# tsilva/gymnasium-solver

Hardware: AMD Instinct MI355X
Metric: env steps/sec (rollout+PPO update), CartPole n_envs=4096, 1/2/4/8 MI355X (higher is better)
Workload: dtype f32; 1 GPU; CartPole-v1:ppo C2 (rollout 4096 envs x 32 steps + 20-epoch PPO update, B=256); n_envs_per_gpu=4096, n_steps=32, batch_size=256, n_epochs=20, policy=MLP 4-256-256-{2,1}, parallelism=single, graph=True, same_device=False, dp_mode=local, track_stats=False

## Files before the change

### gymnasium-solver_amd/csrc/gs_common.h

```cpp
#pragma once
#include <hip/hip_runtime.h>
#include <stdint.h>
#include <stdio.h>
#include <string>
#include <type_traits>

#include "../../include/gsamd.h"

typedef float f32x4 __attribute__((ext_vector_type(4)));
typedef __bf16 bf16x8 __attribute__((ext_vector_type(8)));

namespace gs {

#ifdef GS_STAMPS
extern __device__ unsigned long long g_stamp_acc[8][16];
extern __device__ unsigned long long g_stamp_cnt[8];
#define GS_STAMP_BEGIN_IF(k, cond)                                                 \
    unsigned long long _st_t[17];                                                  \
    int _st_n = 0;                                                                 \
    unsigned long long _st_entry = 0;                                              \
    const bool _st_on = (cond) && threadIdx.x == 0;                                \
    const int _st_k = (k);                                                         \
    if (_st_on) _st_t[0] = __builtin_amdgcn_s_memtime();
#define GS_STAMP_BEGIN(k) GS_STAMP_BEGIN_IF(k, blockIdx.x == 0 && blockIdx.y == 0)
#define GS_STAMP(i)                                                                \
    if (_st_on) _st_t[(i) + 1] = __builtin_amdgcn_s_memtime();                     \
    _st_n = (i) + 1;
#define GS_STAMP_T0 const unsigned long long _st_t0 = __builtin_amdgcn_s_memtime();
#define GS_STAMP_ENTRY                                                             \
    if (_st_on) _st_entry = __builtin_amdgcn_s_memtime() - _st_t0;
#define GS_STAMP_END(i)                                                            \
    GS_STAMP(i)                                                                    \
    if (_st_on) {                                                                  \
        atomicAdd(&g_stamp_acc[_st_k][15], _st_entry);                             \
        for (int _j = 0; _j < _st_n; ++_j)                                         \
            atomicAdd(&g_stamp_acc[_st_k][_j], _st_t[_j + 1] - _st_t[_j]);         \
        atomicAdd(&g_stamp_cnt[_st_k], 1ull);                                      \
    }
#else
#define GS_STAMP_BEGIN(k)
#define GS_STAMP_T0
#define GS_STAMP_ENTRY
#define GS_STAMP_BEGIN_IF(k, cond)
#define GS_STAMP(i)
#define GS_STAMP_END(i)
#endif

void set_error(const char *fmt, ...);
int hip_fail(hipError_t e, const char *what, const char *file, int line);

#define GS_HIP(call)                                                         \
    do {                                                                     \
        hipError_t _e = (call);                                              \
        if (_e != hipSuccess) return gs::hip_fail(_e, #call, __FILE__, __LINE__); \
    } while (0)

#define GS_REQUIRE(cond, ...)                    \
    do {                                         \
        if (!(cond)) {                           \
            gs::set_error(__VA_ARGS__);          \
            return GS_E_INVALID;                 \
        }                                        \
    } while (0)

#define GS_LAUNCH_CHECK(name)                                                        \
    do {                                                                             \
        hipError_t _e = hipGetLastError();                                           \
        if (_e != hipSuccess) return gs::hip_fail(_e, "launch " name, __FILE__, __LINE__); \
    } while (0)

struct Layout {
    int D, H1, H2, A;
    int64_t oW1, ob1, oW2, ob2, oWp, obp, oWv, obv, P;
    __host__ __device__ static constexpr Layout make(int D, int H1, int H2, int A) {
        Layout L{};
        L.D = D; L.H1 = H1; L.H2 = H2; L.A = A;
        L.oW1 = 0;
        L.ob1 = L.oW1 + (int64_t)H1 * D;
        L.oW2 = L.ob1 + H1;
        L.ob2 = L.oW2 + (int64_t)H2 * H1;
        L.oWp = L.ob2 + H2;
        L.obp = L.oWp + (int64_t)A * H2;
        L.oWv = L.obp + A;
        L.obv = L.oWv + H2;
        L.P = L.obv + 1;
        return L;
    }
    __host__ __device__ constexpr int64_t head_row(int a) const { return a < A ? oWp + (int64_t)a * H2 : oWv; }
    __host__ __device__ constexpr int64_t head_bias(int a) const { return a < A ? obp + a : obv; }
};

__host__ __device__ __forceinline__ int64_t part1_index(const Layout &L, int64_t p)
{
    const int D1 = L.D + 1;
    if (p < L.ob1) {
        const int64_t k = p / L.D, d = p - k * L.D;
        return k * D1 + d;
    }
    return (p - L.ob1) * D1 + L.D;
}

template <int D_, int H1_, int H2_, int A_, int B_, int RB_ = 32>
struct ShapeC {
    static constexpr int AMAX = A_, AEX = A_, H1c = H1_, Bc = B_;
    static constexpr int RB = RB_;
    static constexpr bool BF = false;
    __host__ __device__ static constexpr Layout lay(const Layout &) { return Layout::make(D_, H1_, H2_, A_); }
    __host__ __device__ static constexpr int batch(int b) { return B_ > 0 ? B_ : b; }
};
template <int AMAX_>
struct ShapeR {
    static constexpr int AMAX = AMAX_, AEX = 0, H1c = 0, Bc = 0;
    static constexpr int RB = 32;
    static constexpr bool BF = false;
    __host__ __device__ static Layout lay(const Layout &L) { return L; }
    __host__ __device__ static int batch(int b) { return b; }
};

template <class S>
struct Bf16Shape : S {
    static constexpr bool BF = true;
};

constexpr int kTile = 16;

constexpr int kMaxObsDim = 64;
constexpr int kMaxHidden = 1024;
constexpr int kMaxActions = 32;

struct Workspace {
    float *x;
    float *h1;
    float *h2;
    uint16_t *h2mask;
    float *zpart;
    float *dz;
    float *part1;
    float *sumsq;
    float *kl4;
    double *act_parts;
    int32_t *f_act;
    float *f_olp, *f_ov, *f_adv, *f_ret;
    int n_slots;
    size_t bytes;
};
constexpr int kRowsB = 32;
int rows_b(const Layout &L, int64_t B);

struct RowGather {
    const int64_t *actions;
    const float *logprobs, *values, *advantages, *returns;
    int32_t *f_act;
    float *f_olp, *f_ov, *f_adv, *f_ret;
    const int64_t *step_base;
};
Workspace carve_workspace(void *base, const Layout &L, int64_t B);

struct FusedFwd {
    const float *xg;
    const int32_t *fa;
    const float *folp, *fov, *fadv, *fret;
    double *mpart;
    float *headsq;
    double *normsq;
    float *dz;
    const int64_t *step_base;
    int k_local;
    uint32_t *act;
};
constexpr int kActRec = 12;

struct LossArgs {
    float clip_lo, clip_hi;
    float clip_vf;
    float vf_coef, ent_coef;
    float target_kl;
    const int64_t *step_base;
    int normalize;
    float inv_batch;
    int batch_rows;
    const float *adv_stats;
    double *sums_out;
    float *kl_part;
    int bf16;
};

struct AdamArgs {
    float max_norm;
    float one_minus_b1;
    float b2;
    float one_minus_b2;
    float neg_step_size;
    float bc2_sqrt;
    float inv_bc2_sqrt;
    float eps;
    float grad_scale;
    int n_slots;
    int nrb;
    const float *sched;
    int sched_idx;
    const int64_t *step_base;
    int stage_lds;
    double *normsq;
};

struct AdamFwd {
    const float *Min, *Vin;
    const float *G, *part1, *sumsq;
    float *Pout, *Mout, *Vout;
    float *metrics;
    AdamArgs aa;
    int force;
};

constexpr int kBwdXMaxRanks = 8;
constexpr int kBwdXMaxWG = 1024;
constexpr int kBwdXSlot = 1024;
struct BwdXchg {
    char *peer[kBwdXMaxRanks];
    uint32_t off_flags1, off_flags2;
    uint32_t off_data, off_res;
    int world, rank, rsag, region_bytes;
    float scale;
    uint64_t timeout;
    uint32_t *seq;
    uint32_t *err;
};

struct SynthEnvArgs {
    int32_t *state;
    float *ep_ret, *obs;
    int32_t *ep_cnt;
    float *ep_ret_sum, *ep_len_sum;
    int L, trunc_every;
    float reward;
    uint64_t seed, step0;
    int64_t env_offset;
};
struct RolloutRows {
    float *obs;
    int64_t *actions;
    float *logp, *value, *reward;
    uint8_t *done, *timeout;
};

bool rollout_synth_fits(const Layout &L);
int launch_rollout_synth(const float *P, const Layout &L, int64_t N, int T, int mode, uint64_t rng_seed,
                         uint64_t counter0, const SynthEnvArgs &ev, const RolloutRows &rw, hipStream_t s);
bool rollout_env_fits(const Layout &L, int kind);
template <class E>
int launch_rollout(const float *P, const Layout &L, int64_t N, int T, int mode, uint64_t rng_seed, uint64_t counter0,
                   const typename E::Args &ev, const RolloutRows &rw, hipStream_t s);

inline int n_col_blocks(int H) { return (H + kTile - 1) / kTile; }
inline int n_sumsq_slots(const Layout &L) { return n_col_blocks(L.H2) * n_col_blocks(L.H1) + 2 * n_col_blocks(L.H2) + 1; }

int launch_fwd_fused(const float *params, const Layout &L, int64_t B, const FusedFwd &ff, const LossArgs &la,
                     const Workspace &ws, const int32_t *stop, hipStream_t s, const AdamFwd *af = nullptr);
bool has_lagged(const Layout &L, int64_t B);
int launch_gather_all(const Layout &L, int64_t B, int64_t n, const int32_t *idx, const float *obs,
                      const int64_t *actions, const float *logprobs, const float *values, const float *advantages,
                      const float *returns, int64_t T, int64_t N, int normalize, const FusedFwd &ff, float *metrics,
                      hipStream_t s, const float *adv_stats = nullptr);
int launch_kl_decide(const float *kl, float target_kl, int32_t *stop, float *metrics, const int64_t *step_base,
                     hipStream_t s);
int launch_metrics_all(const Layout &L, int64_t B, int64_t n, const FusedFwd &ff, const LossArgs &la, float *metrics,
                       hipStream_t s);
bool has_fused(const Layout &L, int64_t B);
bool has_bf16_chain(const Layout &L, int64_t B);
int launch_fwd_hidden(const float *params, const Layout &L, const float *obs, const int32_t *idx,
                      int64_t T, int64_t N, int64_t rows, float *x_out, float *h1_out, float *h2_out,
                      float *zpart, float *obs_copy, const int32_t *stop_flag, const RowGather *rg, hipStream_t s, uint16_t *h2mask = nullptr);
size_t fwd_lds_bytes(const Layout &L);
int launch_heads_act(const float *P, const Layout &L, const float *zpart, int64_t rows, int mode, uint64_t seed,
                     uint64_t counter, int64_t *actions, float *logp, float *value, hipStream_t s,
                     const uint64_t *clock = nullptr);
int launch_loss(const float *P, const Layout &L, int64_t B, const Workspace &ws, const LossArgs &la, float *metrics,
                int32_t *stop, hipStream_t s);
size_t bwd_lds_bytes(const Layout &L, int64_t B);
int prepare_kernels(const Layout &L, int64_t B);
int launch_bwd(const float *P, const Layout &L, int64_t B, const Workspace &ws, float *G, const int32_t *stop,
               hipStream_t s, const FusedFwd *ff = nullptr, const LossArgs *la = nullptr,
               const BwdXchg *bx = nullptr);
bool bwd_xchg_fits(const Layout &L, int64_t B, int colocated = 1);
int launch_clip_adam(float *P, const Layout &L, float *G, float *M, float *V, const float *part1,
                     const float *sumsq, const AdamArgs &aa, float *metrics, const int32_t *stop, hipStream_t s,
                     bool comp_norms = true);
int launch_act_stats(const float *P, const Layout &L, const float *obs, const int32_t *idx, int64_t T, int64_t N,
                     int64_t R, double *part, hipStream_t s, const int64_t *step_base = nullptr);
int launch_act_parts_record(const Layout &L, int64_t R, const double *part, const int32_t *stop, float *metrics,
                            const int64_t *step_base, hipStream_t s);
int launch_act_stats_fused(const Layout &L, int64_t B, int64_t n, const uint32_t *act, float *metrics, hipStream_t s);
int launch_head_sq(const Layout &L, const float *G, float scale, const FusedFwd &ff, hipStream_t s);
int launch_reduce_part1(const float *part1, const Layout &L, int nrb, float *G, const int32_t *stop, hipStream_t s);
int launch_global_adv_sums(const int32_t *idx, int64_t n, int64_t B, const float *adv, int64_t T, int64_t N,
                           double *sums, hipStream_t s);
int launch_global_adv_stats(const double *sums, int64_t n, int64_t Bg, float *stats, hipStream_t s);
int launch_global_records(const double *sums, int64_t n, const LossArgs &la, float *metrics, hipStream_t s);
int launch_sumsq_flat(const float *G, int64_t n, float *out, int nblocks, hipStream_t s);
int set_lds_limit(const void *fn, size_t bytes);

struct Layout1 {
    int D, H, A;
    int oW1, ob1, oWp, obp, oWv, obv, P;
    __host__ __device__ static constexpr Layout1 make(int D, int H, int A)
    {
        Layout1 L{};
        L.D = D; L.H = H; L.A = A;
        L.oW1 = 0;
        L.ob1 = L.oW1 + H * D;
        L.oWp = L.ob1 + H;
        L.obp = L.oWp + A * H;
        L.oWv = L.obp + A;
        L.obv = L.oWv + H;
        L.P = L.obv + 1;
        return L;
    }
    __host__ __device__ constexpr int head_row(int a) const { return a < A ? oWp + a * H : oWv; }
    __host__ __device__ constexpr int head_bias(int a) const { return a < A ? obp + a : obv; }
};
int mlp1_check_dims(const gs_mlp_dims &d);
size_t mlp1_update_lds_bytes(const gs_mlp_dims &d);
int mlp1_policy_act(const float *params, const gs_mlp_dims &d, const float *obs, int64_t N, int mode, uint64_t rng_seed,
                    uint64_t rng_counter, int64_t *actions, float *logp, float *value, float *obs_store,
                    const uint64_t *clock, hipStream_t s);
int mlp1_update(float *params, float *grads, float *adam_m, float *adam_v, const gs_mlp_dims &d,
                const gs_ppo_hparams &hp, const gs_rollout_view &ro, const int32_t *idx, int64_t batch, int64_t n,
                int64_t adam_step0, float *metrics, int32_t *stop_flag, bool loss_only, hipStream_t s);
int mlp1_activation_stats(const float *params, const gs_mlp_dims &d, const gs_rollout_view &ro, const int32_t *idx,
                          int64_t rows, double *part, hipStream_t s);

__device__ __forceinline__ bf16x8 bf16_frag(float4 lo, float4 hi)
{
    bf16x8 r;
    r[0] = (__bf16)lo.x, r[1] = (__bf16)lo.y, r[2] = (__bf16)lo.z, r[3] = (__bf16)lo.w;
    r[4] = (__bf16)hi.x, r[5] = (__bf16)hi.y, r[6] = (__bf16)hi.z, r[7] = (__bf16)hi.w;
    return r;
}
__device__ __forceinline__ bf16x8 bf16_frag(const float (&v)[8])
{
    bf16x8 r;
#pragma unroll
    for (int j = 0; j < 8; ++j) r[j] = (__bf16)v[j];
    return r;
}
__device__ __forceinline__ f32x4 mfma16_bf16(bf16x8 a, bf16x8 b, f32x4 c)
{
    return __builtin_amdgcn_mfma_f32_16x16x32_bf16(a, b, c, 0, 0, 0);
}

__device__ __forceinline__ uint16_t act_bf16(float v)
{
    const uint16_t u = __builtin_bit_cast(uint16_t, (__bf16)v);
    return (v > 0.f && u == 0) ? (uint16_t)1 : u;
}
__device__ __forceinline__ float bf16_f32(uint16_t u) { return __uint_as_float((uint32_t)u << 16); }
__device__ __forceinline__ float4 bf16x4_f32(uint2 u)
{
    return make_float4(__uint_as_float(u.x << 16), __uint_as_float(u.x & 0xffff0000u), __uint_as_float(u.y << 16),
                       __uint_as_float(u.y & 0xffff0000u));
}
template <bool XH>
using act_t = typename std::conditional<XH, uint16_t, float>::type;
template <bool XH>
__device__ __forceinline__ float act_ld(const act_t<XH> *p, int64_t i)
{
    if constexpr (XH) return bf16_f32(p[i]);
    else return p[i];
}
template <bool XH>
__device__ __forceinline__ float4 act_ld4(const act_t<XH> *p, int64_t i)
{
    if constexpr (XH) return bf16x4_f32(*reinterpret_cast<const uint2 *>(p + i));
    else return *reinterpret_cast<const float4 *>(p + i);
}
template <bool XH>
__device__ __forceinline__ void act_st(act_t<XH> *p, int64_t i, float v)
{
    if constexpr (XH) p[i] = act_bf16(v);
    else p[i] = v;
}

struct ActOut {
    uint32_t *cnt;
    float *part;
};
__device__ __forceinline__ void act_acc(const ActOut &ao, float z, int64_t neuron, float &s, float &q)
{
    s += z;
    q += z * z;
    if (fabsf(z) < 1e-6f) atomicAdd(ao.cnt + neuron, 1u);
}
__device__ __forceinline__ void act_flush(const ActOut &ao, int64_t slot, float s, float q)
{
#pragma unroll
    for (int o = 32; o > 0; o >>= 1) {
        s += __shfl_xor(s, o, 64);
        q += __shfl_xor(q, o, 64);
    }
    if ((threadIdx.x & 63) == 0) {
        ao.part[2 * slot] = s;
        ao.part[2 * slot + 1] = q;
    }
}

}
```

### gymnasium-solver_amd/csrc/gs_mlp.hip

```cpp
#include <float.h>

#include <mutex>
#include <type_traits>
#include <unordered_map>

#include "gs_common.h"
#include "gs_head.h"
#include "gs_xgmi_dev.h"
#include "gs_synth_env.h"
#include "gs_cartpole_env.h"
#include "gs_acrobot_env.h"
#include "gs_mountaincar_env.h"
#include "gs_bandit_env.h"

namespace gs {

#ifdef GS_STAMPS
__device__ unsigned long long g_stamp_acc[8][16];
__device__ unsigned long long g_stamp_cnt[8];
#endif
#if defined(GS_STAMPS) || defined(GS_SPANS)
constexpr int kSpanK = 2048, kSpanWG = 288;
__device__ unsigned g_span[2][kSpanK][kSpanWG][9];
__device__ __forceinline__ int span_wg() { return (int)(blockIdx.x + blockIdx.y * gridDim.x); }
__device__ __forceinline__ void span_start(int kern, int64_t k, unsigned long long t0)
{
    if (threadIdx.x == 0 && k >= 0 && k < kSpanK && span_wg() < kSpanWG) g_span[kern][k][span_wg()][0] = (unsigned)t0;
}
__device__ __forceinline__ void span_end(int kern, int64_t k)
{
    if ((threadIdx.x & 63) == 0 && k >= 0 && k < kSpanK && span_wg() < kSpanWG) {
        asm volatile("s_waitcnt vmcnt(0) lgkmcnt(0)" ::: "memory");
        g_span[kern][k][span_wg()][1 + (threadIdx.x >> 6)] = (unsigned)__builtin_amdgcn_s_memrealtime();
    }
}
#define GS_SPAN_T0 const unsigned long long _sp_t0 = __builtin_amdgcn_s_memrealtime();
#define GS_SPAN_START(slot, k) span_start(slot, k, _sp_t0);
#define GS_SPAN_END(slot, k) span_end(slot, k);
#else
#define GS_SPAN_T0
#define GS_SPAN_START(slot, k) ;
#define GS_SPAN_END(slot, k) ;
#endif

__device__ __forceinline__ f32x4 mfma4(float a, float b, f32x4 c)
{
    return __builtin_amdgcn_mfma_f32_16x16x4f32(a, b, c, 0, 0, 0);
}

__device__ __forceinline__ f32x4 mfma_bf16_pair(float4 a0, float4 a1, float4 b0, float4 b1, f32x4 c)
{
    return mfma16_bf16(bf16_frag(a0, a1), bf16_frag(b0, b1), c);
}
__device__ __forceinline__ float4 f4(const float (&v)[4]) { return make_float4(v[0], v[1], v[2], v[3]); }

template <typename T>
__device__ __forceinline__ T wave_sum(T v)
{
#pragma unroll
    for (int o = 32; o > 0; o >>= 1) v += __shfl_xor(v, o, 64);
    return v;
}

__host__ __device__ constexpr int round4(int n) { return (n + 3) & ~3; }


__device__ __forceinline__ void store_component_norms(double (&hq)[2], double total_sq, float gscale, float *rec,
                                                      double *scratch)
{
    block_reduce<2>(hq, scratch);
    if (threadIdx.x == 0 && rec) {
        rec[GS_M_GN_POLICY_HEAD] = (float)sqrt(hq[0]) * gscale;
        rec[GS_M_GN_VALUE_HEAD] = (float)sqrt(hq[1]) * gscale;
        rec[GS_M_GN_BACKBONE] = (float)sqrt(fmax(0.0, total_sq - hq[0] - hq[1])) * gscale;
        rec[GS_M_GN_MLP] = 0.0f;
    }
}

template <int NV, typename T>
__device__ __forceinline__ void block_reduce_t0(T (&v)[NV], T *scratch)
{
    const int tid = threadIdx.x;
    if (tid < 256)
#pragma unroll
        for (int k = 0; k < NV; ++k) scratch[k * 256 + tid] = v[k];
    __syncthreads();
    T *part = scratch + NV * 256;
    if (tid < NV * 16) {
        const int k = tid >> 4, j = tid & 15;
        T acc = 0;
#pragma unroll
        for (int m = 0; m < 16; ++m) acc += scratch[k * 256 + j * 16 + m];
        part[tid] = acc;
    }
    __syncthreads();
    if (tid == 0)
#pragma unroll
        for (int k = 0; k < NV; ++k) {
            T acc = 0;
#pragma unroll
            for (int j = 0; j < 16; ++j) acc += part[k * 16 + j];
            v[k] = acc;
        }
}

__device__ __forceinline__ void copy_to_lds(float *dst, const float *src, int n)
{
    const int tid = threadIdx.x;
    if ((((uintptr_t)src | (uintptr_t)dst) & 15) == 0) {
        const int n4 = n >> 2;
#pragma unroll 8
        for (int u = tid; u < n4; u += 256)
            reinterpret_cast<float4 *>(dst)[u] = reinterpret_cast<const float4 *>(src)[u];
        for (int u = (n4 << 2) + tid; u < n; u += 256) dst[u] = src[u];
    } else {
#pragma unroll 4
        for (int u = tid; u < n; u += 256) dst[u] = src[u];
    }
}

__device__ __forceinline__ void store_component_norms(double (&hq)[2], double total_sq, float gscale, float *rec,
                                                      double *scratch);
__host__ __device__ inline int64_t head_grad_offset(const Layout &L, int u, bool *value)
{
    const int nw = (L.A + 1) * L.H2;
    if (u < nw) {
        const int a = u / L.H2;
        *value = a == L.A;
        return L.head_row(a) + (u - a * L.H2);
    }
    *value = u - nw == L.A;
    return L.head_bias(u - nw);
}


size_t fwd_lds_bytes(const Layout &L)
{
    const int A1 = L.A + 1;
    size_t n = 16 + round4(L.H1 * L.D) + round4(L.H1) + kTile * (L.H1 + 4) + 16 + round4(A1 * 16) +
               round4(kTile * L.D) + kTile * (L.H1 + 4) + 1024 + kTile * 17;
    return n * sizeof(float);
}

template <int AMAX, int AEX>
__device__ __forceinline__ void gather_head_row(const float *__restrict__ zpart, const float *__restrict__ P,
                                                const Layout &L, int64_t r, float (&z)[AMAX + 1]);
template <int AMAX>
__device__ __forceinline__ void loss_row(const float (&z)[AMAX + 1], int A, int act, float olp, float ov, float adv,
                                         float ret, const LossArgs &la, float invB, float *__restrict__ dzr,
                                         double (&acc)[14]);

#ifndef GS_FWD_ADAM_NT
#define GS_FWD_ADAM_NT 512
#endif
constexpr int kFwdAdamThreads = GS_FWD_ADAM_NT;
static_assert(kFwdAdamThreads == 256 || kFwdAdamThreads == 512, "lagged forward: 256 or 512 threads");

constexpr int kMinDeadWaveLoads = 64;
template <int NT, int NQ1, int NRB>
struct FwdWaveClasses {
    static constexpr int NW = NT / 64, NQ = (NQ1 + 255) / 256, NQP = (NQ1 + NT - 1) / NT;
    static constexpr int live_npq(int w)
    {
        int n = 0;
        for (int j = 0; j < NQ; ++j) n += w < 4 && 256 * j + 64 * w < NQ1;
        return n;
    }
    static constexpr int live_nw1(int w)
    {
        int n = 0;
        for (int j = 0; j < NQP; ++j) n += NT * j + 64 * w < NQ1;
        return n;
    }
    static constexpr int dead_wave_loads()
    {
        int n = 0;
        for (int w = 0; w < NW; ++w) n += (NQ - live_npq(w)) * NRB + (NQP - live_nw1(w)) * 3;
        return n;
    }
    static constexpr bool kSplit = dead_wave_loads() >= kMinDeadWaveLoads;
    static constexpr bool nrm(int w) { return !kSplit || w < 4; }
    static constexpr int npq(int w) { return kSplit ? live_npq(w) : NQ; }
    static constexpr int nw1(int w) { return kSplit ? live_nw1(w) : NQP; }
    static constexpr bool same(int a, int b) { return nrm(a) == nrm(b) && npq(a) == npq(b) && nw1(a) == nw1(b); }
    static constexpr int end(int w)
    {
        int e = w + 1;
        while (e < NW && same(w, e)) ++e;
        return e;
    }
};
template <class WC, int W, class F>
__device__ __forceinline__ void for_wave_class(int wv, F &&f)
{
    constexpr int E = WC::end(W);
    if constexpr (E >= WC::NW) {
        f(std::integral_constant<int, W>{});
    } else {
        if (wv < E)
            f(std::integral_constant<int, W>{});
        else
            for_wave_class<WC, E>(wv, f);
    }
}

template <class S, bool FUSED, bool ADAM, bool STATS, bool BASE>
__device__ __forceinline__ void fwd_hidden_body(
    const float *__restrict__ P, const Layout &Lrt, const float *__restrict__ obs, const int32_t *__restrict__ idx,
    int T, int N, int rows, float *__restrict__ x_out, float *__restrict__ h1_out, float *__restrict__ h2_out,
    float *__restrict__ zpart, float *__restrict__ obs_copy, const int32_t *__restrict__ stop, const RowGather &rg,
    const FusedFwd &ff, uint16_t *__restrict__ h2mask, const AdamFwd &af)
{
    GS_STAMP_BEGIN(0)
    GS_SPAN_T0
    GS_STAMP_T0
    if constexpr (!FUSED)
        if (stop && *stop) return;
    extern __shared__ float lds[];
    const Layout L = S::lay(Lrt);
    const int D = L.D, H1 = L.H1, H2 = L.H2, A1 = L.A + 1;
    const int cb = blockIdx.x, rb = blockIdx.y;
    const int r0 = rb * kTile;
    const int c0 = cb * kTile;
    const int tid = threadIdx.x, lane = tid & 63, wave = tid >> 6;
    constexpr int NT = ADAM ? kFwdAdamThreads : 256;
    const int ldh = H1 + 4;
    int *srcs = reinterpret_cast<int *>(lds);
    float *W1s = lds + 16;
    float *b1s = W1s + round4(H1 * D);
    float *W2s = b1s + round4(H1);
    float *b2s = W2s + kTile * ldh;
    float *whs = b2s + 16;
    float *xs = whs + round4(A1 * 16);
    float *h1s = xs + round4(kTile * D);
    float *red = h1s + kTile * ldh;
    float *h2s = red + 1024;

    if constexpr (!FUSED)
        if (rg.step_base && idx) idx += *rg.step_base * rows;
    int64_t kstep = FUSED ? ff.k_local : 0;
    if constexpr (FUSED && BASE) kstep += ff.step_base ? *ff.step_base : 0;
    if constexpr (ADAM) GS_SPAN_START(0, kstep)
    constexpr bool kStage0 = FUSED && S::H1c > 0 && (S::H1c * 4) % 4 == 0;
    constexpr int kW2v = S::H1c > 0 ? kTile * S::H1c / 4 / NT : 0;
    float4 w2r[kW2v > 0 ? kW2v : 1];
    static_assert(!ADAM || (kStage0 && kW2v > 0), "lagged Adam: compile-time fused shapes only");
    if constexpr (ADAM) {
        constexpr Layout Lc = S::lay(Layout{});
        constexpr int cD = Lc.D, cH1 = Lc.H1, cA1 = Lc.A + 1, n1 = cH1 * (cD + 1), k4n = cH1 / 4;
        constexpr int NQ = (n1 / 4 + 255) / 256, NRB = (S::Bc + S::RB - 1) / S::RB, NS = 2;
        static_assert(Lc.oW1 == 0 && Lc.oW2 == n1 && (cH1 * cD) % 4 == 0 && cH1 % 4 == 0, "W1|b1: one float4 region");
        static_assert(NRB >= 1 && NRB <= 8 && NQ <= 2 && n1 <= kTile * (cH1 + 4), "lagged-Adam register / LDS budget");
        const AdamArgs &aa = af.aa;
        const bool fold = af.part1 != nullptr;
        const float4 z4 = make_float4(0.f, 0.f, 0.f, 0.f);
        auto ld4 = [](const float *base, int64_t q) {
            const f32x4 v = *(const __attribute__((address_space(1))) f32x4 *)(base + 4 * q);
            return make_float4(v[0], v[1], v[2], v[3]);
        };
        auto ld1 = [](const float *base, int64_t o) { return *(const __attribute__((address_space(1))) float *)(base + o); };
        constexpr int nq1 = n1 / 4;
        using WC = FwdWaveClasses<NT, nq1, NRB>;
        static_assert(WC::NQ == NQ, "norm partial quads");
        const float *tsrc = fold ? af.part1 : af.G;
        const int64_t tstride = fold ? (int64_t)n1 : 0;
        const int nrb_used = fold ? NRB : 1;
        auto prologue = [&](auto first_wave) __attribute__((always_inline)) {
            constexpr int W0 = decltype(first_wave)::value;
            constexpr bool nrmc = WC::nrm(W0);
            const bool nrm = nrmc && (WC::kSplit || NT == 256 || tid < 256);
            constexpr int NPQ = WC::npq(W0), NQP = WC::nw1(W0);
            float sl[nrmc ? NS : 1];
            if constexpr (nrmc)
#pragma unroll
                for (int j = 0; j < NS; ++j) sl[j] = ld1(af.sumsq, nrm ? min(tid + 256 * j, aa.n_slots - 1) : 0);
            GS_STAMP_ENTRY
            float4 w1p[NQP > 0 ? NQP : 1], w1m[NQP > 0 ? NQP : 1], w1v[NQP > 0 ? NQP : 1], t[NPQ > 0 ? NPQ : 1][NRB];
#pragma unroll
            for (int j = 0; j < NPQ; ++j)
#pragma unroll
                for (int b = 0; b < NRB; ++b)
                    t[j][b] = ld4(tsrc + (int64_t)b * tstride, nrm ? min(tid + 256 * j, nq1 - 1) : 0);
#pragma unroll
            for (int j = 0; j < NQP; ++j) {
                const int q = min(tid + NT * j, nq1 - 1);
                w1p[j] = ld4(P, q);
                w1m[j] = ld4(af.Min, q);
                w1v[j] = ld4(af.Vin, q);
            }
            float4 w2m[kW2v], w2v[kW2v], w2g[kW2v];
#pragma unroll
            for (int j = 0; j < kW2v; ++j) {
                const int u = tid + NT * j, i = u / k4n, k4 = u - i * k4n;
                const int64_t q = (Lc.oW2 + (int64_t)min(c0 + i, H2 - 1) * cH1) / 4 + k4;
                w2r[j] = ld4(P, q);
                w2m[j] = ld4(af.Min, q);
                w2v[j] = ld4(af.Vin, q);
                w2g[j] = ld4(af.G, q);
            }
            int force = af.force;
            if constexpr (WC::kSplit) {
                __builtin_amdgcn_sched_barrier(0);
                asm volatile("; lagged forward: wave class %1" : "+s"(force) : "n"(W0));
// ... 699 lines not shown
            for (int i = tid / H1; i < kTile; i += 256 / H1) {
                float acc = 0.0f;
#pragma unroll
                for (int d = 0; d < kW1Reg; ++d)
                    if (d < D) acc = fmaf(xs[i * D + d], w1r[d], acc);
                acc += b1r;
                h1s[i * ldh + k] = acc > 0.0f ? acc : 0.0f;
            }
        } else {
            for (int u = tid; u < kTile * H1; u += 256) {
                const int i = u / H1, k = u - i * H1;
                float acc = 0.0f;
                for (int d = 0; d < D; ++d) acc = fmaf(xs[i * D + d], W1s[k * D + d], acc);
                acc += b1s[k];
                h1s[i * ldh + k] = acc > 0.0f ? acc : 0.0f;
            }
        }
        __syncthreads();
        for (int cb = wave; cb < ncb; cb += 4) {
            const int c0 = cb * kTile;
            f32x4 acc0[4], acc1[4], part[4];
#pragma unroll
            for (int q = 0; q < 4; ++q) acc0[q] = acc1[q] = f32x4{0.f, 0.f, 0.f, 0.f};
            const int nmax = (nch + 3) / 4;
            for (int c = 0; c < nmax; ++c) {
#pragma unroll
                for (int q = 0; q < 4; ++q) {
                    const int ch = (q * nch) / 4 + c;
                    if (ch >= ((q + 1) * nch) / 4) continue;
                    const int k = ch * kTile + 4 * lq;
                    const float4 a = *reinterpret_cast<const float4 *>(h1s + li * ldh + k);
                    const float4 b = c0 + li < H2 ? *reinterpret_cast<const float4 *>(W2s + (c0 + li) * ldh + k)
                                                  : make_float4(0.f, 0.f, 0.f, 0.f);
                    acc0[q] = mfma4(a.x, b.x, acc0[q]);
                    acc1[q] = mfma4(a.y, b.y, acc1[q]);
                    acc0[q] = mfma4(a.z, b.z, acc0[q]);
                    acc1[q] = mfma4(a.w, b.w, acc1[q]);
                }
            }
#pragma unroll
            for (int q = 0; q < 4; ++q) part[q] = acc0[q] + acc1[q];
#pragma unroll
            for (int r = 0; r < 4; ++r) {
                const int row = lq * 4 + r;
                const float s = ((part[0][r] + part[1][r]) + part[2][r]) + part[3][r];
                float h = 0.0f;
                if (c0 + li < H2) {
                    h = s + b2s[c0 + li];
                    h = h > 0.0f ? h : 0.0f;
                }
                h2s[(cb * kTile + row) * 17 + li] = h;
            }
        }
        __syncthreads();
        for (int u = tid; u < ncb * kTile * A1; u += 256) {
            const int cb = u / (kTile * A1), rem = u - cb * kTile * A1, row = rem / A1, a = rem - row * A1;
            float z = 0.0f;
#pragma unroll
            for (int c = 0; c < kTile; ++c) {
                const float w = cb * kTile + c < H2 ? whs[a * H2 + cb * kTile + c] : 0.0f;
                z = fmaf(h2s[(cb * kTile + row) * 17 + c], w, z);
            }
            zps[(row * ncb + cb) * A1 + a] = z;
        }
        __syncthreads();
        if (env_thread) {
            float z[AMAX + 1];
#pragma unroll
            for (int a = 0; a < AMAX + 1; ++a) z[a] = 0.0f;
            if constexpr (S::AEX > 0) {
                for (int cbb = 0; cbb < ncb; cbb += 16)
#pragma unroll
                    for (int j = 0; j < 16; ++j)
#pragma unroll
                        for (int a = 0; a < AMAX + 1; ++a)
                            if (a < A1) z[a] += cbb + j < ncb ? zps[(tid * ncb + cbb + j) * A1 + a] : 0.0f;
            } else {
                for (int cb = 0; cb < ncb; ++cb)
#pragma unroll
                    for (int a = 0; a < AMAX + 1; ++a)
                        if (a < A1) z[a] += zps[(tid * ncb + cb) * A1 + a];
            }
#pragma unroll
            for (int a = 0; a < AMAX + 1; ++a)
                if (a < A1) z[a] += bhs[a];
            const int64_t o = row0 + me;
            head_act_row<AMAX>(z, A, mode, rng_seed, counter0 + (uint64_t)t, me, rw.actions + o, rw.logp + o,
                               rw.value + o);
            const auto so = env.step(ev, me, rw.actions[o]);
            rw.reward[o] = so.reward;
            rw.done[o] = so.done ? 1 : 0;
            rw.timeout[o] = so.timeout ? 1 : 0;
        }
        env.next_obs(ev, xs, e0, N, D, t, tid, env_thread);
        __syncthreads();
    }
    if (env_thread) env.store(ev, me);
    for (int u = tid; u < kTile * D; u += 256) {
        const int i = u / D;
        if (e0 + i < N) ev.obs[(e0 + i) * D + (u - i * D)] = xs[u];
    }
}

bool rollout_synth_fits(const Layout &L)
{
    return L.H1 % kTile == 0 && L.H1 >= kTile && rollout_synth_lds_bytes(L) <= 160 * 1024;
}

template <class Sh, class E>
int launch_rollout_sh(const float *P, const Layout &L, int64_t N, int T, int mode, uint64_t rng_seed,
                      uint64_t counter0, const typename E::Args &ev, const RolloutRows &rw, hipStream_t s)
{
    const size_t lds = rollout_synth_lds_bytes(L);
    const dim3 grid((unsigned)((N + kTile - 1) / kTile));
    int rc = set_lds_limit((const void *)k_rollout_env<Sh, E>, lds);
    if (rc) return rc;
    hipLaunchKernelGGL((k_rollout_env<Sh, E>), grid, dim3(256), lds, s, P, L, N, T, mode, rng_seed, counter0, ev, rw);
    GS_LAUNCH_CHECK("k_rollout_env");
    return GS_OK;
}

int launch_rollout_synth(const float *P, const Layout &L, int64_t N, int T, int mode, uint64_t rng_seed,
                         uint64_t counter0, const SynthEnvArgs &ev, const RolloutRows &rw, hipStream_t s)
{
    GS_REQUIRE(rollout_synth_fits(L), "gs_rollout_synth: the policy does not fit in LDS");
    return with_shape(L, 0, [&](auto sh) {
        return launch_rollout_sh<decltype(sh), RolloutSynthEnv>(P, L, N, T, mode, rng_seed, counter0, ev, rw, s);
    });
}

template <class E>
static bool rollout_fits(const Layout &L)
{
    return E::takes_policy(L.D, L.A) && rollout_synth_fits(L);
}

bool rollout_env_fits(const Layout &L, int kind)
{
    if (kind == GS_ENV_CARTPOLE) return rollout_fits<CartPoleEnv>(L);
    if (kind == GS_ENV_ACROBOT) return rollout_fits<AcrobotEnv>(L);
    if (kind == GS_ENV_MOUNTAINCAR) return rollout_fits<MountainCarEnv>(L);
    if (kind == GS_ENV_BANDIT) return rollout_fits<BanditEnv>(L);
    return false;
}

template <class E>
int launch_rollout(const float *P, const Layout &L, int64_t N, int T, int mode, uint64_t rng_seed, uint64_t counter0,
                   const typename E::Args &ev, const RolloutRows &rw, hipStream_t s)
{
    GS_REQUIRE(rollout_fits<E>(L),
               "one-launch rollout: the policy (obs dim %d, %d actions) is not the env's or does not fit in LDS", L.D,
               L.A);
    return launch_rollout_sh<ShapeR<E::kRolloutAmax>, E>(P, L, N, T, mode, rng_seed, counter0, ev, rw, s);
}
#define GS_ROLLOUT_INSTANCE(E)                                                                                  \
    template int launch_rollout<E>(const float *, const Layout &, int64_t, int, int, uint64_t, uint64_t,       \
                                   const E::Args &, const RolloutRows &, hipStream_t)
GS_ROLLOUT_INSTANCE(CartPoleEnv);
GS_ROLLOUT_INSTANCE(CartPoleShapedEnv);
GS_ROLLOUT_INSTANCE(AcrobotEnv);
GS_ROLLOUT_INSTANCE(MountainCarEnv);
GS_ROLLOUT_INSTANCE(BanditEnv);
#undef GS_ROLLOUT_INSTANCE



template <class S>
__global__ __launch_bounds__(256) void k_loss(const float *__restrict__ P, Layout Lrt, const float *__restrict__ zpart,
                                              int Brt, const int32_t *__restrict__ f_act,
                                              const float *__restrict__ f_olp, const float *__restrict__ f_ov,
                                              const float *__restrict__ f_adv, const float *__restrict__ f_ret,
                                              LossArgs la, float *__restrict__ dz, float *__restrict__ metrics,
                                              int32_t *__restrict__ stop)
{
    __shared__ double sred[kNumSums * (256 + 16)];
    constexpr int AMAX = S::AMAX, AEX = S::AEX;
    const Layout L = S::lay(Lrt);
    const int B = S::batch(Brt);
    const int tid = threadIdx.x;
    if (la.step_base) metrics += *la.step_base * GS_NUM_METRICS;
    GS_STAMP_BEGIN(1)
    if (stop && *stop) {
        if (tid == 0) {
            for (int k = 0; k < GS_NUM_METRICS; ++k) metrics[k] = 0.0f;
            metrics[GS_M_SKIPPED] = 1.0f;
            metrics[GS_M_KL_STOP] = 1.0f;
            metrics[GS_M_UNEVALUATED] = 1.0f;
        }
        return;
    }
    const int A = L.A, A1 = A + 1;
    const float invB = la.inv_batch;
    const int64_t kb = la.step_base ? *la.step_base : 0;

    float meanf = 0.0f, stdf = 1.0f;
    if (la.normalize && la.adv_stats) {
        meanf = la.adv_stats[2 * kb];
        stdf = la.adv_stats[2 * kb + 1];
    } else if (la.normalize) {
        double m1[1] = {0.0};
        for (int r = tid; r < B; r += 256) m1[0] += (double)f_adv[r];
        block_reduce<1>(m1, sred);
        const double mean = m1[0] / (double)B;
        double q[1] = {0.0};
        for (int r = tid; r < B; r += 256) {
            const double dv = (double)f_adv[r] - mean;
            q[0] += dv * dv;
        }
        block_reduce<1>(q, sred);
        meanf = (float)mean;
        stdf = (float)sqrt(q[0] / (double)(B - 1));
    }
    GS_STAMP(0)

    double acc[kNumSums];
#pragma unroll
    for (int k = 0; k < kNumSums; ++k) acc[k] = 0.0;
    for (int r = tid; r < B; r += 256) {
        float z[AMAX + 1];
        gather_head_row<AMAX, AEX>(zpart, P, L, r, z);
        const int act = f_act[r];
        float adv = f_adv[r];
        if (la.normalize) adv = (adv - meanf) / (stdf + 1e-8f);
        if (act < 0) {
            for (int a = 0; a < A1; ++a) dz[(int64_t)r * A1 + a] = 0.0f;
            continue;
        }
        loss_row<AMAX>(z, A, act, f_olp[r], f_ov[r], adv, f_ret[r], la, invB, dz + (int64_t)r * A1, acc);
    }
    GS_STAMP(1)
    block_reduce<kNumSums>(acc, sred);
    GS_STAMP(2)
    if (tid == 0) {
        const double rows = (double)la.batch_rows;
        write_metrics(acc, rows, la, metrics, true);
        metrics[GS_M_GRAD_NORM] = 0.0f;
        if (la.sums_out)
            for (int q = 0; q < kNumSums; ++q) la.sums_out[kb * kNumSums + q] = acc[q];
        if (la.kl_part) {
            la.kl_part[0] = (float)(acc[6] * (double)invB);
            metrics[GS_M_KL_STOP] = metrics[GS_M_SKIPPED] = 0.0f;
        } else {
            const float approx_kl = (float)(acc[6] / rows);
            if (la.target_kl > 0.0f && approx_kl > la.target_kl && stop) *stop = 1;
        }
    }
    GS_STAMP_END(3)
}

__device__ __forceinline__ void block_sumsq_store(float v, float *slot, float *sbuf)
{
    float t[1] = {v};
    block_reduce_t0<1>(t, sbuf);
    if (threadIdx.x == 0) *slot = t[0];
}

__device__ __forceinline__ void store_head_split(const float *v, int A, float *headsq, int64_t o)
{
    if (threadIdx.x == 0 && headsq) {
        float p = 0.0f;
        for (int a = 0; a < A; ++a) p += v[a];
        headsq[o] = p;
        headsq[o + 1] = v[A];
    }
}

__device__ __forceinline__ void store_head_sums(float sq, float sqp, float sqv, float *slot, float *headsq,
                                                int64_t o, float *sbuf)
{
    if (!headsq) {
        block_sumsq_store(sq, slot, sbuf);
        return;
    }
    float t[3] = {sq, sqp, sqv};
    block_reduce_t0<3>(t, sbuf);
    if (threadIdx.x == 0) {
        *slot = t[0];
        headsq[o] = t[1];
        headsq[o + 1] = t[2];
    }
}

__host__ __device__ inline int metric_owner(int g, int G, int nW) { return G <= nW ? g : (int)(((int64_t)g * nW) / G); }
__host__ __device__ inline int metric_groups_per_wg(int G, int nW) { return G <= nW ? 1 : (G + nW - 1) / nW; }

struct BwdShape {
    int ncb, nkb, nrbB, ka, nT, nA, nB, nC;
    __host__ __device__ static BwdShape make(const Layout &L, int B, int rb)
    {
        const int kRowsB = rb;
        BwdShape s;
        s.ncb = (L.H2 + kTile - 1) / kTile;
        s.nkb = (L.H1 + kTile - 1) / kTile;
        s.nrbB = (B + kRowsB - 1) / kRowsB;
        s.ka = s.nkb % 2 == 0 ? 2 : 1;
        s.nT = s.ncb * s.nkb;
        s.nA = s.ncb * (s.nkb / s.ka);
        s.nB = s.nrbB * s.nkb;
        s.nC = s.ncb + 1;
        return s;
    }
};

size_t bwd_lds_bytes(const Layout &L, int64_t B)
{
    const int kRowsB = rows_b(L, B);
    const int A1 = L.A + 1;
    const int64_t Bp64 = (B + 63) / 64 * 64, Bp16 = (B + 15) / 16 * 16;
    const int64_t H2p = (L.H2 + 63) / 64 * 64;
    const BwdShape shp = BwdShape::make(L, (int)B, kRowsB);
    const bool fastA = A1 <= 5, regsB = A1 <= 5 && L.H2 % 64 == 0;
    const int64_t roleA = round4((int)B * A1) + round4(A1 * 16) + ((fastA ? 0 : 1) + 2) * kTile * (Bp64 + 4) + 3072 +
                          Bp64 + (fastA ? 0 : 816);
    const int64_t roleB = (regsB ? (int64_t)round4(kRowsB / 16 * 16 * (L.D + 1)) : (int64_t)kRowsB * (H2p + 4)) +
                          kTile * (H2p + 4) + round4(A1 * L.H2) + round4(kRowsB * A1) +
                          kRowsB * 16 + round4(kRowsB * L.D) + kRowsB * 17 + 1024 +
                          (int64_t)kRowsB * n_col_blocks(L.H2);
    const int64_t roleC = Bp16 * 17 + round4((int)Bp16 * A1) + (A1 * 256 > 1024 ? A1 * 256 : 1024) + 2 +
                          (int64_t)metric_groups_per_wg((int)B / kTile, shp.nC) * kTile * kNumSums * 2;
    int64_t m = roleA;
    if (roleB > m) m = roleB;
    if (roleC > m) m = roleC;
    return (size_t)m * sizeof(float);
}

template <class S>
__device__ __forceinline__ void loss_rows_lds(const float *__restrict__ P, const Layout &L,
                                              const float *__restrict__ zpart, const FusedFwd &ff,
                                              const LossArgs &la, int B, int64_t k, int r0, int n, float *dzs,
                                              double *dscr, int t0 = 0, int nthr = 256, int d0 = 0,
                                              int d1 = 1 << 30)
{
    constexpr int AMAX = S::AMAX, AEX = S::AEX;
    const int A1 = L.A + 1;
    const int me = (int)threadIdx.x - t0;
    if (me < 0 || me >= nthr) return;
    for (int i = me; i < n; i += nthr) {
        const int r = r0 + i;
        double acc[kNumSums];
#pragma unroll
        for (int q = 0; q < kNumSums; ++q) acc[q] = 0.0;
        const int rc = r < B ? r : B - 1;
        const int64_t o = k * B + rc;
        const int fa = ff.fa[o];
        const float folp = ff.folp[o], fov = ff.fov[o], fadv = ff.fadv[o], fret = ff.fret[o];
        float z[AMAX + 1];
        gather_head_row<AMAX, AEX>(zpart, P, L, rc, z);
        const bool live = r < B && fa >= 0;
        loss_row<AMAX>(z, L.A, fa, folp, fov, fadv, fret, la, la.inv_batch, dzs + i * A1, acc);
        if (!live) {
            for (int a = 0; a < A1; ++a) dzs[i * A1 + a] = 0.0f;
#pragma unroll
            for (int q = 0; q < kNumSums; ++q) acc[q] = 0.0;
        }
        if (dscr && r >= d0 && r < d1)
#pragma unroll
            for (int q = 0; q < kNumSums; ++q) dscr[(r - d0) * kNumSums + q] = acc[q];
    }
}

__device__ __forceinline__ void store_metric_groups(const double *dscr, int n, int r0, int B, int64_t k,
                                                    double *__restrict__ mp)
{
    const int ng = n / kTile;
    if ((int)threadIdx.x < ng * kNumSums) {
        const int g = threadIdx.x / kNumSums, q = threadIdx.x - g * kNumSums;
        double t = 0.0;
        for (int i = 0; i < kTile; ++i) t += dscr[(g * kTile + i) * kNumSums + q];
        mp[(k * (B / kTile) + r0 / kTile + g) * kNumSums + q] = t;
    }
}

template <class S, bool FUSED, bool XCHG, bool BASE>
__device__ __forceinline__ void bwd_body(const float *__restrict__ P, const Layout &Lrt, int Brt,
                                         const float *__restrict__ x, const float *__restrict__ h1,
                                         const float *__restrict__ h2, const float *__restrict__ dz,
                                         float *__restrict__ G, float *__restrict__ part1,
                                         float *__restrict__ sumsq, const int32_t *__restrict__ stop,
                                         const float *__restrict__ zpart, const FusedFwd &ff, const LossArgs &la,
                                         const uint16_t *__restrict__ h2mask, const BwdXchg &bx)
{
    GS_SPAN_T0
    GS_STAMP_T0
    if constexpr (!FUSED)
        if (stop && *stop) return;
    const bool xchg = XCHG && bx.world > 1;
    const uint32_t xseq = xchg ? bx.seq[blockIdx.x] + 1u : 0u;
    int64_t kstep = FUSED ? ff.k_local : 0;
    if constexpr (FUSED && BASE) kstep += ff.step_base ? *ff.step_base : 0;
    if constexpr (FUSED) GS_SPAN_START(1, kstep)
    extern __shared__ float lds[];
    __shared__ float sbuf[FUSED ? 3 * 272 : 272];
    const Layout L = S::lay(Lrt);
    const int B = S::batch(Brt);
    const int D = L.D, H1 = L.H1, H2 = L.H2, A = L.A, A1 = A + 1;
    constexpr int kRowsB = S::RB;
    const BwdShape sh = BwdShape::make(L, B, kRowsB);
    const int tid = threadIdx.x, lane = tid & 63, wave = tid >> 6;
    const int li = lane & 15, lq = lane >> 4;
    int bid = (int)blockIdx.x;
    if (bid < sh.nB) bid += sh.nA;
    else if (bid < sh.nB + sh.nA) bid -= sh.nB;

    if (bid < sh.nA) {
        const int nkg = sh.nkb / sh.ka;
        const int nb = bid / nkg, kb = (bid - nb * nkg) * sh.ka;
        const int n0 = nb * kTile, k0 = kb * kTile, kw = kTile * sh.ka;
        GS_STAMP_BEGIN_IF(2, bid == 0)
        const int Bp = (B + 63) / 64 * 64;
        const int ld = Bp + 4;
        const bool fast = A1 <= 5;
        float *dzs = lds;
        float *whs = dzs + round4(B * A1);
        float *dh2T = whs + round4(A1 * 16);
        float *h1T = dh2T + (fast ? 0 : kTile * ld);
        float *red = h1T + kw * ld;
        int *mkA = reinterpret_cast<int *>(red + 3072);
        if constexpr (S::H1c > 0 && S::Bc > 0) {
            constexpr Layout Lc = S::lay(Layout{});
            constexpr int cB = S::Bc, cBp = (cB + 63) / 64 * 64, cncb = (Lc.H2 + kTile - 1) / kTile;
            constexpr int cka = (Lc.H1 / kTile) % 2 == 0 ? 2 : 1, ckw = kTile * cka, cq = ckw / 4;
            constexpr int NMk = (cBp + 255) / 256, NH1 = (cBp * cq + 255) / 256;
            int mr[NMk];
            float4 hr[NH1];
            float wh = 0.0f;
#pragma unroll
            for (int j = 0; j < NMk; ++j) {
                const int b = tid + 256 * j;
                mr[j] = (int)h2mask[(int64_t)min(b, cB - 1) * cncb + nb];
            }
            GS_STAMP_ENTRY
#pragma unroll
            for (int j = 0; j < NH1; ++j) {
                const int u = tid + 256 * j, b = u / cq, c4 = u % cq;
                hr[j] = *reinterpret_cast<const float4 *>(h1 + (int64_t)min(b, cB - 1) * Lc.H1 +
                                                          min(k0 + 4 * c4, Lc.H1 - 4));
            }
            {
                const int a = min(tid >> 4, A1 - 1), j = tid & 15;
                wh = P[L.head_row(a) + min(n0 + j, H2 - 1)];
            }
            if constexpr (FUSED)
                loss_rows_lds<S>(P, L, zpart, ff, la, B, kstep, 0, B, dzs, nullptr);
            else
                copy_to_lds(dzs, dz, B * A1);
            if (tid < A1 * kTile) whs[tid] = n0 + (tid & 15) < H2 ? wh : 0.0f;
#pragma unroll
            for (int j = 0; j < NMk; ++j)
                if (tid + 256 * j < cBp) mkA[tid + 256 * j] = tid + 256 * j < cB ? mr[j] : 0;
#pragma unroll
            for (int j = 0; j < NH1; ++j) {
                const int u = tid + 256 * j, b = u / cq, c4 = u % cq;
                if (u < cBp * cq) {
                    const bool ok = b < cB && k0 + 4 * c4 < Lc.H1;
                    h1T[(4 * c4 + 0) * ld + b] = ok ? hr[j].x : 0.0f;
                    h1T[(4 * c4 + 1) * ld + b] = ok ? hr[j].y : 0.0f;
                    h1T[(4 * c4 + 2) * ld + b] = ok ? hr[j].z : 0.0f;
                    h1T[(4 * c4 + 3) * ld + b] = ok ? hr[j].w : 0.0f;
                }
            }
        } else {
            if constexpr (FUSED)
                loss_rows_lds<S>(P, L, zpart, ff, la, B, kstep, 0, B, dzs, nullptr);
            else
                copy_to_lds(dzs, dz, B * A1);
            if (tid < A1 * kTile) {
                const int a = tid >> 4, j = tid & 15;
                whs[tid] = n0 + j < H2 ? P[L.head_row(a) + n0 + j] : 0.0f;
            }
            for (int b = tid; b < Bp; b += 256) mkA[b] = b < B ? (int)h2mask[(int64_t)b * sh.ncb + nb] : 0;
            const int q4 = kw / 4;
#pragma unroll 4
            for (int u = tid; u < Bp * q4; u += 256) {
                const int b = u / q4, c4 = u - b * q4;
                float4 gv = make_float4(0.f, 0.f, 0.f, 0.f);
                if (b < B && k0 + 4 * c4 < H1)
                    gv = *reinterpret_cast<const float4 *>(h1 + (int64_t)b * H1 + k0 + 4 * c4);
                h1T[(4 * c4 + 0) * ld + b] = gv.x;
                h1T[(4 * c4 + 1) * ld + b] = gv.y;
                h1T[(4 * c4 + 2) * ld + b] = gv.z;
                h1T[(4 * c4 + 3) * ld + b] = gv.w;
            }
        }
        __syncthreads();
        GS_STAMP(0)
        const int nch = Bp / kTile;
        const int ch0 = (wave * nch) / 4, ch1 = ((wave + 1) * nch) / 4;
        const int nt = sh.ka + (!fast && kb == 0 ? 1 : 0);
        if (fast) {
            float w[5];
#pragma unroll
            for (int a = 0; a < 5; ++a) w[a] = a < A1 ? whs[a * 16 + li] : 0.0f;
            f32x4 acc[3][2];
#pragma unroll
            for (int t = 0; t < 3; ++t) acc[t][0] = acc[t][1] = f32x4{0.f, 0.f, 0.f, 0.f};
            float dsum = 0.0f;
            auto dh2_rows = [&](int b, float (&av)[4]) {
#pragma unroll
                for (int c = 0; c < 4; ++c) {
                    float sacc = 0.0f;
#pragma unroll
                    for (int a = 0; a < 5; ++a) sacc = a < A1 ? fmaf(dzs[(b + c) * A1 + a], w[a], sacc) : sacc;
                    av[c] = (mkA[b + c] >> li) & 1 ? sacc : 0.0f;
                }
            };
            if constexpr (S::BF) {
                const float4 z4 = make_float4(0.f, 0.f, 0.f, 0.f);
#pragma unroll 2
                for (int ch = ch0; ch < ch1; ch += 2) {
                    const int b = ch * kTile + 4 * lq;
                    const bool two = ch + 1 < ch1;
                    float av0[4], av1[4] = {0.f, 0.f, 0.f, 0.f};
                    dh2_rows(b, av0);
                    if (two) dh2_rows(b + kTile, av1);
                    if (kb == 0) {
                        dsum = (((dsum + av0[0]) + av0[1]) + av0[2]) + av0[3];
                        dsum = (((dsum + av1[0]) + av1[1]) + av1[2]) + av1[3];
                    }
#pragma unroll
                    for (int t = 0; t < 2; ++t) {
                        if (t >= nt) break;
                        const float *hb = h1T + (t * kTile + li) * ld + b;
                        const float4 bb0 = *reinterpret_cast<const float4 *>(hb);
                        const float4 bb1 = two ? *reinterpret_cast<const float4 *>(hb + kTile) : z4;
                        acc[t][0] = mfma_bf16_pair(f4(av0), f4(av1), bb0, bb1, acc[t][0]);
                    }
                }
            } else {
#pragma unroll 2
            for (int ch = ch0; ch < ch1; ++ch) {
                const int b = ch * kTile + 4 * lq;
                float av[4];
                dh2_rows(b, av);
                if (kb == 0) dsum = (((dsum + av[0]) + av[1]) + av[2]) + av[3];
#pragma unroll
                for (int t = 0; t < 3; ++t) {
                    if (t >= nt) break;
                    const float4 bb = t == sh.ka ? make_float4(1.f, 1.f, 1.f, 1.f)
                                                 : *reinterpret_cast<const float4 *>(h1T + (t * kTile + li) * ld + b);
                    acc[t][0] = mfma4(av[0], bb.x, acc[t][0]);
                    acc[t][1] = mfma4(av[1], bb.y, acc[t][1]);
                    acc[t][0] = mfma4(av[2], bb.z, acc[t][0]);
                    acc[t][1] = mfma4(av[3], bb.w, acc[t][1]);
                }
            }
            }
            GS_STAMP(1)
#pragma unroll
            for (int t = 0; t < 3; ++t) {
                if (t >= nt) break;
                const f32x4 at = acc[t][0] + acc[t][1];
#pragma unroll
                for (int r = 0; r < 4; ++r) red[(wave * 3 + t) * 256 + (lq * 4 + r) * kTile + li] = at[r];
            }
            if (kb == 0) red[(wave * 3 + 2) * 256 + lq * kTile + li] = dsum;
        } else {
            {
                const int i = tid & 15;
                float w[kMaxActions + 1];
#pragma unroll
                for (int a = 0; a < kMaxActions + 1; ++a) w[a] = a < A1 ? whs[a * 16 + i] : 0.0f;
                for (int b = tid >> 4; b < Bp; b += 16) {
                    const bool on = (mkA[b] >> i) & 1;
                    float s = 0.0f;
#pragma unroll
                    for (int a = 0; a < kMaxActions + 1; ++a) s = a < A1 ? fmaf(dzs[b * A1 + a], w[a], s) : s;
                    dh2T[i * ld + b] = on ? s : 0.0f;
                }
            }
            __syncthreads();
            GS_STAMP(1)
            for (int t = 0; t < nt; ++t) {
                f32x4 acc0 = {0.f, 0.f, 0.f, 0.f}, acc1 = {0.f, 0.f, 0.f, 0.f};
                const float *hb = h1T + t * kTile * ld;
                const bool ones = t == sh.ka;
#pragma unroll 4
                for (int ch = ch0; ch < ch1; ++ch) {
                    const int b = ch * kTile + 4 * lq;
                    const float4 a = *reinterpret_cast<const float4 *>(dh2T + li * ld + b);
                    const float4 bb = ones ? make_float4(1.f, 1.f, 1.f, 1.f)
                                           : *reinterpret_cast<const float4 *>(hb + li * ld + b);
                    acc0 = mfma4(a.x, bb.x, acc0);
                    acc1 = mfma4(a.y, bb.y, acc1);
                    acc0 = mfma4(a.z, bb.z, acc0);
                    acc1 = mfma4(a.w, bb.w, acc1);
                }
                const f32x4 acc = acc0 + acc1;
#pragma unroll
                for (int r = 0; r < 4; ++r) red[(wave * 3 + t) * 256 + (lq * 4 + r) * kTile + li] = acc[r];
            }
        }
        __syncthreads();
        GS_STAMP(2)
        {
            const int row = tid >> 4, col = tid & 15;
            float gv[3] = {0.0f, 0.0f, 0.0f};
            bool ok[3] = {false, false, false};
            for (int t = 0; t < nt; ++t) {
                const float g = ((red[(0 + t) * 256 + tid] + red[(3 + t) * 256 + tid]) + red[(6 + t) * 256 + tid]) +
                                red[(9 + t) * 256 + tid];
                const int j = t < sh.ka ? t : 2;
                gv[j] = g;
                ok[j] = t < sh.ka ? (n0 + row < H2 && k0 + t * kTile + col < H1) : (col == 0 && n0 + row < H2);
            }
            int db2n = n0 + row;
            if (fast && kb == 0) {
                db2n = n0 + tid;
                float d = 0.0f;
                if (tid < kTile)
#pragma unroll
                    for (int q = 0; q < 16; ++q) d += red[((q >> 2) * 3 + 2) * 256 + (q & 3) * kTile + tid];
                gv[2] = d;
                ok[2] = tid < kTile && n0 + tid < H2;
            }
            if (xchg) bwd_exchange<3>(bx, xseq, gv, ok);
            float sqt[3] = {0.0f, 0.0f, 0.0f};
            for (int t = 0; t < sh.ka; ++t) {
                if (!ok[t]) continue;
                G[L.oW2 + (int64_t)(n0 + row) * H1 + k0 + t * kTile + col] = gv[t];
                sqt[t] = gv[t] * gv[t];
            }
            if (ok[2]) {
                G[L.ob2 + db2n] = gv[2];
                sqt[2] = gv[2] * gv[2];
            }
            block_reduce_t0<3>(sqt, fast ? h1T : reinterpret_cast<float *>(mkA + Bp));
            if (tid == 0) {
                for (int t = 0; t < sh.ka; ++t) sumsq[nb * sh.nkb + kb + t] = sqt[t];
                if (kb == 0) sumsq[sh.nT + nb] = sqt[2];
            }
        }
        GS_STAMP_END(3)
        if constexpr (FUSED) GS_SPAN_END(1, kstep)
        return;
    }
    bid -= sh.nA;
    if (bid < sh.nB) {
        int rb, kb;
        if (sh.nkb == 16 && sh.ka == 2 && sh.nB % 8 == 0) {
            const int x = bid & 7, i = bid >> 3;
            kb = 2 * x + (i & 1);
            rb = i >> 1;
        } else {
            rb = bid / sh.nkb;
            kb = bid - rb * sh.nkb;
        }
        const int b0 = rb * kRowsB, k0 = kb * kTile;
        GS_STAMP_BEGIN_IF(4, bid == 0)
        const int H2p = (H2 + 63) / 64 * 64;
        const int ld = H2p + 4;
        const bool dh2_regs = A1 <= 5 && H2 % 64 == 0;
        float *dh2s = lds;
        float *W2T = dh2s + (dh2_regs ? round4(kRowsB / 16 * 16 * (D + 1)) : kRowsB * ld);
        float *whs = W2T + kTile * ld;
        float *dzs = whs + round4(A1 * H2);
        float *h1m = dzs + round4(kRowsB * A1);
        float *xs = h1m + kRowsB * 16;
        float *tile = xs + round4(kRowsB * D);
        float *kred = tile + kRowsB * 17;
        constexpr int kLd = FUSED ? 192 : 256;
        int *mkB = reinterpret_cast<int *>(kred + 1024);
        if constexpr (S::H1c > 0 && S::Bc > 0) {
            constexpr Layout Lc = S::lay(Layout{});
            constexpr int cH1 = Lc.H1, cH2 = Lc.H2, cD = Lc.D, cA1 = Lc.A + 1, cB = S::Bc;
            constexpr int cncb = (cH2 + kTile - 1) / kTile, cH2p = (cH2 + 63) / 64 * 64;
            constexpr int NM = (kRowsB * cncb + kLd - 1) / kLd, NW = (cH2p * 4 + kLd - 1) / kLd;
            constexpr int NH = (cA1 * cH2 + kLd - 1) / kLd, N1 = (kRowsB * 16 + kLd - 1) / kLd;
            constexpr int NX = (kRowsB * cD + kLd - 1) / kLd;
            if (tid < kLd) {
                int mr[NM];
                float4 wr[NW];
                float hr[NH], h1r[N1], xr[NX];
#pragma unroll
                for (int j = 0; j < NM; ++j) {
                    const int u = min(tid + j * kLd, kRowsB * cncb - 1), i = u / cncb, c = u - i * cncb;
                    mr[j] = (int)h2mask[(int64_t)min(b0 + i, cB - 1) * cncb + c];
                }
                GS_STAMP_ENTRY
#pragma unroll
                for (int j = 0; j < NW; ++j) {
                    const int u = tid + j * kLd, n = min(u >> 2, cH2 - 1), c4 = u & 3;
                    wr[j] = *reinterpret_cast<const float4 *>(P + Lc.oW2 + (int64_t)n * cH1 + min(k0 + 4 * c4, cH1 - 4));
                }
#pragma unroll
                for (int j = 0; j < NH; ++j) {
                    const int u = min(tid + j * kLd, cA1 * cH2 - 1), a = u / cH2, n = u - a * cH2;
                    hr[j] = P[Lc.head_row(a) + n];
                }
#pragma unroll
                for (int j = 0; j < N1; ++j) {
                    const int u = tid + j * kLd, i = min(u >> 4, kRowsB - 1), jj = u & 15;
                    h1r[j] = h1[(int64_t)min(b0 + i, cB - 1) * cH1 + min(k0 + jj, cH1 - 1)];
                }
#pragma unroll
                for (int j = 0; j < NX; ++j) {
                    const int u = tid + j * kLd;
                    xr[j] = x[min((int64_t)b0 * cD + u, (int64_t)cB * cD - 1)];
                }
#pragma unroll
                for (int j = 0; j < NM; ++j) {
                    const int u = tid + j * kLd, i = u / cncb;
                    if (u < kRowsB * cncb) mkB[u] = b0 + i < cB ? mr[j] : 0;
                }
#pragma unroll
                for (int j = 0; j < NW; ++j) {
                    const int u = tid + j * kLd, n = u >> 2, c4 = u & 3;
                    if (u < cH2p * 4) {
                        const bool ok = n < cH2 && k0 + 4 * c4 < cH1;
                        W2T[(4 * c4 + 0) * ld + n] = ok ? wr[j].x : 0.0f;
                        W2T[(4 * c4 + 1) * ld + n] = ok ? wr[j].y : 0.0f;
                        W2T[(4 * c4 + 2) * ld + n] = ok ? wr[j].z : 0.0f;
                        W2T[(4 * c4 + 3) * ld + n] = ok ? wr[j].w : 0.0f;
                    }
                }
#pragma unroll
                for (int j = 0; j < NH; ++j)
                    if (tid + j * kLd < cA1 * cH2) whs[tid + j * kLd] = hr[j];
#pragma unroll
                for (int j = 0; j < N1; ++j) {
                    const int u = tid + j * kLd, i = u >> 4, jj = u & 15;
                    if (u < kRowsB * 16) h1m[u] = (b0 + i < cB && k0 + jj < cH1) ? h1r[j] : 0.0f;
                }
#pragma unroll
                for (int j = 0; j < NX; ++j) {
                    const int u = tid + j * kLd;
                    if (u < kRowsB * cD) xs[u] = b0 * cD + u < cB * cD ? xr[j] : 0.0f;
                }
            }
        } else if (!FUSED || tid < kLd) {
            for (int u = tid; u < kRowsB * sh.ncb; u += kLd) {
                const int i = u / sh.ncb, c = u - i * sh.ncb;
                mkB[u] = b0 + i < B ? (int)h2mask[(int64_t)(b0 + i) * sh.ncb + c] : 0;
            }
#pragma unroll 4
            for (int u = tid; u < H2p * 4; u += kLd) {
                const int n = u >> 2, c4 = u & 3;
                float4 w = make_float4(0.f, 0.f, 0.f, 0.f);
                if (n < H2 && k0 + 4 * c4 < H1)
                    w = *reinterpret_cast<const float4 *>(P + L.oW2 + (int64_t)n * H1 + k0 + 4 * c4);
                W2T[(4 * c4 + 0) * ld + n] = w.x;
                W2T[(4 * c4 + 1) * ld + n] = w.y;
                W2T[(4 * c4 + 2) * ld + n] = w.z;
                W2T[(4 * c4 + 3) * ld + n] = w.w;
            }
            for (int u = tid; u < A1 * H2; u += kLd) {
                const int a = u / H2, n = u - a * H2;
                whs[u] = P[L.head_row(a) + n];
            }
            for (int u = tid; u < kRowsB * 16; u += kLd) {
                const int i = u >> 4, j = u & 15;
                h1m[u] = (b0 + i < B && k0 + j < H1) ? h1[(int64_t)(b0 + i) * H1 + k0 + j] : 0.0f;
            }
            for (int u = tid; u < kRowsB * D; u += kLd) xs[u] = b0 * D + u < B * D ? x[(int64_t)b0 * D + u] : 0.0f;
        }
#ifdef GS_STAMPS
        const unsigned long long t_rb0 = __builtin_amdgcn_s_memtime();
        if (bid == 0 && tid == 0) {
            asm volatile("s_waitcnt vmcnt(0) lgkmcnt(0)" ::: "memory");
            atomicAdd(&g_stamp_acc[6][0], __builtin_amdgcn_s_memtime() - t_rb0);
            atomicAdd(&g_stamp_cnt[6], 1ull);
        }
#endif
        if constexpr (FUSED) {
            loss_rows_lds<S>(P, L, zpart, ff, la, B, kstep, b0, kRowsB, dzs, nullptr, kLd, 256 - kLd);
        } else {
            for (int u = tid; u < kRowsB * A1; u += 256)
                dzs[u] = b0 * A1 + u < B * A1 ? dz[(int64_t)b0 * A1 + u] : 0.0f;
        }
#ifdef GS_STAMPS
        if (bid == 0 && tid == 192) {
            asm volatile("s_waitcnt vmcnt(0) lgkmcnt(0)" ::: "memory");
            atomicAdd(&g_stamp_acc[7][0], __builtin_amdgcn_s_memtime() - t_rb0);
            atomicAdd(&g_stamp_cnt[7], 1ull);
        }
#endif
        __syncthreads();
        GS_STAMP(0)
        static_assert(kRowsB == 32 || kRowsB == 64, "role-B slabs of 32 or 64 rows");
        const int nchB = H2p / kTile;
        const int rt = kRowsB == 64 ? wave : wave >> 1, half = kRowsB == 64 ? 0 : wave & 1;
        const int chb = half ? nchB / 2 : 0, che = (half || kRowsB == 64) ? nchB : nchB / 2;
        f32x4 acc0 = {0.f, 0.f, 0.f, 0.f}, acc1 = {0.f, 0.f, 0.f, 0.f};
        if (dh2_regs) {
            const int row = rt * 16 + li;
            float dzr[5];
#pragma unroll
            for (int a = 0; a < 5; ++a) dzr[a] = a < A1 ? dzs[row * A1 + a] : 0.0f;
            const float *brow = W2T + li * ld;
            auto dh2_cols = [&](int ch, float (&av)[4]) {
                const int n = ch * kTile + 4 * lq;
                const unsigned m = (unsigned)(mkB[row * sh.ncb + ch] >> (4 * lq));
                float4 wh[5];
#pragma unroll
                for (int a = 0; a < 5; ++a)
                    wh[a] = a < A1 ? *reinterpret_cast<const float4 *>(whs + a * H2 + n) : make_float4(0.f, 0.f, 0.f, 0.f);
#pragma unroll
                for (int j = 0; j < 4; ++j) {
                    float sacc = 0.0f;
#pragma unroll
                    for (int a = 0; a < 5; ++a) {
                        const float wv = j == 0 ? wh[a].x : j == 1 ? wh[a].y : j == 2 ? wh[a].z : wh[a].w;
                        sacc = a < A1 ? fmaf(dzr[a], wv, sacc) : sacc;
                    }
                    av[j] = ((m >> j) & 1u) ? sacc : 0.0f;
                }
            };
            if constexpr (S::BF) {
                const float4 z4 = make_float4(0.f, 0.f, 0.f, 0.f);
#pragma unroll 2
                for (int ch = chb; ch < che; ch += 2) {
                    const int n = ch * kTile + 4 * lq;
                    const bool two = ch + 1 < che;
                    float av0[4], av1[4] = {0.f, 0.f, 0.f, 0.f};
                    dh2_cols(ch, av0);
                    if (two) dh2_cols(ch + 1, av1);
                    const float4 w0 = *reinterpret_cast<const float4 *>(brow + n);
                    const float4 w1 = two ? *reinterpret_cast<const float4 *>(brow + n + kTile) : z4;
                    acc0 = mfma_bf16_pair(f4(av0), f4(av1), w0, w1, acc0);
                }
            } else {
#pragma unroll 2
            for (int ch = chb; ch < che; ++ch) {
                const int n = ch * kTile + 4 * lq;
                float av[4];
                dh2_cols(ch, av);
                const float4 w = *reinterpret_cast<const float4 *>(brow + n);
                acc0 = mfma4(av[0], w.x, acc0);
                acc1 = mfma4(av[1], w.y, acc1);
                acc0 = mfma4(av[2], w.z, acc0);
                acc1 = mfma4(av[3], w.w, acc1);
            }
            }
            GS_STAMP(1)
        } else {
        if (A1 <= 5 && H2 <= 1024 && 1024 % H2 == 0) {
            const int nt = H2 >> 2, rstep = 256 / nt;
            const int n0 = 4 * (tid % nt), nb = n0 >> 4, sh4 = n0 & 15;
            float w[5][4];
#pragma unroll
            for (int a = 0; a < 5; ++a)
#pragma unroll
                for (int j = 0; j < 4; ++j) w[a][j] = a < A1 ? whs[a * H2 + n0 + j] : 0.0f;
            for (int i0 = tid / nt; i0 < kRowsB; i0 += 8 * rstep) {
                unsigned mm[8];
                float dzr[8][5];
#pragma unroll
                for (int c = 0; c < 8; ++c) {
                    const int i = min(i0 + c * rstep, kRowsB - 1);
                    mm[c] = (unsigned)(mkB[i * sh.ncb + nb] >> sh4);
#pragma unroll
                    for (int a = 0; a < 5; ++a) dzr[c][a] = a < A1 ? dzs[i * A1 + a] : 0.0f;
                }
#pragma unroll
                for (int c = 0; c < 8; ++c) {
                    const int i = i0 + c * rstep;
                    float o[4];
#pragma unroll
                    for (int j = 0; j < 4; ++j) {
                        float sacc = 0.0f;
#pragma unroll
                        for (int a = 0; a < 5; ++a) sacc = a < A1 ? fmaf(dzr[c][a], w[a][j], sacc) : sacc;
                        o[j] = ((mm[c] >> j) & 1u) ? sacc : 0.0f;
                    }
                    if (i < kRowsB)
                        *reinterpret_cast<float4 *>(dh2s + i * ld + n0) = make_float4(o[0], o[1], o[2], o[3]);
                }
            }
        } else
        for (int n = tid; n < H2; n += 256) {
            float w[kMaxActions + 1];
#pragma unroll
            for (int a = 0; a < kMaxActions + 1; ++a) w[a] = a < A1 ? whs[a * H2 + n] : 0.0f;
            const int nb = n >> 4, nbit = n & 15;
            if (A1 <= 5) {
#pragma unroll 8
                for (int i = 0; i < kRowsB; ++i) {
                    const bool on = (mkB[i * sh.ncb + nb] >> nbit) & 1;
                    float s = 0.0f;
#pragma unroll
                    for (int a = 0; a < 5; ++a) s = a < A1 ? fmaf(dzs[i * A1 + a], w[a], s) : s;
                    dh2s[i * ld + n] = on ? s : 0.0f;
                }
            } else {
                for (int i = 0; i < kRowsB; ++i) {
                    const bool on = (mkB[i * sh.ncb + nb] >> nbit) & 1;
                    float s = 0.0f;
#pragma unroll
                    for (int a = 0; a < kMaxActions + 1; ++a) s = a < A1 ? fmaf(dzs[i * A1 + a], w[a], s) : s;
                    dh2s[i * ld + n] = on ? s : 0.0f;
                }
            }
        }
        for (int u = tid; u < kRowsB * (H2p - H2); u += 256) {
            const int i = u / (H2p - H2), n = H2 + (u - i * (H2p - H2));
            dh2s[i * ld + n] = 0.0f;
        }
        __syncthreads();
        GS_STAMP(1)
        {
            const float *arow = dh2s + (rt * 16 + li) * ld;
            const float *brow = W2T + li * ld;
#pragma unroll 4
            for (int ch = chb; ch < che; ++ch) {
                const int n = ch * kTile + 4 * lq;
                const float4 a = *reinterpret_cast<const float4 *>(arow + n);
                const float4 w = *reinterpret_cast<const float4 *>(brow + n);
                acc0 = mfma4(a.x, w.x, acc0);
                acc1 = mfma4(a.y, w.y, acc1);
                acc0 = mfma4(a.z, w.z, acc0);
                acc1 = mfma4(a.w, w.w, acc1);
            }
        }
        }
        {
            const f32x4 acc = acc0 + acc1;
#pragma unroll
            for (int r = 0; r < 4; ++r) kred[wave * 256 + (lq * 4 + r) * kTile + li] = acc[r];
        }
        __syncthreads();
        for (int u = tid; u < kRowsB * kTile; u += 256) {
            const int row = u >> 4, col = u & 15;
            const int t = row >> 4, rr = row & 15;
            const float g = kRowsB == 64 ? kred[t * 256 + rr * kTile + col]
                                         : kred[(2 * t) * 256 + rr * kTile + col] + kred[(2 * t + 1) * 256 + rr * kTile + col];
            tile[row * 17 + col] = h1m[row * 16 + col] > 0.0f ? g : 0.0f;
        }
        __syncthreads();
        GS_STAMP(2)
        {
            constexpr int ng = kRowsB / 16;
            float *pr = dh2s;
            const int nout = kTile * (D + 1);
            for (int u = tid; u < ng * nout; u += 256) {
                const int g = u / nout, o = u - g * nout;
                const int col = o / (D + 1), d = o - col * (D + 1);
                float s = 0.0f;
#pragma unroll 4
                for (int row = g * 16; row < g * 16 + 16; ++row) {
                    const float xv = d < D ? xs[row * D + d] : 1.0f;
                    s = fmaf(tile[row * 17 + col], xv, s);
                }
                pr[u] = s;
            }
            __syncthreads();
            if (xchg) {
                float pv[4];
                bool ok[4];
#pragma unroll
                for (int j = 0; j < 4; ++j) {
                    const int o = tid + 256 * j, col = o / (D + 1);
                    ok[j] = o < nout && k0 + col < H1;
                    float t = 0.0f;
                    if (o < nout)
#pragma unroll
                        for (int g = 0; g < ng; ++g) t += pr[g * nout + o];
                    pv[j] = t;
                }
                bwd_exchange<4>(bx, xseq, pv, ok);
#pragma unroll
                for (int j = 0; j < 4; ++j) {
                    const int o = tid + 256 * j, col = o / (D + 1), d = o - col * (D + 1);
                    if (ok[j]) part1[((int64_t)rb * H1 + k0 + col) * (D + 1) + d] = pv[j];
                }
            } else
            for (int o = tid; o < nout; o += 256) {
                const int col = o / (D + 1), d = o - col * (D + 1);
                float t = 0.0f;
#pragma unroll
                for (int g = 0; g < ng; ++g) t += pr[g * nout + o];
                if (k0 + col < H1) part1[((int64_t)rb * H1 + k0 + col) * (D + 1) + d] = t;
            }
        }
        GS_STAMP_END(3)
        if constexpr (FUSED) GS_SPAN_END(1, kstep)
        return;
    }
    bid -= sh.nB;
    {
        const int nb = (sh.ncb == 16 && bid < 16) ? 2 * (bid & 7) + (bid >> 3) : bid;
        const int n0 = nb * kTile;
        const int Bp = (B + 15) / 16 * 16;
        GS_STAMP_BEGIN_IF(5, bid == 0)
        float *hs = lds;
        float *dzs = hs + Bp * 17;
        int gs = 0, ge = 0;
        if constexpr (FUSED) {
            const int G = B / kTile;
            gs = G;
            for (int g = 0; g < G; ++g)
                if (metric_owner(g, G, sh.nC) == nb) {
                    gs = min(gs, g);
                    ge = g + 1;
                }
            if (ge == 0) gs = 0;
        }
        double *dscrC = reinterpret_cast<double *>(
            (reinterpret_cast<uintptr_t>(dzs + Bp * A1 + (A1 * 256 > 1024 ? A1 * 256 : 1024)) + 7) & ~(uintptr_t)7);
        auto loss_in = [&]() {
            if constexpr (FUSED)
                loss_rows_lds<S>(P, L, zpart, ff, la, B, kstep, 0, Bp, dzs, ge > gs ? dscrC : nullptr, 0, 256,
                                 kTile * gs, kTile * ge);
            else
                for (int u = tid; u < Bp * A1; u += 256) dzs[u] = u < B * A1 ? dz[u] : 0.0f;
        };
        if constexpr (S::H1c > 0 && S::Bc > 0) {
            constexpr Layout Lc = S::lay(Layout{});
            constexpr int cB = S::Bc, cBp = (cB + 15) / 16 * 16, NH = (cBp * 4 + 255) / 256;
            float4 hr[NH];
#pragma unroll
            for (int j = 0; j < NH; ++j) {
                const int u = tid + 256 * j, b = u >> 2, c4 = u & 3;
                hr[j] = *reinterpret_cast<const float4 *>(h2 + (int64_t)min(b, cB - 1) * Lc.H2 +
                                                          min(n0 + 4 * c4, Lc.H2 - 4));
            }
            GS_STAMP_ENTRY
            loss_in();
#pragma unroll
            for (int j = 0; j < NH; ++j) {
                const int u = tid + 256 * j, b = u >> 2, c4 = u & 3;
                if (u < cBp * 4) {
                    const bool ok = b < cB && n0 + 4 * c4 < Lc.H2;
                    hs[b * 17 + 4 * c4 + 0] = ok ? hr[j].x : 0.0f;
                    hs[b * 17 + 4 * c4 + 1] = ok ? hr[j].y : 0.0f;
                    hs[b * 17 + 4 * c4 + 2] = ok ? hr[j].z : 0.0f;
                    hs[b * 17 + 4 * c4 + 3] = ok ? hr[j].w : 0.0f;
                }
            }
        } else {
#pragma unroll 4
            for (int u = tid; u < Bp * 4; u += 256) {
                const int b = u >> 2, c4 = u & 3;
                float4 hv = make_float4(0.f, 0.f, 0.f, 0.f);
                if (b < B && n0 + 4 * c4 < H2)
                    hv = *reinterpret_cast<const float4 *>(h2 + (int64_t)b * H2 + n0 + 4 * c4);
                hs[b * 17 + 4 * c4 + 0] = hv.x;
                hs[b * 17 + 4 * c4 + 1] = hv.y;
                hs[b * 17 + 4 * c4 + 2] = hv.z;
                hs[b * 17 + 4 * c4 + 3] = hv.w;
            }
            loss_in();
        }
        __syncthreads();
        GS_STAMP(0)
        if constexpr (FUSED)
            for (int g = gs; g < ge; ++g)
                store_metric_groups(dscrC + (int64_t)(g - gs) * kTile * kNumSums, kTile, g * kTile, B, kstep,
                                    ff.mpart);
        float *partC = dzs + Bp * A1;
        if (nb < sh.ncb) {
            const int nout = kTile * A1;
            float sq = 0.0f, sqp = 0.0f, sqv = 0.0f;
            if (A1 <= kTile) {
                const int li = lane & 15, lq = lane >> 4;
                const int nch = Bp / kTile;
                const int ch0 = (wave * nch) / 4, ch1 = ((wave + 1) * nch) / 4;
                f32x4 acc0 = {0.f, 0.f, 0.f, 0.f}, acc1 = {0.f, 0.f, 0.f, 0.f};
                auto chunk = [&](int b, float (&av)[4], float (&bv)[4]) {
#pragma unroll
                    for (int c = 0; c < 4; ++c) {
                        av[c] = li < A1 ? dzs[(b + c) * A1 + li] : 0.0f;
                        bv[c] = hs[(b + c) * 17 + li];
                    }
                };
                if constexpr (S::BF) {
#pragma unroll 2
                    for (int ch = ch0; ch < ch1; ch += 2) {
                        const int b = ch * kTile + 4 * lq;
                        float av0[4], bv0[4], av1[4] = {0.f, 0.f, 0.f, 0.f}, bv1[4] = {0.f, 0.f, 0.f, 0.f};
                        chunk(b, av0, bv0);
                        if (ch + 1 < ch1) chunk(b + kTile, av1, bv1);
                        acc0 = mfma_bf16_pair(f4(av0), f4(av1), f4(bv0), f4(bv1), acc0);
                    }
                } else {
    #pragma unroll 2
                for (int ch = ch0; ch < ch1; ++ch) {
                    const int b = ch * kTile + 4 * lq;
                    float av[4], bv[4];
                    chunk(b, av, bv);
                    acc0 = mfma4(av[0], bv[0], acc0);
                    acc1 = mfma4(av[1], bv[1], acc1);
                    acc0 = mfma4(av[2], bv[2], acc0);
                    acc1 = mfma4(av[3], bv[3], acc1);
                }
                }
                const f32x4 acc = acc0 + acc1;
#pragma unroll
                for (int r = 0; r < 4; ++r) partC[wave * 256 + (lq * 4 + r) * kTile + li] = acc[r];
                __syncthreads();
                const int a = tid >> 4, i = tid & 15;
                float hv[1] = {tid < nout ? ((partC[tid] + partC[256 + tid]) + partC[512 + tid]) + partC[768 + tid]
                                          : 0.0f};
                bool ok[1] = {tid < nout && n0 + i < H2};
                if (xchg) bwd_exchange<1>(bx, xseq, hv, ok);
                if (ok[0]) {
                    G[L.head_row(a) + n0 + i] = hv[0];
                    sq = hv[0] * hv[0];
                }
            } else {
                for (int u = tid; u < nout * 16; u += 256) {
                    const int o = u >> 4, j = u & 15;
                    const int a = o >> 4, i = o & 15;
                    float s = 0.0f;
                    for (int b = j; b < Bp; b += 16) s = fmaf(dzs[b * A1 + a], hs[b * 17 + i], s);
                    partC[u] = s;
                }
                __syncthreads();
                float hv[4];
                bool ok[4];
#pragma unroll
                for (int j = 0; j < 4; ++j) {
                    const int o = tid + 256 * j;
                    float s = 0.0f;
                    if (o < nout)
#pragma unroll
                        for (int m = 0; m < 16; ++m) s += partC[o * 16 + m];
                    hv[j] = s;
                    ok[j] = o < nout && n0 + (o & 15) < H2;
                }
                if (xchg) bwd_exchange<4>(bx, xseq, hv, ok);
#pragma unroll
                for (int j = 0; j < 4; ++j) {
                    const int o = tid + 256 * j, a = o >> 4, i = o & 15;
                    if (ok[j]) {
                        G[L.head_row(a) + n0 + i] = hv[j];
                        sq += hv[j] * hv[j];
                        if (a == A) sqv += hv[j] * hv[j];
                        else sqp += hv[j] * hv[j];
                    }
                }
            }
            if (A1 <= kTile) {
                block_sumsq_store(sq, sumsq + sh.nT + sh.ncb + nb, sbuf);
                if constexpr (FUSED) store_head_split(sbuf + 256, A, ff.headsq, (kstep * (sh.ncb + 1) + nb) * 2);
            } else {
                store_head_sums(sq, sqp, sqv, sumsq + sh.nT + sh.ncb + nb, FUSED ? ff.headsq : nullptr,
                                (kstep * (sh.ncb + 1) + nb) * 2, sbuf);
            }
        } else {
            for (int u = tid; u < A1 * 16; u += 256) {
                const int a = u >> 4, j = u & 15;
                float s = 0.0f;
                for (int b = j; b < Bp; b += 16) s += dzs[b * A1 + a];
                partC[u] = s;
            }
            __syncthreads();
            float sqb = 0.0f;
            float bv[1] = {0.0f};
            bool ok[1] = {tid < A1};
            if (tid < A1)
#pragma unroll
                for (int m = 0; m < 16; ++m) bv[0] += partC[tid * 16 + m];
            if (xchg) bwd_exchange<1>(bx, xseq, bv, ok);
            if (ok[0]) {
                G[L.head_bias(tid)] = bv[0];
                sqb = bv[0] * bv[0];
            }
            block_sumsq_store(sqb, sumsq + sh.nT + 2 * sh.ncb, sbuf);
            if constexpr (FUSED) store_head_split(sbuf, A, ff.headsq, (kstep * (sh.ncb + 1) + sh.ncb) * 2);
        }
        GS_STAMP_END(1)
        if constexpr (FUSED) GS_SPAN_END(1, kstep)
    }
}

template <class S, bool FUSED>
__global__ __launch_bounds__(256) void k_bwd(const float *__restrict__ P, Layout Lrt, int Brt,
                                             const float *__restrict__ x, const float *__restrict__ h1,
                                             const float *__restrict__ h2, const float *__restrict__ dz,
                                             float *__restrict__ G, float *__restrict__ part1,
                                             float *__restrict__ sumsq, const int32_t *__restrict__ stop,
                                             const float *__restrict__ zpart, FusedFwd ff, LossArgs la,
                                             const uint16_t *__restrict__ h2mask, BwdXchg bx)
{
    bwd_body<S, FUSED, true, true>(P, Lrt, Brt, x, h1, h2, dz, G, part1, sumsq, stop, zpart, ff, la, h2mask, bx);
}

struct BwdTail {
    const float *h2;
    float *G, *part1, *sumsq;
    double *mpart;
    float *headsq;
    const int64_t *step_base;
    LossArgs la;
};
template <class S, bool BASE>
__global__ __launch_bounds__(256) void k_bwd_chain(const float *__restrict__ P, const float *__restrict__ h1,
                                                   const uint16_t *__restrict__ h2mask,
                                                   const float *__restrict__ zpart, const float *__restrict__ fields,
                                                   const float *__restrict__ x, int fstride, int k_local, BwdTail t)
{
    static_assert(S::Bc > 0 && S::H1c > 0, "chain entry: compile-time shapes only");
    FusedFwd ff{};
    ff.fa = reinterpret_cast<const int32_t *>(fields);
    ff.folp = fields + fstride, ff.fov = fields + 2 * (int64_t)fstride;
    ff.fadv = fields + 3 * (int64_t)fstride, ff.fret = fields + 4 * (int64_t)fstride;
    ff.mpart = t.mpart, ff.headsq = t.headsq, ff.step_base = t.step_base, ff.k_local = k_local;
    bwd_body<S, true, false, BASE>(P, Layout{}, S::Bc, x, h1, t.h2, nullptr, t.G, t.part1, t.sumsq, nullptr, zpart, ff,
                                   t.la, h2mask, BwdXchg{});
}


template <class S, int NRB, int NQ>
__global__ __launch_bounds__(256) void k_clip_adam(float *__restrict__ Pm, Layout Lrt, float *__restrict__ G,
                                                   float *__restrict__ M, float *__restrict__ V,
                                                   const float *__restrict__ part1, const float *__restrict__ sumsq,
                                                   AdamArgs aa, float *__restrict__ metrics,
                                                   const int32_t *__restrict__ stop)
{
    if (stop && *stop) {
        if (metrics && blockIdx.x == 0 && threadIdx.x == 0) {
            float *m = metrics + (aa.step_base ? *aa.step_base : 0) * GS_NUM_METRICS;
            m[GS_M_SKIPPED] = 1.0f;
            m[GS_M_KL_STOP] = 1.0f;
        }
        return;
    }
    GS_STAMP_BEGIN(3)
    const int64_t kb = aa.step_base ? *aa.step_base : 0;
    if (metrics) metrics += kb * GS_NUM_METRICS;
    __shared__ double sred[2 * 272];
    __shared__ float s_coef;
    const Layout L = S::lay(Lrt);
    const int tid = threadIdx.x;
    const int64_t n1 = (int64_t)L.H1 * (L.D + 1);
    const int64_t base = (int64_t)blockIdx.x * 1024;
    extern __shared__ float stage[];
    double ss = 0.0;
    float gv[4], mv[4], vv[4], pv[4];
    const int64_t p0 = base + 4 * tid;
    auto pidx = [&](int i) -> int64_t { return NRB > 0 ? p0 + i : base + i * 256 + tid; };
    if constexpr (NRB > 0) {
        const bool full = p0 + 3 < L.P;
        if (full) {
            const float4 g4 = p0 >= L.oW2 ? *reinterpret_cast<const float4 *>(G + p0) : make_float4(0.f, 0.f, 0.f, 0.f);
            const float4 m4 = *reinterpret_cast<const float4 *>(M + p0);
            const float4 v4 = *reinterpret_cast<const float4 *>(V + p0);
            const float4 q4 = *reinterpret_cast<const float4 *>(Pm + p0);
            gv[0] = g4.x, gv[1] = g4.y, gv[2] = g4.z, gv[3] = g4.w;
            mv[0] = m4.x, mv[1] = m4.y, mv[2] = m4.z, mv[3] = m4.w;
            vv[0] = v4.x, vv[1] = v4.y, vv[2] = v4.z, vv[3] = v4.w;
            pv[0] = q4.x, pv[1] = q4.y, pv[2] = q4.z, pv[3] = q4.w;
        } else {
#pragma unroll
            for (int i = 0; i < 4; ++i) {
                const int64_t p = p0 + i;
                const bool ok = p < L.P;
                gv[i] = ok && p >= L.oW2 ? G[p] : 0.0f;
                mv[i] = ok ? M[p] : 0.0f;
                vv[i] = ok ? V[p] : 0.0f;
                pv[i] = ok ? Pm[p] : 0.0f;
            }
        }
        constexpr int NS = 2;
        float sl[NS];
#pragma unroll
        for (int j = 0; j < NS; ++j) sl[j] = tid + 256 * j < aa.n_slots ? sumsq[tid + 256 * j] : 0.0f;
        float4 t[NQ][NRB];
#pragma unroll
        for (int j = 0; j < NQ; ++j) {
            const int64_t q = tid + 256 * j;
#pragma unroll
            for (int rb = 0; rb < NRB; ++rb)
                t[j][rb] = 4 * q < n1 ? *reinterpret_cast<const float4 *>(part1 + (int64_t)rb * n1 + 4 * q)
                                      : make_float4(0.f, 0.f, 0.f, 0.f);
        }
#pragma unroll
        for (int j = 0; j < NS; ++j)
            if (tid + 256 * j < aa.n_slots) stage[tid + 256 * j] = sl[j];
        float *w1s = stage + round4(aa.n_slots);
        float4 gsum[NQ];
#pragma unroll
        for (int j = 0; j < NQ; ++j) {
            const int64_t q = tid + 256 * j;
            float4 g = make_float4(0.f, 0.f, 0.f, 0.f);
#pragma unroll
            for (int rb = 0; rb < NRB; ++rb) {
                g.x += t[j][rb].x;
                g.y += t[j][rb].y;
                g.z += t[j][rb].z;
                g.w += t[j][rb].w;
            }
            gsum[j] = g;
            if (4 * q < n1) *reinterpret_cast<float4 *>(w1s + 4 * q) = g;
        }
        __syncthreads();
        GS_STAMP(0)
        if (p0 < L.oW2) {
#pragma unroll
            for (int i = 0; i < 4; ++i) gv[i] = w1s[part1_index(L, p0 + i)];
        }
        for (int s0 = tid; s0 < aa.n_slots; s0 += 256) ss += (double)stage[s0];
#pragma unroll
        for (int j = 0; j < NQ; ++j)
            if (4 * (tid + 256 * j) < n1) {
                const float4 g = gsum[j];
                ss += (double)g.x * (double)g.x;
                ss += (double)g.y * (double)g.y;
                ss += (double)g.z * (double)g.z;
                ss += (double)g.w * (double)g.w;
            }
    } else {
#pragma unroll
        for (int j = 0; j < 4; ++j) {
            const int64_t p = pidx(j);
            const bool ok = p < L.P;
            float g = 0.0f;
            if (ok) {
                if (aa.nrb > 0 && p < L.oW2) {
                    if (!aa.stage_lds) {
                        const int64_t u = part1_index(L, p);
#pragma unroll 4
                        for (int rb = 0; rb < aa.nrb; ++rb) g += part1[(int64_t)rb * n1 + u];
                    }
                } else {
                    g = G[p];
                }
            }
            gv[j] = g;
            mv[j] = ok ? M[p] : 0.0f;
            vv[j] = ok ? V[p] : 0.0f;
            pv[j] = ok ? Pm[p] : 0.0f;
        }
        const int64_t npart = (int64_t)aa.nrb * n1;
        if (aa.stage_lds) {
            copy_to_lds(stage, sumsq, aa.n_slots);
            const int off = round4(aa.n_slots);
            if (npart > 0) copy_to_lds(stage + off, part1, (int)npart);
            __syncthreads();
            GS_STAMP(0)
            if (aa.nrb > 0 && base < L.oW2) {
#pragma unroll
                for (int j = 0; j < 4; ++j) {
                    const int64_t p = pidx(j);
                    if (p < L.oW2) {
                        const int64_t u = part1_index(L, p);
                        float g = 0.0f;
                        for (int rb = 0; rb < aa.nrb; ++rb) g += stage[off + rb * n1 + u];
                        gv[j] = g;
                    }
                }
            }
            for (int s0 = tid; s0 < aa.n_slots; s0 += 256) ss += (double)stage[s0];
            for (int64_t u = tid; u < n1 && aa.nrb > 0; u += 256) {
                float g = 0.0f;
                for (int rb = 0; rb < aa.nrb; ++rb) g += stage[off + rb * n1 + u];
                ss += (double)g * (double)g;
            }
        } else {
            GS_STAMP(0)
            for (int s0 = tid; s0 < aa.n_slots; s0 += 256) ss += (double)sumsq[s0];
            for (int64_t u = tid; u < n1 && aa.nrb > 0; u += 256) {
                float g = 0.0f;
                for (int rb = 0; rb < aa.nrb; ++rb) g += part1[(int64_t)rb * n1 + u];
                ss += (double)g * (double)g;
            }
        }
    }
    GS_STAMP(1)
    double tt[1] = {ss};
    block_reduce<1>(tt, sred);
    GS_STAMP(2)
    if (tid == 0) {
        const double tot = tt[0];
        const float total = (float)sqrt(tot) * aa.grad_scale;
        s_coef = clip_coef(total, aa);
        if (blockIdx.x == 0 && metrics) metrics[GS_M_GRAD_NORM] = total;
        if (blockIdx.x == 0 && aa.normsq) aa.normsq[kb] = tot * (double)aa.grad_scale * (double)aa.grad_scale;
    }
    __syncthreads();
    const float coef = s_coef * aa.grad_scale;
    const float neg_step = aa.sched ? aa.sched[2 * (aa.sched_idx + kb)] : aa.neg_step_size;
    const float bc2s = aa.sched ? aa.sched[2 * (aa.sched_idx + kb) + 1] : aa.inv_bc2_sqrt;
    float go[4], mo[4], vo[4], po[4];
#pragma unroll
    for (int j = 0; j < 4; ++j) {
        float m = mv[j], v = vv[j], p = pv[j];
        go[j] = adam_param(gv[j], coef, m, v, p, aa, neg_step, bc2s);
        mo[j] = m;
        vo[j] = v;
        po[j] = p;
    }
    if (NRB > 0 && p0 + 3 < L.P) {
        *reinterpret_cast<float4 *>(G + p0) = make_float4(go[0], go[1], go[2], go[3]);
        *reinterpret_cast<float4 *>(Pm + p0) = make_float4(po[0], po[1], po[2], po[3]);
        *reinterpret_cast<float4 *>(M + p0) = make_float4(mo[0], mo[1], mo[2], mo[3]);
        *reinterpret_cast<float4 *>(V + p0) = make_float4(vo[0], vo[1], vo[2], vo[3]);
    } else {
#pragma unroll
        for (int j = 0; j < 4; ++j) {
            const int64_t p = pidx(j);
            if (p >= L.P) break;
            G[p] = go[j];
            Pm[p] = po[j];
            M[p] = mo[j];
            V[p] = vo[j];
        }
    }
    GS_STAMP_END(3)
}

__global__ __launch_bounds__(256) void k_sumsq_flat(const float *__restrict__ G, int64_t n, float *__restrict__ out)
{
    __shared__ float sbuf[272];
    float s = 0.0f;
    for (int64_t i = (int64_t)blockIdx.x * 256 + threadIdx.x; i < n; i += (int64_t)gridDim.x * 256) s += G[i] * G[i];
    block_sumsq_store(s, out + blockIdx.x, sbuf);
}

__global__ __launch_bounds__(256) void k_reduce_part1(const float *__restrict__ part1, Layout L, int nrb,
                                                      float *__restrict__ G, const int32_t *__restrict__ stop)
{
    if (stop && *stop) return;
    const int64_t p = (int64_t)blockIdx.x * 256 + threadIdx.x;
    if (p >= L.oW2) return;
    const int64_t n1 = (int64_t)L.H1 * (L.D + 1);
    const int64_t u = part1_index(L, p);
    float g = 0.0f;
    for (int rb = 0; rb < nrb; ++rb) g += part1[(int64_t)rb * n1 + u];
    G[p] = g;
}

template <class F>
static int with_shape(const Layout &L, int64_t B, F &&f)
{
    if (L.D == 4 && L.H1 == 256 && L.H2 == 256 && L.A == 2) {
        if (B == 256) return f(ShapeC<4, 256, 256, 2, 256>{});
        return f(ShapeC<4, 256, 256, 2, 0>{});
    }
    if (L.D == 8 && L.H1 == 128 && L.H2 == 128 && L.A == 4) {
        if (B == 64) return f(ShapeC<8, 128, 128, 4, 64>{});
        return f(ShapeC<8, 128, 128, 4, 0>{});
    }
    if (L.A <= 4) return f(ShapeR<4>{});
    return f(ShapeR<kMaxActions>{});
}

int rows_b(const Layout &L, int64_t B)
{
    int rb = kRowsB;
    with_shape(L, B, [&](auto sh) {
        rb = decltype(sh)::RB;
        return GS_OK;
    });
    return rb;
}

int set_lds_limit(const void *fn, size_t bytes)
{
    static std::mutex mu;
    static std::unordered_map<const void *, size_t> done;
    if (bytes <= 65536) return GS_OK;
    std::lock_guard<std::mutex> lk(mu);
    auto it = done.find(fn);
    if (it != done.end() && it->second >= bytes) return GS_OK;
    GS_HIP(hipFuncSetAttribute(fn, hipFuncAttributeMaxDynamicSharedMemorySize, (int)bytes));
    done[fn] = bytes;
    return GS_OK;
}

template <class Sh>
constexpr bool chain_shape() { return Sh::AEX > 0 && Sh::H1c > 0 && Sh::Bc > 0; }

template <class Sh>
constexpr bool bf16_shape()
{
    if constexpr (Sh::AEX == 0 || Sh::H1c == 0 || Sh::Bc == 0) {
        return false;
    } else {
        constexpr Layout Lc = Sh::lay(Layout{});
        return Lc.A + 1 <= 5 && Lc.H2 % 64 == 0;
    }
}

bool has_bf16_chain(const Layout &L, int64_t B)
{
    bool ok = false;
    with_shape(L, B, [&](auto sh) {
        ok = bf16_shape<decltype(sh)>();
        return GS_OK;
    });
    return ok && has_fused(L, B);
}

int prepare_kernels(const Layout &L, int64_t B)
{
    if (has_bf16_chain(L, B)) {
        const int rc = with_shape(L, B, [&](auto sh) {
            using Sh = decltype(sh);
            if constexpr (bf16_shape<Sh>())
                return set_lds_limit((const void *)k_bwd<Bf16Shape<Sh>, true>, bwd_lds_bytes(L, B));
            return GS_OK;
        });
        if (rc) return rc;
    }
    int rc = with_shape(L, B, [&](auto sh) {
        return set_lds_limit((const void *)k_bwd<decltype(sh), false>, bwd_lds_bytes(L, B));
    });
    if (rc) return rc;
    if (has_fused(L, B)) {
        rc = with_shape(L, B, [&](auto sh) {
            using Sh = decltype(sh);
            const size_t lds = bwd_lds_bytes(L, B);
            int r = set_lds_limit((const void *)k_bwd<Sh, true>, lds);
            if constexpr (chain_shape<Sh>()) {
                if (!r) r = set_lds_limit((const void *)k_bwd_chain<Sh, false>, lds);
                if (!r) r = set_lds_limit((const void *)k_bwd_chain<Sh, true>, lds);
                if constexpr (bf16_shape<Sh>()) {
                    if (!r) r = set_lds_limit((const void *)k_bwd_chain<Bf16Shape<Sh>, false>, lds);
                    if (!r) r = set_lds_limit((const void *)k_bwd_chain<Bf16Shape<Sh>, true>, lds);
                }
            }
            return r;
        });
        if (rc) return rc;
    }
    rc = with_shape(L, 0, [&](auto sh) {
        return set_lds_limit((const void *)k_fwd_hidden<decltype(sh), false>, fwd_lds_bytes(L));
    });
    if (rc) return rc;
    if (!has_fused(L, B)) return GS_OK;
    GS_REQUIRE(fwd_lds_bytes(L) <= 65536, "fused forward: %zu bytes of LDS exceed the default limit", fwd_lds_bytes(L));
    return GS_OK;
}

int launch_heads_act(const float *P, const Layout &L, const float *zpart, int64_t rows, int mode, uint64_t seed,
                     uint64_t counter, int64_t *actions, float *logp, float *value, hipStream_t s,
                     const uint64_t *clock)
{
    const dim3 grid((unsigned)((rows + 255) / 256));
    return with_shape(L, 0, [&](auto sh) {
        hipLaunchKernelGGL(k_heads_act<decltype(sh)>, grid, dim3(256), 0, s, P, L, zpart, rows, mode, seed, counter,
                           actions, logp, value, clock);
        GS_LAUNCH_CHECK("k_heads_act");
        return GS_OK;
    });
}

int launch_loss(const float *P, const Layout &L, int64_t B, const Workspace &ws, const LossArgs &la, float *metrics,
                int32_t *stop, hipStream_t s)
{
    return with_shape(L, B, [&](auto sh) {
        hipLaunchKernelGGL(k_loss<decltype(sh)>, dim3(1), dim3(256), 0, s, P, L, ws.zpart, (int)B, ws.f_act,
                           ws.f_olp, ws.f_ov, ws.f_adv, ws.f_ret, la, ws.dz, metrics, stop);
        GS_LAUNCH_CHECK("k_loss");
        return GS_OK;
    });
}

bool bwd_xchg_coresident(int64_t nblk, size_t lds_bytes, int colocated);

bool bwd_xchg_fits(const Layout &L, int64_t B, int colocated)
{
    const BwdShape sh = BwdShape::make(L, (int)B, rows_b(L, B));
    const int64_t nblk = sh.nA + sh.nB + sh.nC;
    return nblk <= kBwdXMaxWG && kTile * (L.D + 1) <= kBwdXSlot && (L.A + 1) * kTile <= kBwdXSlot &&
           bwd_xchg_coresident(nblk, bwd_lds_bytes(L, B), colocated);
}

bool bwd_xchg_coresident(int64_t nblk, size_t lds_bytes, int colocated)
{
    if (colocated <= 1) return true;
    int dev = 0, ncu = 0;
    if (hipGetDevice(&dev) != hipSuccess ||
        hipDeviceGetAttribute(&ncu, hipDeviceAttributeMultiprocessorCount, dev) != hipSuccess)
        return false;
    int64_t per_cu = (int64_t)(160 * 1024) / (int64_t)(lds_bytes > 0 ? lds_bytes : 1);
    if (per_cu > 4) per_cu = 4;
    return (int64_t)(colocated - 1) * nblk < (int64_t)ncu * per_cu;
}

int launch_bwd(const float *P, const Layout &L, int64_t B, const Workspace &ws, float *G, const int32_t *stop,
               hipStream_t s, const FusedFwd *ff, const LossArgs *la, const BwdXchg *bxp)
{
    const BwdShape sh0 = BwdShape::make(L, (int)B, rows_b(L, B));
    const unsigned nblk = (unsigned)(sh0.nA + sh0.nB + sh0.nC);
    const size_t lds = bwd_lds_bytes(L, B);
    BwdXchg bx{};
    if (bxp && bxp->world > 1) {
        GS_REQUIRE(bwd_xchg_fits(L, B), "k_bwd exchange: %u workgroups or their output slots exceed the limits",
                   nblk);
        bx = *bxp;
    }
    GS_REQUIRE(!ff || !stop, "the fused chain takes no stop flag (it runs only without a KL early stop)");
    GS_REQUIRE(!ff || la, "fused backward: no loss arguments");
    const bool lean = ff && bx.world <= 1;
    BwdTail t{};
    int64_t fstride = 0;
    if (lean) {
        fstride = ff->folp - reinterpret_cast<const float *>(ff->fa);
        GS_REQUIRE(fstride > 0 && fstride < ((int64_t)1 << 29) && ff->fov == ff->folp + fstride &&
                       ff->fadv == ff->fov + fstride && ff->fret == ff->fadv + fstride,
                   "fused backward: the per-update field arrays are not at one stride");
        t.h2 = ws.h2, t.G = G, t.part1 = ws.part1, t.sumsq = ws.sumsq;
        t.mpart = ff->mpart, t.headsq = ff->headsq, t.step_base = ff->step_base, t.la = *la;
    }
    return with_shape(L, B, [&](auto sh) {
        using Sh = decltype(sh);
        auto chain = [&](auto shape) -> int {
            using S = decltype(shape);
            const float *fields = reinterpret_cast<const float *>(ff->fa);
            const void *fn = ff->step_base ? (const void *)k_bwd_chain<S, true> : (const void *)k_bwd_chain<S, false>;
            int rc = set_lds_limit(fn, lds);
            if (rc) return rc;
            if (ff->step_base)
                hipLaunchKernelGGL((k_bwd_chain<S, true>), dim3(nblk), dim3(256), lds, s, P, ws.h1, ws.h2mask, ws.zpart,
                                   fields, ws.x, (int)fstride, ff->k_local, t);
            else
                hipLaunchKernelGGL((k_bwd_chain<S, false>), dim3(nblk), dim3(256), lds, s, P, ws.h1, ws.h2mask,
                                   ws.zpart, fields, ws.x, (int)fstride, ff->k_local, t);
            GS_LAUNCH_CHECK("k_bwd_chain");
            return GS_OK;
        };
        if (ff && la->bf16) {
            if constexpr (bf16_shape<Sh>()) {
                if (lean) return chain(Bf16Shape<Sh>{});
                int rc = set_lds_limit((const void *)k_bwd<Bf16Shape<Sh>, true>, lds);
                if (rc) return rc;
                hipLaunchKernelGGL((k_bwd<Bf16Shape<Sh>, true>), dim3(nblk), dim3(256), lds, s, P, L, (int)B, ws.x,
                                   ws.h1, ws.h2, ws.dz, G, ws.part1, ws.sumsq, stop, ws.zpart, *ff, *la, ws.h2mask, bx);
                GS_LAUNCH_CHECK("k_bwd<bf16>");
                return GS_OK;
            } else {
                GS_REQUIRE(false, "precision bf16: no bf16 instantiation of the MLP chain for this shape");
            }
        }
        if (lean) {
            if constexpr (chain_shape<Sh>()) {
                return chain(sh);
            } else {
                GS_REQUIRE(false, "fused backward: no compile-time instantiation for this shape");
            }
        }
        if (ff) {
            int rc = set_lds_limit((const void *)k_bwd<Sh, true>, lds);
            if (rc) return rc;
            hipLaunchKernelGGL((k_bwd<Sh, true>), dim3(nblk), dim3(256), lds, s, P, L, (int)B, ws.x, ws.h1, ws.h2,
                               ws.dz, G, ws.part1, ws.sumsq, stop, ws.zpart, *ff, *la, ws.h2mask, bx);
        } else {
            int rc = set_lds_limit((const void *)k_bwd<Sh, false>, lds);
            if (rc) return rc;
            hipLaunchKernelGGL((k_bwd<Sh, false>), dim3(nblk), dim3(256), lds, s, P, L, (int)B, ws.x, ws.h1, ws.h2,
                               ws.dz, G, ws.part1, ws.sumsq, stop, (const float *)nullptr, FusedFwd{}, LossArgs{},
                               ws.h2mask, bx);
        }
        GS_LAUNCH_CHECK("k_bwd");
        return GS_OK;
    });
}

__global__ __launch_bounds__(256) void k_component_norms(Layout L, const float *__restrict__ G,
                                                         const float *__restrict__ part1,
                                                         const float *__restrict__ sumsq, int n_slots, int nrb,
                                                         float gscale, const int64_t *__restrict__ step_base,
                                                         float *__restrict__ metrics,
                                                         const int32_t *__restrict__ stop)
{
    if (stop && *stop) return;
    __shared__ double sred[2 * 272];
    const int tid = threadIdx.x;
    const int64_t n1 = (int64_t)L.H1 * (L.D + 1);
    double tt[1] = {0.0};
    for (int s0 = tid; s0 < n_slots; s0 += 256) tt[0] += (double)sumsq[s0];
    for (int64_t u = tid; u < n1 && nrb > 0; u += 256) {
        float g = 0.0f;
        for (int rb = 0; rb < nrb; ++rb) g += part1[(int64_t)rb * n1 + u];
        tt[0] += (double)g * (double)g;
    }
    block_reduce<1>(tt, sred);
    double hq[2] = {0.0, 0.0};
    const int nhg = (L.A + 1) * (L.H2 + 1);
    for (int u = tid; u < nhg; u += 256) {
        bool val;
        const double g = (double)G[head_grad_offset(L, u, &val)];
        hq[val ? 1 : 0] += g * g;
    }
    store_component_norms(hq, tt[0], gscale, metrics + (step_base ? *step_base : 0) * GS_NUM_METRICS, sred);
}

int launch_clip_adam(float *P, const Layout &L, float *G, float *M, float *V, const float *part1,
                     const float *sumsq, const AdamArgs &aa_in, float *metrics, const int32_t *stop, hipStream_t s,
                     bool comp_norms)
{
    AdamArgs aa = aa_in;
    if (metrics && comp_norms) {
        hipLaunchKernelGGL(k_component_norms, dim3(1), dim3(256), 0, s, L, G, part1, sumsq, aa.n_slots, aa.nrb,
                           aa.grad_scale, aa.step_base, metrics, stop);
        GS_LAUNCH_CHECK("k_component_norms");
    }
    const size_t stage = sizeof(float) * (round4(aa.n_slots) + (size_t)aa.nrb * L.H1 * (L.D + 1));
    aa.stage_lds = stage <= 65536 ? 1 : 0;
    const unsigned nblk = (unsigned)((L.P + 1023) / 1024);
    return with_shape(L, 0, [&](auto sh) {
        const int64_t n1 = (int64_t)L.H1 * (L.D + 1);
        const bool al = (((uintptr_t)P | (uintptr_t)G | (uintptr_t)M | (uintptr_t)V | (uintptr_t)part1) & 15) == 0;
        const int nq = (int)((n1 / 4 + 255) / 256);
        const bool vec = aa.stage_lds && n1 % 4 == 0 && L.oW2 % 4 == 0 && al && aa.n_slots <= 512 && nq <= 2;
        using Sh = decltype(sh);
        const void *fn = nullptr;
        if (vec && aa.nrb == 8) fn = nq == 2 ? (const void *)k_clip_adam<Sh, 8, 2> : (const void *)k_clip_adam<Sh, 8, 1>;
        if (vec && aa.nrb == 4) fn = nq == 2 ? (const void *)k_clip_adam<Sh, 4, 2> : (const void *)k_clip_adam<Sh, 4, 1>;
        if (vec && aa.nrb == 2) fn = nq == 2 ? (const void *)k_clip_adam<Sh, 2, 2> : (const void *)k_clip_adam<Sh, 2, 1>;
        if (fn) {
            void *args[] = {&P, (void *)&L, &G, &M, &V, &part1, &sumsq, &aa, &metrics, &stop};
            GS_HIP(hipLaunchKernel(fn, dim3(nblk), dim3(256), args, stage, s));
        } else {
            hipLaunchKernelGGL((k_clip_adam<Sh, 0, 0>), dim3(nblk), dim3(256), aa.stage_lds ? stage : 0, s, P, L, G,
                               M, V, part1, sumsq, aa, metrics, stop);
        }
        GS_LAUNCH_CHECK("k_clip_adam");
        return GS_OK;
    });
}

template <class S>
__global__ __launch_bounds__(256) void k_gather_all(const int32_t *__restrict__ idx, int Brt, const float *__restrict__ obs,
                                                    const int64_t *__restrict__ actions,
                                                    const float *__restrict__ logprobs, const float *__restrict__ values,
                                                    const float *__restrict__ advantages,
                                                    const float *__restrict__ returns, int T, int N, int D,
                                                    int normalize, FusedFwd ff, float *__restrict__ metrics,
                                                    const float *__restrict__ adv_stats)
{
    __shared__ double sred[2 * (256 + 16)];
    const int B = S::batch(Brt);
    const int64_t k = blockIdx.x;
    const int tid = threadIdx.x;
    constexpr int kMaxRows = 4;
    float adv[kMaxRows];
    bool mine[kMaxRows];
    double m1[1] = {0.0};
#pragma unroll
    for (int j = 0; j < kMaxRows; ++j) {
        const int r = tid + 256 * j;
        adv[j] = 0.0f;
        mine[j] = false;
        if (r < B) {
            const int si = idx[k * B + r];
            const int64_t o = k * B + r;
            if (si < 0) {
                for (int d = 0; d < D; ++d) const_cast<float *>(ff.xg)[o * D + d] = 0.0f;
                const_cast<int32_t *>(ff.fa)[o] = -1;
                const_cast<float *>(ff.folp)[o] = 0.0f;
                const_cast<float *>(ff.fov)[o] = 0.0f;
                const_cast<float *>(ff.fret)[o] = 0.0f;
                continue;
            }
            const int src = sample_row(si, T, N);
            for (int d = 0; d < D; ++d) const_cast<float *>(ff.xg)[o * D + d] = obs[(int64_t)src * D + d];
            const_cast<int32_t *>(ff.fa)[o] = (int32_t)actions[src];
            const_cast<float *>(ff.folp)[o] = logprobs[src];
            const_cast<float *>(ff.fov)[o] = values[src];
            const_cast<float *>(ff.fret)[o] = returns[src];
            adv[j] = advantages[src];
            mine[j] = true;
            m1[0] += (double)adv[j];
        }
    }
    if (normalize && adv_stats) {
        const float meanf = adv_stats[2 * k], stdf = adv_stats[2 * k + 1];
#pragma unroll
        for (int j = 0; j < kMaxRows; ++j)
            if (tid + 256 * j < B)
                const_cast<float *>(ff.fadv)[k * B + tid + 256 * j] = mine[j] ? (adv[j] - meanf) / (stdf + 1e-8f) : 0.0f;
        return;
    }
    if (!normalize) {
#pragma unroll
        for (int j = 0; j < kMaxRows; ++j)
            if (tid + 256 * j < B) const_cast<float *>(ff.fadv)[k * B + tid + 256 * j] = adv[j];
        if (tid == 0) {
            metrics[k * GS_NUM_METRICS + GS_M_ADV_NORM_MEAN] = 0.0f;
            metrics[k * GS_NUM_METRICS + GS_M_ADV_NORM_STD] = 0.0f;
        }
        return;
    }
    block_reduce<1>(m1, sred);
    const double mean = m1[0] / (double)B;
    double q[1] = {0.0};
#pragma unroll
    for (int j = 0; j < kMaxRows; ++j)
        if (tid + 256 * j < B) {
            const double dv = (double)adv[j] - mean;
            q[0] += dv * dv;
        }
    block_reduce<1>(q, sred);
    const float meanf = (float)mean;
    const float stdf = (float)sqrt(q[0] / (double)(B - 1));
    double st[2] = {0.0, 0.0};
#pragma unroll
    for (int j = 0; j < kMaxRows; ++j)
        if (tid + 256 * j < B) {
            const float a = (adv[j] - meanf) / (stdf + 1e-8f);
            const_cast<float *>(ff.fadv)[k * B + tid + 256 * j] = a;
            st[0] += (double)a;
            st[1] += (double)a * (double)a;
        }
    block_reduce<2>(st, sred);
    if (tid == 0) {
        const double Bd = (double)B;
        metrics[k * GS_NUM_METRICS + GS_M_ADV_NORM_MEAN] = (float)(st[0] / Bd);
        metrics[k * GS_NUM_METRICS + GS_M_ADV_NORM_STD] =
            (float)sqrt(fmax(0.0, (st[1] - st[0] * st[0] / Bd) / (Bd - 1.0)));
    }
}

__global__ __launch_bounds__(256) void k_global_adv_sums(const int32_t *__restrict__ idx, int B,
                                                         const float *__restrict__ advantages, int T, int N,
                                                         double *__restrict__ sums)
{
    __shared__ double sred[2 * (256 + 16)];
    const int64_t k = blockIdx.x;
    double st[2] = {0.0, 0.0};
    for (int r = threadIdx.x; r < B; r += 256) {
        const int si = idx[k * B + r];
        if (si < 0) continue;
        const double a = (double)advantages[sample_row(si, T, N)];
        st[0] += a;
        st[1] += a * a;
    }
    block_reduce<2>(st, sred);
    if (threadIdx.x == 0) {
        sums[2 * k] = st[0];
        sums[2 * k + 1] = st[1];
    }
}

__global__ __launch_bounds__(256) void k_global_adv_stats(const double *__restrict__ sums, int64_t n, int Bg,
                                                          float *__restrict__ stats)
{
    const int64_t k = (int64_t)blockIdx.x * 256 + threadIdx.x;
    if (k >= n) return;
    const double Bd = (double)Bg, s1 = sums[2 * k], s2 = sums[2 * k + 1];
    const double mean = s1 / Bd;
    stats[2 * k] = (float)mean;
    stats[2 * k + 1] = (float)sqrt(fmax(0.0, (s2 - s1 * mean) / (Bd - 1.0)));
}

__global__ __launch_bounds__(256) void k_global_records(const double *__restrict__ sums, int64_t n, LossArgs la,
                                                        float *__restrict__ metrics)
{
    const int64_t k = (int64_t)blockIdx.x * 256 + threadIdx.x;
    if (k >= n) return;
    float *rec = metrics + k * GS_NUM_METRICS;
    if (rec[GS_M_UNEVALUATED] != 0.0f) return;
    float tmp[GS_NUM_METRICS];
    write_metrics(sums + k * kNumSums, (double)la.batch_rows, la, tmp, true);
    const int cols[] = {GS_M_LOSS, GS_M_POLICY_LOSS, GS_M_VALUE_LOSS, GS_M_ENTROPY, GS_M_CLIP_FRAC,
                        GS_M_CLIP_FRAC_VF, GS_M_EXPLAINED_VAR, GS_M_KL, GS_M_APPROX_KL, GS_M_ADV_NORM_MEAN,
                        GS_M_ADV_NORM_STD};
#pragma unroll
    for (int c : cols) rec[c] = tmp[c];
}

int launch_global_adv_sums(const int32_t *idx, int64_t n, int64_t B, const float *adv, int64_t T, int64_t N,
                           double *sums, hipStream_t s)
{
    hipLaunchKernelGGL(k_global_adv_sums, dim3((unsigned)n), dim3(256), 0, s, idx, (int)B, adv, (int)T, (int)N, sums);
    GS_LAUNCH_CHECK("k_global_adv_sums");
    return GS_OK;
}

int launch_global_adv_stats(const double *sums, int64_t n, int64_t Bg, float *stats, hipStream_t s)
{
    hipLaunchKernelGGL(k_global_adv_stats, dim3((unsigned)((n + 255) / 256)), dim3(256), 0, s, sums, n, (int)Bg, stats);
    GS_LAUNCH_CHECK("k_global_adv_stats");
    return GS_OK;
}

int launch_global_records(const double *sums, int64_t n, const LossArgs &la, float *metrics, hipStream_t s)
{
    hipLaunchKernelGGL(k_global_records, dim3((unsigned)((n + 255) / 256)), dim3(256), 0, s, sums, n, la, metrics);
    GS_LAUNCH_CHECK("k_global_records");
    return GS_OK;
}

__global__ __launch_bounds__(256) void k_metrics_all(const double *__restrict__ mpart, int nrb, int64_t n, int B,
                                                     LossArgs la, float *__restrict__ metrics,
                                                     const float *__restrict__ headsq, int nhw,
                                                     const double *__restrict__ normsq)
{
    const int64_t k = (int64_t)blockIdx.x * 256 + threadIdx.x;
    if (k >= n) return;
    double t[kNumSums];
#pragma unroll
    for (int q = 0; q < kNumSums; ++q) t[q] = 0.0;
    for (int rb = 0; rb < nrb; ++rb)
#pragma unroll
        for (int q = 0; q < kNumSums; ++q) t[q] += mpart[(k * nrb + rb) * kNumSums + q];
    float *rec = metrics + k * GS_NUM_METRICS;
    write_metrics(t, (double)la.batch_rows, la, rec, la.sums_out != nullptr);
    if (la.sums_out)
#pragma unroll
        for (int q = 0; q < kNumSums; ++q) la.sums_out[k * kNumSums + q] = t[q];
    (void)B;
    if (headsq) {
        double hq[2] = {0.0, 0.0};
        for (int w = 0; w < nhw; ++w) {
            hq[0] += (double)headsq[(k * nhw + w) * 2];
            hq[1] += (double)headsq[(k * nhw + w) * 2 + 1];
        }
        rec[GS_M_GN_POLICY_HEAD] = (float)sqrt(hq[0]);
        rec[GS_M_GN_VALUE_HEAD] = (float)sqrt(hq[1]);
        rec[GS_M_GN_BACKBONE] = (float)sqrt(fmax(0.0, normsq[k] - hq[0] - hq[1]));
        rec[GS_M_GN_MLP] = 0.0f;
    }
}

constexpr int kActRows = 16;
__host__ __device__ inline int act_part_stride(const Layout &L) { return 2 * (2 + (L.H1 > L.H2 ? L.H1 : L.H2)); }

__global__ __launch_bounds__(256) void k_mlp_act_stats(const float *__restrict__ P, Layout L,
                                                       const float *__restrict__ obs, const int32_t *__restrict__ idx,
                                                       int T, int N, int R, double *__restrict__ part,
                                                       const int64_t *__restrict__ step_base)
// ... 390 lines not shown
```

### gymnasium-solver_amd/csrc/gs_ppo.hip

```cpp
#include <math.h>
#include <stdlib.h>
#include <string.h>
#include <mutex>
#include <unordered_map>
#include <vector>

#include "gs_comm_internal.h"
#include "gs_cartpole_env.h"
#include "gs_acrobot_env.h"
#include "gs_mountaincar_env.h"
#include "gs_bandit_env.h"

namespace gs {

static size_t align256(size_t b) { return (b + 255) & ~size_t(255); }

Workspace carve_workspace(void *base, const Layout &L, int64_t B)
{
    Workspace w{};
    char *p = (char *)base;
    size_t off = 0;
    auto take = [&](size_t nfloats) {
        float *r = p ? (float *)(p + off) : nullptr;
        off += align256(nfloats * sizeof(float));
// ... 43 lines not shown
    g.logprobs = ro.logprobs;
    g.values = ro.values;
    g.advantages = ro.advantages;
    g.returns = ro.returns;
    g.f_act = ws.f_act;
    g.f_olp = ws.f_olp;
    g.f_ov = ws.f_ov;
    g.f_adv = ws.f_adv;
    g.f_ret = ws.f_ret;
    return g;
}

}

using namespace gs;

static bool one_layer(const gs_mlp_dims &d) { return d.hidden2 == 0; }
#define GS_REFUSE_ONE_LAYER(dims, what) \
    GS_REQUIRE(!one_layer(dims), what ": not available for a policy with one hidden layer (hidden2 == 0)")

extern "C" int64_t gs_mlp_param_count(gs_mlp_dims dims)
{
    if (one_layer(dims)) return Layout1::make(dims.obs_dim, dims.hidden1, dims.n_actions).P;
    return layout_of(dims).P;
}

extern "C" size_t gs_policy_scratch_bytes(gs_mlp_dims dims, int64_t N)
{
    if (one_layer(dims)) return 256;
    const Layout L = layout_of(dims);
    return align256((size_t)n_col_blocks(L.H2) * N * (L.A + 1) * sizeof(float));
}

extern "C" int gs_policy_act(const float *params, gs_mlp_dims dims, const float *obs, int64_t N, int mode,
                             uint64_t rng_seed, uint64_t rng_counter, int64_t *actions, float *logp, float *value,
                             float *obs_store, void *scratch, const uint64_t *clock, void *stream)
{
    if (one_layer(dims)) {
        GS_REQUIRE(actions && logp && value, "gs_policy_act: null buffer");
        return mlp1_policy_act(params, dims, obs, N, mode, rng_seed, rng_counter, actions, logp, value, obs_store,
                               clock, (hipStream_t)stream);
    }
    int rc = check_dims(dims);
    if (rc) return rc;
    GS_REQUIRE(N > 0, "gs_policy_act: N must be > 0");
    GS_REQUIRE(mode >= 0 && mode <= 2, "gs_policy_act: mode %d not in {0,1,2}", mode);
    GS_REQUIRE(params && obs && actions && logp && value && scratch, "gs_policy_act: null buffer");
    GS_REQUIRE(((uintptr_t)scratch & 15) == 0, "gs_policy_act: scratch must be 16-byte aligned");
    const Layout L = layout_of(dims);
    hipStream_t s = (hipStream_t)stream;
    float *zpart = (float *)scratch;
    rc = launch_fwd_hidden(params, L, obs, nullptr, 1, N, N, nullptr, nullptr, nullptr, zpart, obs_store, nullptr,
                           nullptr, s);
    if (rc) return rc;
    return launch_heads_act(params, L, zpart, N, mode, rng_seed, rng_counter, actions, logp, value, s, clock);
}

extern "C" int gs_rollout_synth_supported(gs_mlp_dims dims, int *supported)
{
    GS_REQUIRE(supported, "gs_rollout_synth_supported: null output");
    if (one_layer(dims)) {
        *supported = 0;
        return mlp1_check_dims(dims);
    }
    int rc = check_dims(dims);
    if (rc) return rc;
    *supported = rollout_synth_fits(layout_of(dims)) ? 1 : 0;
    return GS_OK;
}

extern "C" int gs_rollout_synth(const float *params, gs_mlp_dims dims, int64_t N, int64_t T, int mode,
                                uint64_t rng_seed, uint64_t rng_counter0, int32_t *env_state, float *env_ep_ret,
                                float *env_obs, int32_t episode_len, int32_t truncate_every, float reward,
                                uint64_t env_seed, int64_t env_offset, uint64_t env_step0, int32_t *ep_done_count,
                                float *ep_ret_sum, float *ep_len_sum, float *obs_rows, int64_t *action_rows,
                                float *logp_rows, float *value_rows, float *reward_rows, uint8_t *done_rows,
                                uint8_t *timeout_rows, void *stream)
{
    GS_REFUSE_ONE_LAYER(dims, "gs_rollout_synth");
    int rc = check_dims(dims);
    if (rc) return rc;
    GS_REQUIRE(N > 0 && T >= 0 && T < (int64_t)1 << 31, "gs_rollout_synth: bad N / T");
    GS_REQUIRE(mode >= 0 && mode <= 2, "gs_rollout_synth: mode %d not in {0,1,2}", mode);
    GS_REQUIRE(episode_len > 0, "gs_rollout_synth: episode_len must be > 0");
    GS_REQUIRE(params && env_state && env_ep_ret && env_obs && obs_rows && action_rows && logp_rows && value_rows &&
                   reward_rows && done_rows && timeout_rows,
               "gs_rollout_synth: null buffer");
    if (T == 0) return GS_OK;
    SynthEnvArgs ev{env_state, env_ep_ret, env_obs, ep_done_count, ep_ret_sum, ep_len_sum, episode_len,
                    truncate_every, reward, env_seed, env_step0, env_offset};
    RolloutRows rw{obs_rows, action_rows, logp_rows, value_rows, reward_rows, done_rows, timeout_rows};
    return launch_rollout_synth(params, layout_of(dims), N, (int)T, mode, rng_seed, rng_counter0, ev, rw,
                                (hipStream_t)stream);
}

extern "C" int gs_rollout_env_supported(gs_mlp_dims dims, int kind, int *supported)
{
    GS_REQUIRE(supported, "gs_rollout_env_supported: null output");
    if (one_layer(dims)) {
        *supported = 0;
        return mlp1_check_dims(dims);
    }
    int rc = check_dims(dims);
    if (rc) return rc;
    const Layout L = layout_of(dims);
    *supported = (kind == GS_ENV_SYNTHETIC ? rollout_synth_fits(L) : rollout_env_fits(L, kind)) ? 1 : 0;
    return GS_OK;
}

static int check_rollout_entry(const char *who, gs_mlp_dims dims, int64_t N, int64_t T, int mode,
                               const float *params, const EnvArgs &ev, const RolloutRows &rw)
{
    GS_REQUIRE(!one_layer(dims), "%s: not available for a policy with one hidden layer (hidden2 == 0)", who);
    int rc = check_dims(dims);
    if (rc) return rc;
    GS_REQUIRE(N > 0 && T >= 0 && T < (int64_t)1 << 31, "%s: bad N / T", who);
    GS_REQUIRE(mode >= 0 && mode <= 2, "%s: mode %d not in {0,1,2}", who, mode);
    GS_REQUIRE(ev.max_steps > 0, "%s: max_steps must be > 0", who);
    GS_REQUIRE(params && ev.meta && ev.ep_ret && ev.obs && rw.obs && rw.actions && rw.logp && rw.value &&
                   rw.reward && rw.done && rw.timeout,
               "%s: null buffer", who);
    return GS_OK;
}

template <class E>
static int rollout_entry(const char *who, const float *params, gs_mlp_dims dims, int64_t N, int64_t T, int mode,
                         uint64_t rng_seed, uint64_t rng_counter0, const typename E::Args &ev, const RolloutRows &rw,
                         const char *bad, void *stream)
{
    int rc = check_rollout_entry(who, dims, N, T, mode, params, ev, rw);
    if (rc) return rc;
    GS_REQUIRE(!bad, "%s: %s", who, bad);
    if (T == 0) return GS_OK;
    return launch_rollout<E>(params, layout_of(dims), N, (int)T, mode, rng_seed, rng_counter0, ev, rw,
                             (hipStream_t)stream);
}

extern "C" int gs_rollout_env(const float *params, gs_mlp_dims dims, int64_t N, int64_t T, int mode, uint64_t rng_seed,
                              uint64_t rng_counter0, int kind, double *env_state, int32_t *env_meta,
                              float *env_ep_ret, float *env_obs, int32_t max_steps, uint64_t env_seed,
                              int64_t env_offset, int32_t *ep_done_count, float *ep_ret_sum, float *ep_len_sum,
                              float *obs_rows, int64_t *action_rows, float *logp_rows, float *value_rows,
                              float *reward_rows, uint8_t *done_rows, uint8_t *timeout_rows, void *stream)
{
    GS_REQUIRE(kind != GS_ENV_MOUNTAINCAR,
               "gs_rollout_env: MountainCar takes its count tables and wrappers through gs_rollout_mountaincar");
    GS_REQUIRE(kind != GS_ENV_BANDIT, "gs_rollout_env: the bandit takes its spec through gs_rollout_bandit");
    GS_REQUIRE(kind == GS_ENV_CARTPOLE || kind == GS_ENV_ACROBOT,
               "gs_rollout_env: env kind %d has no dynamics here (the synthetic env: gs_rollout_synth)", kind);
    const DynEnvArgs ev{{env_meta, env_ep_ret, env_obs, ep_done_count, ep_ret_sum, ep_len_sum, max_steps, env_seed,
                         env_offset},
                        env_state};
    const RolloutRows rw{obs_rows, action_rows, logp_rows, value_rows, reward_rows, done_rows, timeout_rows};
    const auto run = kind == GS_ENV_CARTPOLE ? rollout_entry<CartPoleEnv> : rollout_entry<AcrobotEnv>;
    return run("gs_rollout_env", params, dims, N, T, mode, rng_seed, rng_counter0, ev, rw,
               env_state ? nullptr : "null buffer", stream);
}

extern "C" int gs_rollout_mountaincar(const float *params, gs_mlp_dims dims, int64_t N, int64_t T, int mode,
                                      uint64_t rng_seed, uint64_t rng_counter0, double *env_state, int32_t *env_meta,
                                      float *env_ep_ret, float *env_obs, int32_t *env_counts,
                                      gs_mountaincar_wrappers wrappers, int32_t max_steps, uint64_t env_seed,
                                      int64_t env_offset, int32_t *ep_done_count, float *ep_ret_sum,
                                      float *ep_len_sum, float *obs_rows, int64_t *action_rows, float *logp_rows,
                                      float *value_rows, float *reward_rows, uint8_t *done_rows,
                                      uint8_t *timeout_rows, void *stream)
{
    const MountainCarEnv::Args ev{{{env_meta, env_ep_ret, env_obs, ep_done_count, ep_ret_sum, ep_len_sum, max_steps,
                                    env_seed, env_offset},
                                   env_state},
                                  env_counts,
                                  wrappers};
    const RolloutRows rw{obs_rows, action_rows, logp_rows, value_rows, reward_rows, done_rows, timeout_rows};
    const char *bad = env_state ? mountaincar_wrappers_error(wrappers, env_counts) : "null buffer";
    return rollout_entry<MountainCarEnv>("gs_rollout_mountaincar", params, dims, N, T, mode, rng_seed, rng_counter0,
                                         ev, rw, bad, stream);
}

extern "C" int gs_rollout_cartpole_shaped(const float *params, gs_mlp_dims dims, int64_t N, int64_t T, int mode,
                                          uint64_t rng_seed, uint64_t rng_counter0, double *env_state,
                                          double *env_prev_phi, int32_t *env_meta, float *env_ep_ret, float *env_obs,
                                          gs_cartpole_wrappers wrappers, int32_t max_steps, uint64_t env_seed,
                                          int64_t env_offset, int32_t *ep_done_count, float *ep_ret_sum,
                                          float *ep_len_sum, float *obs_rows, int64_t *action_rows, float *logp_rows,
                                          float *value_rows, float *reward_rows, uint8_t *done_rows,
                                          uint8_t *timeout_rows, void *stream)
{
    const CartPoleShapedEnv::Args ev{{{env_meta, env_ep_ret, env_obs, ep_done_count, ep_ret_sum, ep_len_sum,
                                       max_steps, env_seed, env_offset},
                                      env_state},
                                     env_prev_phi,
                                     wrappers};
    const RolloutRows rw{obs_rows, action_rows, logp_rows, value_rows, reward_rows, done_rows, timeout_rows};
    return rollout_entry<CartPoleShapedEnv>("gs_rollout_cartpole_shaped", params, dims, N, T, mode, rng_seed,
                                            rng_counter0, ev, rw,
                                            env_state && env_prev_phi ? nullptr : "null buffer", stream);
}

extern "C" int gs_rollout_bandit(const float *params, gs_mlp_dims dims, int64_t N, int64_t T, int mode,
                                 uint64_t rng_seed, uint64_t rng_counter0, int32_t *env_meta, float *env_ep_ret,
                                 float *env_obs, gs_bandit_spec spec, int32_t max_steps, uint64_t env_seed,
                                 int64_t env_offset, int32_t *ep_done_count, float *ep_ret_sum, float *ep_len_sum,
                                 float *obs_rows, int64_t *action_rows, float *logp_rows, float *value_rows,
                                 float *reward_rows, uint8_t *done_rows, uint8_t *timeout_rows, void *stream)
{
    const BanditEnv::Args ev{{env_meta, env_ep_ret, env_obs, ep_done_count, ep_ret_sum, ep_len_sum, max_steps,
                              env_seed, env_offset},
                             spec};
    const RolloutRows rw{obs_rows, action_rows, logp_rows, value_rows, reward_rows, done_rows, timeout_rows};
    const char *bad = bandit_spec_error(spec);
    if (!bad && T > 0 && dims.n_actions != spec.n_arms) bad = "the policy's actions are not the spec's n_arms";
    return rollout_entry<BanditEnv>("gs_rollout_bandit", params, dims, N, T, mode, rng_seed, rng_counter0, ev, rw,
                                    bad, stream);
}

extern "C" int gs_policy_value(const float *params, gs_mlp_dims dims, const float *obs, int64_t N, float *value,
                               void *scratch, void *stream)
{
    if (one_layer(dims))
        return mlp1_policy_act(params, dims, obs, N, 0, 0, 0, nullptr, nullptr, value, nullptr, nullptr,
                               (hipStream_t)stream);
    int rc = check_dims(dims);
    if (rc) return rc;
    GS_REQUIRE(N > 0 && params && obs && value && scratch, "gs_policy_value: bad argument");
    GS_REQUIRE(((uintptr_t)scratch & 15) == 0, "gs_policy_value: scratch must be 16-byte aligned");
    const Layout L = layout_of(dims);
    hipStream_t s = (hipStream_t)stream;
    float *zpart = (float *)scratch;
    rc = launch_fwd_hidden(params, L, obs, nullptr, 1, N, N, nullptr, nullptr, nullptr, zpart, nullptr, nullptr,
                           nullptr, s);
    if (rc) return rc;
    return launch_heads_act(params, L, zpart, N, 0, 0, 0, nullptr, nullptr, value, s);
}

extern "C" size_t gs_ppo_workspace_bytes(gs_mlp_dims dims, int64_t batch)
{
    if (one_layer(dims)) return mlp1_check_dims(dims) ? 0 : 256;
    return carve_workspace(nullptr, layout_of(dims), batch).bytes;
}

namespace {

constexpr int64_t kChunk = 512;
constexpr int64_t kWholeCapture = 16384;
constexpr int64_t kNumSumsHost = 14;

struct FusedWs {
    float *xg, *folp, *fov, *fadv, *fret;
    int32_t *fa;
    double *mpart;
    float *headsq;
    double *normsq;
    float *p1, *m1, *v1;
    uint32_t *act;
    size_t bytes;
};

FusedWs carve_fused(void *base, const Layout &L, int64_t B, int64_t n)
{
    const size_t step = carve_workspace(nullptr, L, B).bytes;
    char *p = (char *)base;
    size_t off = step;
    auto take = [&](size_t bytes) {
        void *q = p ? (void *)(p + off) : nullptr;
        off += align256(bytes);
        return q;
    };
    FusedWs f{};
    f.xg = (float *)take(sizeof(float) * (size_t)(n * B * L.D));
    f.fa = (int32_t *)take(sizeof(int32_t) * (size_t)(n * B));
    f.folp = (float *)take(sizeof(float) * (size_t)(n * B));
    f.fov = (float *)take(sizeof(float) * (size_t)(n * B));
    f.fadv = (float *)take(sizeof(float) * (size_t)(n * B));
    f.fret = (float *)take(sizeof(float) * (size_t)(n * B));
    f.mpart = (double *)take(sizeof(double) * (size_t)(n * (B / kTile) * 14));
    f.headsq = (float *)take(sizeof(float) * (size_t)(n * ((L.H2 + kTile - 1) / kTile + 1) * 2));
    f.normsq = (double *)take(sizeof(double) * (size_t)n);
    f.p1 = (float *)take(sizeof(float) * (size_t)L.P);
    f.m1 = (float *)take(sizeof(float) * (size_t)L.P);
    f.v1 = (float *)take(sizeof(float) * (size_t)L.P);
    f.act = (uint32_t *)take(sizeof(uint32_t) * (size_t)n * (size_t)(B / kTile) * (size_t)n_col_blocks(L.H2) * kActRec);
    f.bytes = off;
    return f;
}

}

extern "C" size_t gs_ppo_update_workspace_bytes(gs_mlp_dims dims, int64_t batch, int64_t n_minibatches)
{
    if (one_layer(dims)) return mlp1_check_dims(dims) || batch < 1 || n_minibatches < 0 ? 0 : 256;
    if (check_dims(dims) || batch < 1 || n_minibatches < 0) return 0;
    const Layout L = layout_of(dims);
    if (!has_fused(L, batch)) return carve_workspace(nullptr, L, batch).bytes;
    return carve_fused(nullptr, L, batch, n_minibatches).bytes;
}

namespace {

struct StepArgs {
    LossArgs la;
    AdamArgs aa;
    bool sum_exchange;
    bool act_stats;
};

StepArgs make_step_args(const gs_ppo_hparams &hp, const Layout &L, int64_t B, int64_t t,
                        const gs_ppo_global *glob = nullptr)
{
    StepArgs a{};
    a.la.batch_rows = (int)(glob ? glob->batch_global : B);
    a.la.inv_batch = 1.0f / (float)a.la.batch_rows;
    if (glob) {
        a.la.adv_stats = glob->adv_stats;
        a.la.sums_out = glob->metric_sums;
        a.sum_exchange = true;
    }
    a.la.clip_lo = (float)(1.0 - (double)hp.clip_range);
    a.la.clip_hi = (float)(1.0 + (double)hp.clip_range);
    a.la.clip_vf = hp.clip_range_vf;
    a.la.vf_coef = hp.vf_coef;
    a.la.ent_coef = hp.ent_coef;
    a.la.target_kl = hp.target_kl;
    a.la.normalize = hp.normalize_adv;
    a.la.bf16 = (hp.flags & GS_HP_BF16) ? 1 : 0;
    a.act_stats = (hp.flags & GS_HP_ACT_STATS) && !glob;
    const double b1 = hp.adam_beta1, b2 = hp.adam_beta2;
    a.aa.max_norm = hp.max_grad_norm;
    a.aa.one_minus_b1 = (float)(1.0 - b1);
    a.aa.b2 = (float)b2;
    a.aa.one_minus_b2 = (float)(1.0 - b2);
    const double bc1 = 1.0 - pow(b1, (double)t);
    const double bc2 = 1.0 - pow(b2, (double)t);
    a.aa.neg_step_size = (float)(-(double)hp.lr / bc1);
    a.aa.bc2_sqrt = (float)sqrt(bc2);
    a.aa.inv_bc2_sqrt = (float)(1.0 / sqrt(bc2));
    a.aa.eps = hp.adam_eps;
    a.aa.grad_scale = 1.0f;
    a.aa.n_slots = n_sumsq_slots(L);
    a.aa.nrb = (int)((B + rows_b(L, B) - 1) / rows_b(L, B));
    return a;
}

int exchange_and_adam(float *P, float *G, float *M, float *V, const Layout &L, const StepArgs &sa, float *metrics,
                      int32_t *stop, const Workspace &ws, gs_comm *comm, hipStream_t s, const FusedFwd *ff = nullptr)
{
    int world = 1, n_slots = 0;
    int rc = comm_grad_exchange(comm, G, L.P, Part1Fold{ws.part1, sa.aa.nrb, L}, ws.sumsq, &n_slots, stop, s,
                                &world);
    if (rc) return rc;
    AdamArgs aa = sa.aa;
    aa.n_slots = n_slots;
    aa.nrb = 0;
    aa.grad_scale = sa.sum_exchange ? 1.0f : 1.0f / (float)world;
    if (ff && (rc = launch_head_sq(L, G, aa.grad_scale, *ff, s))) return rc;
    return launch_clip_adam(P, L, G, M, V, nullptr, ws.sumsq, aa, metrics, stop, s, ff == nullptr);
}

int enqueue_step(float *P, float *G, float *M, float *V, const Layout &L, const StepArgs &sa,
                 const gs_rollout_view &ro, const int32_t *idx, int64_t B, float *metrics, int32_t *stop,
                 const Workspace &ws, gs_comm *comm, hipStream_t s)
{
    RowGather rg = gather_of(ro, ws);
    rg.step_base = sa.la.step_base;
    int rc = launch_fwd_hidden(P, L, ro.obs, idx, ro.T, ro.N, B, ws.x, ws.h1, ws.h2, ws.zpart, nullptr, stop, &rg, s,
                               ws.h2mask);
    if (rc) return rc;
    if (sa.act_stats && ((rc = launch_act_stats(P, L, ro.obs, idx, ro.T, ro.N, B, ws.act_parts, s, sa.la.step_base)) ||
                         (rc = launch_act_parts_record(L, B, ws.act_parts, stop, metrics, sa.la.step_base, s))))
        return rc;
    rc = launch_loss(P, L, B, ws, sa.la, metrics, stop, s);
    if (rc) return rc;
    if (sa.la.kl_part) {
        int world = 1;
        if (comm && (rc = comm_allreduce_sum(comm, sa.la.kl_part, 1, s, &world))) return rc;
        rc = launch_kl_decide(sa.la.kl_part, sa.la.target_kl, stop, metrics, sa.la.step_base, s);
        if (rc) return rc;
    }
    rc = launch_bwd(P, L, B, ws, G, stop, s);
    if (rc) return rc;
    if (!comm) return launch_clip_adam(P, L, G, M, V, ws.part1, ws.sumsq, sa.aa, metrics, stop, s);
    return exchange_and_adam(P, G, M, V, L, sa, metrics, stop, ws, comm, s);
}

bool bwd_exchange_of(gs_comm *comm, const Layout &L, int64_t B, BwdXchg *bx, bool sum_exchange = false)
{
    if (!(comm && xgmi_bwd_args(comm, bx) && bwd_xchg_fits(L, B, comm->colocated))) return false;
    if (sum_exchange) bx->scale = 1.0f;
    return true;
}

int enqueue_step_fused(float *P, float *G, float *M, float *V, const Layout &L, const StepArgs &sa, int64_t B,
                       const FusedFwd &ff, float *metrics, int32_t *stop, const Workspace &ws, gs_comm *comm,
                       hipStream_t s)
{
    BwdXchg bx;
    const bool inbwd = bwd_exchange_of(comm, L, B, &bx, sa.sum_exchange);
    int rc = launch_fwd_fused(P, L, B, ff, sa.la, ws, stop, s);
    if (rc) return rc;
    rc = launch_bwd(P, L, B, ws, G, stop, s, &ff, &sa.la, inbwd ? &bx : nullptr);
    if (rc) return rc;
    if (!comm || inbwd) return launch_clip_adam(P, L, G, M, V, ws.part1, ws.sumsq, sa.aa, metrics, stop, s, false);
    return exchange_and_adam(P, G, M, V, L, sa, metrics, stop, ws, comm, s, &ff);
}

bool lagged_enabled()
{
    const char *e = getenv("GS_LAGGED_ADAM");
    return !(e && e[0] == '0');
}

struct ParamSet {
    float *P, *M, *V;
};

AdamArgs exchanged_adam_args(const AdamArgs &aa_in, const gs_comm *comm, bool sum_exchange = false)
{
    AdamArgs aa = aa_in;
    aa.n_slots = comm_sumsq_slots(comm);
    aa.nrb = 0;
    aa.grad_scale = sum_exchange ? 1.0f : 1.0f / (float)comm->nranks;
    return aa;
}

int enqueue_step_lagged(const ParamSet (&ps)[2], float *G, const Layout &L, const StepArgs &sa_prev, int64_t B,
                        const FusedFwd &ff, int64_t k, float *metrics, int32_t *stop, const Workspace &ws,
                        gs_comm *comm, hipStream_t s)
{
    const ParamSet &cur = ps[k & 1], &prev = ps[(k & 1) ^ 1];
    BwdXchg bx;
    const bool inbwd = bwd_exchange_of(comm, L, B, &bx, sa_prev.sum_exchange);
    const bool after = comm && !inbwd;
    AdamFwd af{};
    af.Min = prev.M, af.Vin = prev.V, af.G = G, af.part1 = after ? nullptr : ws.part1, af.sumsq = ws.sumsq;
    af.Pout = cur.P, af.Mout = cur.M, af.Vout = cur.V;
    af.metrics = metrics;
    af.aa = after ? exchanged_adam_args(sa_prev.aa, comm, sa_prev.sum_exchange) : sa_prev.aa;
    int rc = launch_fwd_fused(prev.P, L, B, ff, sa_prev.la, ws, stop, s, &af);
    if (rc) return rc;
    rc = launch_bwd(cur.P, L, B, ws, G, stop, s, &ff, &sa_prev.la, inbwd ? &bx : nullptr);
    if (rc || !after) return rc;
    int world = 1, n_slots = 0;
    rc = comm_grad_exchange(comm, G, L.P, Part1Fold{ws.part1, sa_prev.aa.nrb, L}, ws.sumsq, &n_slots, stop, s, &world);
    if (rc) return rc;
    return launch_head_sq(L, G, exchanged_adam_args(sa_prev.aa, comm, sa_prev.sum_exchange).grad_scale, ff, s);
}

int validate_update(const gs_mlp_dims &dims, const gs_rollout_view &ro, int64_t batch, const void *ws)
{
    int rc = check_dims(dims);
    if (rc) return rc;
    GS_REQUIRE(batch >= 2 && batch <= 1024, "batch %lld outside [2, 1024]", (long long)batch);
    GS_REQUIRE(ro.T > 0 && ro.N > 0, "empty rollout");
    GS_REQUIRE(ro.obs && ro.actions && ro.logprobs && ro.values && ro.advantages && ro.returns,
               "rollout view has a null buffer");
    GS_REQUIRE(ws, "null workspace");
    const Layout L = layout_of(dims);
    GS_REQUIRE(bwd_lds_bytes(L, batch) <= 160 * 1024, "batch %lld too large for the LDS budget", (long long)batch);
    GS_REQUIRE(fwd_lds_bytes(L) <= 160 * 1024, "obs_dim x hidden1 too large for the LDS budget");
    GS_REQUIRE(ro.T * ro.N < (int64_t)1 << 31, "rollout larger than 2^31 samples");
    return GS_OK;
}

}

extern "C" int gs_ppo_minibatch_step(float *params, float *grads, float *adam_m, float *adam_v, gs_mlp_dims dims,
                                     gs_ppo_hparams hp, gs_rollout_view ro, const int32_t *idx, int64_t batch,
                                     int64_t adam_step, float *metrics, int32_t *stop_flag, void *workspace,
                                     gs_comm *comm, void *stream)
{
    if (one_layer(dims)) {
        GS_REQUIRE(!comm, "gs_ppo_minibatch_step: no gradient exchange for a policy with one hidden layer");
        GS_REQUIRE(adam_step >= 1, "adam_step is 1-based");
        return mlp1_update(params, grads, adam_m, adam_v, dims, hp, ro, idx, batch, 1, adam_step - 1, metrics,
                           stop_flag, false, (hipStream_t)stream);
    }
    int rc = validate_update(dims, ro, batch, workspace);
    if (rc) return rc;
    GS_REQUIRE(adam_step >= 1, "adam_step is 1-based");
    GS_REQUIRE(params && grads && adam_m && adam_v && idx && metrics, "gs_ppo_minibatch_step: null buffer");
    GS_REQUIRE(!(hp.flags & GS_HP_BF16), "gs_ppo_minibatch_step: precision bf16 is a mode of the fused chain "
                                         "(gs_ppo_update) only; the single-step entries are fp32");
    const Layout L = layout_of(dims);
    const Workspace ws = carve_workspace(workspace, L, batch);
    const StepArgs sa = make_step_args(hp, L, batch, adam_step);
    return enqueue_step(params, grads, adam_m, adam_v, L, sa, ro, idx, batch, metrics, stop_flag, ws, comm,
                        (hipStream_t)stream);
}

extern "C" int gs_mlp_activation_stats(const float *params, gs_mlp_dims dims, gs_rollout_view ro, const int32_t *idx,
                                       int64_t rows, double *part, void *stream)
{
    if (one_layer(dims)) return mlp1_activation_stats(params, dims, ro, idx, rows, part, (hipStream_t)stream);
    int rc = check_dims(dims);
    if (rc) return rc;
    GS_REQUIRE(params && ro.obs && part && rows >= 1, "gs_mlp_activation_stats: null buffer or no rows");
    GS_REQUIRE(idx || rows <= ro.T * ro.N, "gs_mlp_activation_stats: more rows than the rollout holds");
    return launch_act_stats(params, layout_of(dims), ro.obs, idx, ro.T, ro.N, rows, part, (hipStream_t)stream);
}

extern "C" int gs_ppo_loss(const float *params, gs_mlp_dims dims, gs_ppo_hparams hp, gs_rollout_view ro,
                           const int32_t *idx, int64_t batch, float *metrics, void *workspace, void *stream)
{
    if (one_layer(dims))
        return mlp1_update(const_cast<float *>(params), nullptr, nullptr, nullptr, dims, hp, ro, idx, batch, 1, 0,
                           metrics, nullptr, true, (hipStream_t)stream);
    int rc = validate_update(dims, ro, batch, workspace);
    if (rc) return rc;
    GS_REQUIRE(params && idx && metrics, "gs_ppo_loss: null buffer");
    GS_REQUIRE(!(hp.flags & GS_HP_BF16), "gs_ppo_loss: precision bf16 is a mode of the fused chain "
                                         "(gs_ppo_update) only; the single-step entries are fp32");
    const Layout L = layout_of(dims);
    const Workspace ws = carve_workspace(workspace, L, batch);
    const StepArgs sa = make_step_args(hp, L, batch, 1);
    hipStream_t s = (hipStream_t)stream;
    const RowGather rg = gather_of(ro, ws);
    rc = launch_fwd_hidden(params, L, ro.obs, idx, ro.T, ro.N, batch, ws.x, ws.h1, ws.h2, ws.zpart, nullptr,
                           nullptr, &rg, s, ws.h2mask);
    if (rc) return rc;
    return launch_loss(params, L, batch, ws, sa.la, metrics, nullptr, s);
}

extern "C" int gs_ppo_stage(int stage, float *params, float *grads, float *adam_m, float *adam_v, gs_mlp_dims dims,
                            gs_ppo_hparams hp, gs_rollout_view ro, const int32_t *idx, int64_t batch,
                            int64_t adam_step, float *metrics, void *workspace, void *stream)
{
    GS_REFUSE_ONE_LAYER(dims, "gs_ppo_stage");
    int rc = validate_update(dims, ro, batch, workspace);
    if (rc) return rc;
    GS_REQUIRE(stage >= 0 && stage <= 7, "gs_ppo_stage: stage %d not in [0, 7]", stage);
    const Layout L0 = layout_of(dims);
    GS_REQUIRE(!(hp.flags & GS_HP_BF16) || (stage >= 4 && has_bf16_chain(L0, batch)),
               "gs_ppo_stage: precision bf16 runs only on the fused chain's stages (4..7) of a shape with a bf16 "
               "instantiation; stage %d is fp32", stage);
    const Layout L = layout_of(dims);
    const Workspace ws = carve_workspace(workspace, L, batch);
    const StepArgs sa = make_step_args(hp, L, batch, adam_step < 1 ? 1 : adam_step);
    hipStream_t s = (hipStream_t)stream;
    if (stage >= 4) {
        GS_REQUIRE(has_fused(L, batch), "gs_ppo_stage: no fused instantiation for this shape");
        const FusedWs fw = carve_fused(workspace, L, batch, 1);
        FusedFwd ff{};
        ff.xg = fw.xg, ff.fa = fw.fa, ff.folp = fw.folp, ff.fov = fw.fov, ff.fadv = fw.fadv, ff.fret = fw.fret;
        ff.mpart = fw.mpart;
        ff.headsq = fw.headsq;
        ff.dz = ws.dz;
        if (stage == 6)
            return launch_gather_all(L, batch, 1, idx, ro.obs, ro.actions, ro.logprobs, ro.values, ro.advantages,
                                     ro.returns, ro.T, ro.N, hp.normalize_adv, ff, metrics, s);
        if (stage == 4) return launch_fwd_fused(params, L, batch, ff, sa.la, ws, nullptr, s);
        if (stage == 7) {
            GS_REQUIRE(lagged_enabled() && has_lagged(L, batch), "gs_ppo_stage: no lagged optimizer step here");
            AdamFwd af{};
            af.Min = adam_m, af.Vin = adam_v, af.G = grads, af.part1 = ws.part1, af.sumsq = ws.sumsq;
            af.Pout = fw.p1, af.Mout = fw.m1, af.Vout = fw.v1;
            af.metrics = metrics;
            af.aa = sa.aa;
            af.force = 1;
            return launch_fwd_fused(params, L, batch, ff, sa.la, ws, nullptr, s, &af);
        }
        return launch_bwd(params, L, batch, ws, grads, nullptr, s, &ff, &sa.la);
    }
    switch (stage) {
    case 0: {
        const RowGather rg = gather_of(ro, ws);
        return launch_fwd_hidden(params, L, ro.obs, idx, ro.T, ro.N, batch, ws.x, ws.h1, ws.h2, ws.zpart, nullptr,
                                 nullptr, &rg, s, ws.h2mask);
    }
    case 1:
        return launch_loss(params, L, batch, ws, sa.la, metrics, nullptr, s);
    case 2:
        return launch_bwd(params, L, batch, ws, grads, nullptr, s);
    default:
        return launch_clip_adam(params, L, grads, adam_m, adam_v, ws.part1, ws.sumsq, sa.aa, metrics, nullptr, s);
    }
}

namespace {

struct GraphKey {
    const void *p[14];
    int64_t n[6];
    bool operator==(const GraphKey &o) const
    {
        for (int i = 0; i < 14; ++i)
            if (p[i] != o.p[i]) return false;
        for (int i = 0; i < 6; ++i)
            if (n[i] != o.n[i]) return false;
        return true;
    }
};
struct GraphKeyHash {
    size_t operator()(const GraphKey &k) const
    {
        size_t h = 1469598103934665603ull;
        for (int i = 0; i < 14; ++i) h = (h ^ (size_t)k.p[i]) * 1099511628211ull;
        for (int i = 0; i < 6; ++i) h = (h ^ (size_t)k.n[i]) * 1099511628211ull;
        return h;
    }
};
struct GraphEntry {
    hipGraphExec_t exec;
    float *sched;
    int64_t *base;
    int64_t *hbase;
    float *hsched;
    hipEvent_t sched_copied;
    uint32_t hbits[12];
};
std::mutex g_graph_mu;
std::unordered_map<GraphKey, GraphEntry, GraphKeyHash> g_graphs;
int64_t g_graph_captures = 0;

void baked_hparam_bits(const gs_ppo_hparams &hp, uint32_t (&out)[12])
{
    gs_ppo_hparams h = hp;
    h.lr = 0.0f;
    memcpy(out, &h, sizeof(out));
}

}

static int ppo_update(float *params, float *grads, float *adam_m, float *adam_v, gs_mlp_dims dims,
                      gs_ppo_hparams hp, gs_rollout_view ro, const int32_t *idx, int64_t batch,
                      int64_t n_minibatches, int64_t adam_step0, float *metrics, int32_t *stop_flag,
                      void *workspace, size_t workspace_bytes, gs_comm *comm, int use_graph, void *stream,
                      const gs_ppo_global *glob)
{
    if (one_layer(dims)) {
        GS_REQUIRE(!comm, "gs_ppo_update: no gradient exchange for a policy with one hidden layer");
        return mlp1_update(params, grads, adam_m, adam_v, dims, hp, ro, idx, batch, n_minibatches, adam_step0, metrics,
                           stop_flag, false, (hipStream_t)stream);
    }
    int rc = validate_update(dims, ro, batch, workspace);
    if (rc) return rc;
    GS_REQUIRE(n_minibatches >= 0 && adam_step0 >= 0, "bad n_minibatches/adam_step0");
    GS_REQUIRE(params && grads && adam_m && adam_v && idx && metrics, "gs_ppo_update: null buffer");
    if (n_minibatches == 0) return GS_OK;
    const Layout L = layout_of(dims);
    const Workspace ws = carve_workspace(workspace, L, batch);
    auto make_step_args = [&](const gs_ppo_hparams &h, const Layout &Lx, int64_t Bx, int64_t t) {
        StepArgs a = ::make_step_args(h, Lx, Bx, t, glob);
        if (glob && h.target_kl > 0.0f) a.la.kl_part = ws.kl4;
        return a;
    };
    auto at_step = [](StepArgs a, int64_t k) {
        if (a.la.adv_stats) a.la.adv_stats += 2 * k;
        if (a.la.sums_out) a.la.sums_out += kNumSumsHost * k;
        return a;
    };
    hipStream_t s = (hipStream_t)stream;
    const bool fused = has_fused(L, batch) && !(hp.target_kl > 0.0f) &&
                       workspace_bytes >= carve_fused(nullptr, L, batch, n_minibatches).bytes &&
                       (((uintptr_t)params | (uintptr_t)grads | (uintptr_t)adam_m | (uintptr_t)adam_v) & 15) == 0;
    GS_REQUIRE(!(hp.flags & GS_HP_BF16) || (fused && has_bf16_chain(L, batch)),
               "precision bf16: the MLP update's bf16 mode runs on the fused chain of the compile-time shapes "
               "(CartPole 4-256-256-2 / LunarLander 8-128-128-4, B %% 16 == 0, no target_kl)");
    if (fused) stop_flag = nullptr;
    FusedWs fw{};
    FusedFwd ff0{};
    if (fused) {
        fw = carve_fused(workspace, L, batch, n_minibatches);
        ff0.xg = fw.xg, ff0.fa = fw.fa, ff0.folp = fw.folp, ff0.fov = fw.fov, ff0.fadv = fw.fadv, ff0.fret = fw.fret;
        ff0.mpart = fw.mpart;
        ff0.headsq = fw.headsq;
        ff0.normsq = fw.normsq;
        ff0.dz = ws.dz;
        if ((hp.flags & GS_HP_ACT_STATS) && !glob) ff0.act = fw.act;
        rc = launch_gather_all(L, batch, n_minibatches, idx, ro.obs, ro.actions, ro.logprobs, ro.values,
                               ro.advantages, ro.returns, ro.T, ro.N, hp.normalize_adv, ff0, metrics, s,
                               glob ? glob->adv_stats : nullptr);
        if (rc) return rc;
    }
    const bool lagged = fused && lagged_enabled() && has_lagged(L, batch);
    const ParamSet ps[2] = {{params, adam_m, adam_v}, {fw.p1, fw.m1, fw.v1}};
    if (lagged) GS_HIP(hipMemcpyAsync(fw.p1, params, sizeof(float) * (size_t)L.P, hipMemcpyDeviceToDevice, s));
    auto step_ff = [&](int64_t k_local, int64_t slot, const int64_t *base) {
        FusedFwd f = ff0;
        f.k_local = (int)k_local;
        f.step_base = base;
        (void)slot;
        return f;
    };
    auto lag_step = [&](int64_t k, const int64_t *base, const float *sched, hipStream_t st) {
        StepArgs sp = make_step_args(hp, L, batch, adam_step0 + k > 0 ? adam_step0 + k : 1);
        sp.aa.sched = sched;
        sp.aa.normsq = fw.normsq;
        return enqueue_step_lagged(ps, grads, L, sp, batch, step_ff(k, k, base), k, metrics, stop_flag, ws, comm, st);
    };
    auto with_norm = [&](StepArgs a, int64_t k) {
        a.aa.normsq = fw.normsq ? fw.normsq + k : nullptr;
        return a;
    };
    auto finish = [&]() -> int {
        if (!fused) return GS_OK;
        if (lagged) {
            const int64_t k = n_minibatches - 1;
            const ParamSet &q = ps[k & 1];
            StepArgs sl = make_step_args(hp, L, batch, adam_step0 + k + 1);
            sl.aa.normsq = fw.normsq + k;
            BwdXchg bx;
            const bool after = comm && !bwd_exchange_of(comm, L, batch, &bx, sl.sum_exchange);
            int rc2 = after ? launch_clip_adam(q.P, L, grads, q.M, q.V, nullptr, ws.sumsq,
                                              exchanged_adam_args(sl.aa, comm, sl.sum_exchange),
                                              metrics + k * GS_NUM_METRICS,
                                              stop_flag, s, false)
                           : launch_clip_adam(q.P, L, grads, q.M, q.V, ws.part1, ws.sumsq, sl.aa,
                                              metrics + k * GS_NUM_METRICS, stop_flag, s, false);
            if (rc2) return rc2;
            if (k & 1) {
                const size_t nb = sizeof(float) * (size_t)L.P;
                GS_HIP(hipMemcpyAsync(params, q.P, nb, hipMemcpyDeviceToDevice, s));
                GS_HIP(hipMemcpyAsync(adam_m, q.M, nb, hipMemcpyDeviceToDevice, s));
                GS_HIP(hipMemcpyAsync(adam_v, q.V, nb, hipMemcpyDeviceToDevice, s));
            }
        }
        StepArgs sa = make_step_args(hp, L, batch, 1);
        const int rc3 = launch_metrics_all(L, batch, n_minibatches, ff0, sa.la, metrics, s);
        if (rc3 || !ff0.act) return rc3;
        return launch_act_stats_fused(L, batch, n_minibatches, ff0.act, metrics, s);
    };
    if (!use_graph) {
        for (int64_t k = 0; k < n_minibatches; ++k) {
            const StepArgs sa = make_step_args(hp, L, batch, adam_step0 + k + 1);
            rc = lagged  ? lag_step(k, nullptr, nullptr, s)
                 : fused ? enqueue_step_fused(params, grads, adam_m, adam_v, L, with_norm(sa, k), batch,
                                              step_ff(k, k, nullptr), metrics + k * GS_NUM_METRICS, stop_flag, ws,
                                              comm, s)
                         : enqueue_step(params, grads, adam_m, adam_v, L, at_step(sa, k), ro, idx + k * batch, batch,
                                        metrics + k * GS_NUM_METRICS, stop_flag, ws, comm, s);
            if (rc) return rc;
        }
        return finish();
    }
    const int64_t chunk = n_minibatches <= kWholeCapture ? n_minibatches : kChunk;
    const int64_t n_full = n_minibatches / chunk;
    const bool whole = chunk == n_minibatches;
    GraphKey key{};
    const void *ptrs[14] = {params, grads, adam_m, adam_v, ro.obs, ro.actions, ro.logprobs, ro.values,
                            ro.advantages, ro.returns, idx, metrics, glob ? glob->adv_stats : nullptr,
                            glob ? glob->metric_sums : nullptr};
    for (int i = 0; i < 14; ++i) key.p[i] = ptrs[i];
    key.n[0] = batch;
    key.n[1] = n_minibatches;
    key.n[2] = ((int64_t)dims.obs_dim << 48) ^ ((int64_t)dims.hidden1 << 32) ^ ((int64_t)dims.hidden2 << 16) ^ dims.n_actions;
    key.n[3] = (int64_t)(intptr_t)workspace;
    BwdXchg bx_key;
    const bool in_bwd = comm && bwd_exchange_of(comm, L, batch, &bx_key);
    key.n[4] = (int64_t)(intptr_t)stop_flag ^ ((int64_t)(intptr_t)comm << 1) ^ (fused ? 1 : 0) ^
               ((int64_t)lagged << 62) ^ ((int64_t)in_bwd << 61);
    key.n[5] = ro.T * 1000003 + ro.N + (glob ? glob->batch_global << 40 : 0);
    uint32_t hbits[12];
    baked_hparam_bits(hp, hbits);
    std::lock_guard<std::mutex> lk(g_graph_mu);
    auto it = g_graphs.find(key);
    const bool fresh = it == g_graphs.end();
    if (!fresh && memcmp(it->second.hbits, hbits, sizeof(hbits)) != 0) {
        GS_HIP(hipEventSynchronize(it->second.sched_copied));
        GS_HIP(hipStreamSynchronize(s));
        GS_HIP(hipGraphExecDestroy(it->second.exec));
        it->second.exec = nullptr;
    }
    if (fresh || it->second.exec == nullptr) {
        rc = prepare_kernels(L, batch);
        if (rc) return rc;
        GraphEntry ent{};
        if (fresh) {
            GS_HIP(hipMalloc(&ent.sched, sizeof(float) * 2 * (size_t)n_minibatches + 64));
            ent.base = (int64_t *)((char *)ent.sched + sizeof(float) * 2 * (size_t)n_minibatches);
            GS_HIP(hipHostMalloc((void **)&ent.hbase, sizeof(int64_t) * (size_t)(n_full + 1), hipHostMallocDefault));
            for (int64_t r = 0; r <= n_full; ++r) ent.hbase[r] = r * chunk;
            GS_HIP(hipHostMalloc((void **)&ent.hsched, sizeof(float) * 2 * (size_t)n_minibatches,
                                 hipHostMallocDefault));
            GS_HIP(hipEventCreateWithFlags(&ent.sched_copied, hipEventDisableTiming));
        } else {
            ent = it->second;
        }
        memcpy(ent.hbits, hbits, sizeof(hbits));
        hipStream_t cs;
        GS_HIP(hipStreamCreateWithFlags(&cs, hipStreamNonBlocking));
        hipGraph_t g;
        GS_HIP(hipStreamBeginCapture(cs, hipStreamCaptureModeThreadLocal));
        const int64_t *base = whole ? nullptr : ent.base;
        for (int64_t k = 0; k < chunk; ++k) {
            StepArgs sa = make_step_args(hp, L, batch, 1);
            sa.aa.sched = ent.sched;
            sa.aa.sched_idx = (int)k;
            sa.aa.step_base = base;
            sa.la.step_base = base;
            if (lagged) {
                rc = lag_step(k, base, ent.sched, cs);
            } else if (fused) {
                LossArgs la_f = sa.la;
                la_f.step_base = nullptr;
                StepArgs saf = sa;
                saf.la = la_f;
                rc = enqueue_step_fused(params, grads, adam_m, adam_v, L, with_norm(saf, k), batch,
                                        step_ff(k, k, base),
                                        metrics + k * GS_NUM_METRICS, stop_flag, ws, comm, cs);
            } else {
                rc = enqueue_step(params, grads, adam_m, adam_v, L, at_step(sa, k), ro, idx + k * batch, batch,
                                  metrics + k * GS_NUM_METRICS, stop_flag, ws, comm, cs);
            }
            if (rc) {
                hipGraph_t dummy;
                (void)hipStreamEndCapture(cs, &dummy);
                (void)hipStreamDestroy(cs);
                if (!fresh) g_graphs.erase(it);
                (void)hipFree(ent.sched);
                (void)hipHostFree(ent.hbase);
                (void)hipHostFree(ent.hsched);
                (void)hipEventDestroy(ent.sched_copied);
                return rc;
            }
        }
        GS_HIP(hipStreamEndCapture(cs, &g));
        GS_HIP(hipStreamDestroy(cs));
        GS_HIP(hipGraphInstantiate(&ent.exec, g, nullptr, nullptr, 0));
        GS_HIP(hipGraphDestroy(g));
        ++g_graph_captures;
        if (fresh)
            it = g_graphs.emplace(key, ent).first;
        else
            it->second = ent;
    }
    GraphEntry &e = it->second;
    GS_HIP(hipEventSynchronize(e.sched_copied));
    for (int64_t k = 0; k < n_minibatches; ++k) {
        const StepArgs sa = make_step_args(hp, L, batch, adam_step0 + k + 1);
        e.hsched[2 * k] = sa.aa.neg_step_size;
        e.hsched[2 * k + 1] = sa.aa.inv_bc2_sqrt;
    }
    GS_HIP(hipMemcpyAsync(e.sched, e.hsched, sizeof(float) * 2 * (size_t)n_minibatches, hipMemcpyHostToDevice, s));
    GS_HIP(hipEventRecord(e.sched_copied, s));
    for (int64_t r = 0; r < n_full; ++r) {
        GS_HIP(hipMemcpyAsync(it->second.base, it->second.hbase + r, sizeof(int64_t), hipMemcpyHostToDevice, s));
        GS_HIP(hipGraphLaunch(it->second.exec, s));
    }
    for (int64_t k = n_full * chunk; k < n_minibatches; ++k) {
        const StepArgs sa = make_step_args(hp, L, batch, adam_step0 + k + 1);
        rc = lagged  ? lag_step(k, nullptr, nullptr, s)
             : fused ? enqueue_step_fused(params, grads, adam_m, adam_v, L, with_norm(sa, k), batch,
                                          step_ff(k, k, nullptr), metrics + k * GS_NUM_METRICS, stop_flag, ws, comm,
                                          s)
                     : enqueue_step(params, grads, adam_m, adam_v, L, at_step(sa, k), ro, idx + k * batch, batch,
                                  metrics + k * GS_NUM_METRICS, stop_flag, ws, comm, s);
        if (rc) return rc;
    }
    return finish();
}

extern "C" int gs_ppo_update(float *params, float *grads, float *adam_m, float *adam_v, gs_mlp_dims dims,
                             gs_ppo_hparams hp, gs_rollout_view ro, const int32_t *idx, int64_t batch,
                             int64_t n_minibatches, int64_t adam_step0, float *metrics, int32_t *stop_flag,
                             void *workspace, size_t workspace_bytes, gs_comm *comm, int use_graph, void *stream)
{
    return ppo_update(params, grads, adam_m, adam_v, dims, hp, ro, idx, batch, n_minibatches, adam_step0, metrics,
                      stop_flag, workspace, workspace_bytes, comm, use_graph, stream, nullptr);
}

extern "C" int gs_ppo_update_global(float *params, float *grads, float *adam_m, float *adam_v, gs_mlp_dims dims,
                                    gs_ppo_hparams hp, gs_rollout_view ro, const int32_t *idx, int64_t batch,
                                    int64_t n_minibatches, int64_t adam_step0, float *metrics, int32_t *stop_flag,
                                    void *workspace, size_t workspace_bytes, gs_comm *comm, int use_graph,
                                    const gs_ppo_global *glob, void *stream)
{
    GS_REFUSE_ONE_LAYER(dims, "gs_ppo_update_global");
    GS_REQUIRE(glob && glob->batch_global >= 2 && glob->metric_sums, "gs_ppo_update_global: bad global arguments");
    GS_REQUIRE(!hp.normalize_adv || glob->adv_stats, "gs_ppo_update_global: normalize_adv needs adv_stats");
    GS_REQUIRE(glob->batch_global >= batch || !comm, "gs_ppo_update_global: batch_global < local rows");
    return ppo_update(params, grads, adam_m, adam_v, dims, hp, ro, idx, batch, n_minibatches, adam_step0, metrics,
                      stop_flag, workspace, workspace_bytes, comm, use_graph, stream, glob);
}

extern "C" int gs_ppo_global_adv_stats(const int32_t *idx, int64_t n_minibatches, int64_t batch, int64_t batch_global,
                                       const float *advantages, int64_t T, int64_t N, gs_comm *comm, double *sums,
                                       float *adv_stats, void *stream)
{
    GS_REQUIRE(idx && advantages && sums && adv_stats, "gs_ppo_global_adv_stats: null buffer");
    GS_REQUIRE(n_minibatches >= 0 && batch >= 1 && batch <= 1 << 20 && batch_global >= 2 && T > 0 && N > 0,
               "gs_ppo_global_adv_stats: bad sizes");
    if (n_minibatches == 0) return GS_OK;
    hipStream_t s = (hipStream_t)stream;
    int rc = launch_global_adv_sums(idx, n_minibatches, batch, advantages, T, N, sums, s);
    if (rc) return rc;
    if (comm && (rc = gs_comm_allreduce_sum_f64(comm, sums, 2 * n_minibatches, stream))) return rc;
    return launch_global_adv_stats(sums, n_minibatches, batch_global, adv_stats, s);
}

extern "C" int gs_ppo_global_records(const gs_ppo_hparams *hp, int64_t n_minibatches, int64_t batch_global,
                                     gs_comm *comm, double *metric_sums, float *metrics, void *stream)
{
    GS_REQUIRE(hp && metric_sums && metrics && n_minibatches >= 0 && batch_global >= 2,
               "gs_ppo_global_records: bad argument");
    if (n_minibatches == 0) return GS_OK;
    int rc;
    if (comm && (rc = gs_comm_allreduce_sum_f64(comm, metric_sums, kNumSumsHost * n_minibatches, stream))) return rc;
    gs_ppo_global g{batch_global, nullptr, metric_sums};
    const StepArgs sa = make_step_args(*hp, Layout{}, batch_global, 1, &g);
    return launch_global_records(metric_sums, n_minibatches, sa.la, metrics, (hipStream_t)stream);
}

extern "C" int gs_ppo_graph_cache_info(int64_t *n_entries, int64_t *n_captures)
{
    std::lock_guard<std::mutex> lk(g_graph_mu);
    if (n_entries) *n_entries = (int64_t)g_graphs.size();
    if (n_captures) *n_captures = g_graph_captures;
    return GS_OK;
}

extern "C" int gs_ppo_exchange_inside_bwd(gs_comm *comm, gs_mlp_dims dims, int64_t batch, int *inside)
{
    GS_REQUIRE(comm && inside, "gs_ppo_exchange_inside_bwd: null argument");
    GS_REFUSE_ONE_LAYER(dims, "gs_ppo_exchange_inside_bwd");
    int rc = check_dims(dims);
    if (rc) return rc;
    GS_REQUIRE(batch >= 2 && batch <= 1024, "batch %lld outside [2, 1024]", (long long)batch);
    const Layout L = layout_of(dims);
    BwdXchg bx;
    *inside = has_fused(L, batch) && bwd_exchange_of(comm, L, batch, &bx) ? 1 : 0;
    return GS_OK;
}
```

Measured before the change: 980,500 env_steps/s.

## Run fused backward chain kernel with eight waves per workgroup

After: 994,200 env_steps/s (median of 6 runs). 1.4% higher.

```diff
diff --git a/gymnasium-solver_amd/csrc/gs_common.h b/gymnasium-solver_amd/csrc/gs_common.h
--- a/gymnasium-solver_amd/csrc/gs_common.h
+++ b/gymnasium-solver_amd/csrc/gs_common.h
@@ -277,11 +277,12 @@
                      const uint64_t *clock = nullptr);
 int launch_loss(const float *P, const Layout &L, int64_t B, const Workspace &ws, const LossArgs &la, float *metrics,
                 int32_t *stop, hipStream_t s);
-size_t bwd_lds_bytes(const Layout &L, int64_t B);
+size_t bwd_lds_bytes(const Layout &L, int64_t B, int nt = 256);
 int prepare_kernels(const Layout &L, int64_t B);
+int bwd_chain_threads();
 int launch_bwd(const float *P, const Layout &L, int64_t B, const Workspace &ws, float *G, const int32_t *stop,
                hipStream_t s, const FusedFwd *ff = nullptr, const LossArgs *la = nullptr,
-               const BwdXchg *bx = nullptr);
+               const BwdXchg *bx = nullptr, int chain_nt = 0);
 bool bwd_xchg_fits(const Layout &L, int64_t B, int colocated = 1);
 int launch_clip_adam(float *P, const Layout &L, float *G, float *M, float *V, const float *part1,
                      const float *sumsq, const AdamArgs &aa, float *metrics, const int32_t *stop, hipStream_t s,
diff --git a/gymnasium-solver_amd/csrc/gs_mlp.hip b/gymnasium-solver_amd/csrc/gs_mlp.hip
--- a/gymnasium-solver_amd/csrc/gs_mlp.hip
+++ b/gymnasium-solver_amd/csrc/gs_mlp.hip
@@ -1,4 +1,6 @@
 #include <float.h>
+#include <stdlib.h>
+#include <string.h>
 
 #include <mutex>
 #include <type_traits>
@@ -1304,9 +1306,10 @@
     }
 };
 
-size_t bwd_lds_bytes(const Layout &L, int64_t B)
+size_t bwd_lds_bytes(const Layout &L, int64_t B, int nt)
 {
     const int kRowsB = rows_b(L, B);
+    const int64_t wtiles = nt == 512 ? 2048 : 1024;
     const int A1 = L.A + 1;
     const int64_t Bp64 = (B + 63) / 64 * 64, Bp16 = (B + 15) / 16 * 16;
     const int64_t H2p = (L.H2 + 63) / 64 * 64;
@@ -1316,9 +1319,9 @@
                           Bp64 + (fastA ? 0 : 816);
     const int64_t roleB = (regsB ? (int64_t)round4(kRowsB / 16 * 16 * (L.D + 1)) : (int64_t)kRowsB * (H2p + 4)) +
                           kTile * (H2p + 4) + round4(A1 * L.H2) + round4(kRowsB * A1) +
-                          kRowsB * 16 + round4(kRowsB * L.D) + kRowsB * 17 + 1024 +
+                          kRowsB * 16 + round4(kRowsB * L.D) + kRowsB * 17 + wtiles +
                           (int64_t)kRowsB * n_col_blocks(L.H2);
-    const int64_t roleC = Bp16 * 17 + round4((int)Bp16 * A1) + (A1 * 256 > 1024 ? A1 * 256 : 1024) + 2 +
+    const int64_t roleC = Bp16 * 17 + round4((int)Bp16 * A1) + (A1 * 256 > wtiles ? A1 * 256 : wtiles) + 2 +
                           (int64_t)metric_groups_per_wg((int)B / kTile, shp.nC) * kTile * kNumSums * 2;
     int64_t m = roleA;
     if (roleB > m) m = roleB;
@@ -1373,7 +1376,7 @@
     }
 }
 
-template <class S, bool FUSED, bool XCHG, bool BASE>
+template <class S, bool FUSED, bool XCHG, bool BASE, int NT = 256>
 __device__ __forceinline__ void bwd_body(const float *__restrict__ P, const Layout &Lrt, int Brt,
                                          const float *__restrict__ x, const float *__restrict__ h1,
                                          const float *__restrict__ h2, const float *__restrict__ dz,
@@ -1398,8 +1401,13 @@
     const int D = L.D, H1 = L.H1, H2 = L.H2, A = L.A, A1 = A + 1;
     constexpr int kRowsB = S::RB;
     const BwdShape sh = BwdShape::make(L, B, kRowsB);
-    const int tid = threadIdx.x, lane = tid & 63, wave = tid >> 6;
+    const int tid = threadIdx.x, lane = tid & 63;
+    const int wave = NT == 512 ? __builtin_amdgcn_readfirstlane(tid >> 6) : tid >> 6;
     const int li = lane & 15, lq = lane >> 4;
+    static_assert(NT == 256 || NT == 512, "k_bwd: 256 or 512 threads");
+    constexpr bool W8 = NT == 512;
+    static_assert(!W8 || (FUSED && !XCHG && S::H1c > 0 && S::Bc > 0), "eight waves: the chain entry only");
+    const int cw = W8 ? wave & 3 : wave, hi = W8 ? wave >> 2 : 0;
     int bid = (int)blockIdx.x;
     if (bid < sh.nB) bid += sh.nA;
     else if (bid < sh.nB + sh.nA) bid -= sh.nB;
@@ -1411,7 +1419,7 @@
         GS_STAMP_BEGIN_IF(2, bid == 0)
         const int Bp = (B + 63) / 64 * 64;
         const int ld = Bp + 4;
-        const bool fast = A1 <= 5;
+        const bool fast = W8 || A1 <= 5;
         float *dzs = lds;
         float *whs = dzs + round4(B * A1);
         float *dh2T = whs + round4(A1 * 16);
@@ -1423,6 +1431,53 @@
             constexpr int cB = S::Bc, cBp = (cB + 63) / 64 * 64, cncb = (Lc.H2 + kTile - 1) / kTile;
             constexpr int cka = (Lc.H1 / kTile) % 2 == 0 ? 2 : 1, ckw = kTile * cka, cq = ckw / 4;
             constexpr int NMk = (cBp + 255) / 256, NH1 = (cBp * cq + 255) / 256;
+            if constexpr (W8) {
+                if (wave >= 4) {
+                    const int lt = tid - 256;
+                    int mr[NMk];
+                    float4 hr[NH1];
+#pragma unroll
+                    for (int j = 0; j < NMk; ++j) {
+                        const int b = lt + 256 * j;
+                        mr[j] = (int)h2mask[(int64_t)min(b, cB - 1) * cncb + nb];
+                    }
+#ifdef GS_STAMPS
+                    const unsigned long long t_ld0 = __builtin_amdgcn_s_memtime();
+#endif
+#pragma unroll
+                    for (int j = 0; j < NH1; ++j) {
+                        const int u = lt + 256 * j, b = u / cq, c4 = u % cq;
+                        hr[j] = *reinterpret_cast<const float4 *>(h1 + (int64_t)min(b, cB - 1) * Lc.H1 +
+                                                                  min(k0 + 4 * c4, Lc.H1 - 4));
+                    }
+                    const float wh = P[L.head_row(min(lt >> 4, A1 - 1)) + min(n0 + (lt & 15), H2 - 1)];
+                    if (lt < A1 * kTile) whs[lt] = n0 + (lt & 15) < H2 ? wh : 0.0f;
+#pragma unroll
+                    for (int j = 0; j < NMk; ++j)
+                        if (lt + 256 * j < cBp) mkA[lt + 256 * j] = lt + 256 * j < cB ? mr[j] : 0;
+#pragma unroll
+                    for (int j = 0; j < NH1; ++j) {
+                        const int u = lt + 256 * j, b = u / cq, c4 = u % cq;
+                        if (u < cBp * cq) {
+                            const bool ok = b < cB && k0 + 4 * c4 < Lc.H1;
+                            h1T[(4 * c4 + 0) * ld + b] = ok ? hr[j].x : 0.0f;
+                            h1T[(4 * c4 + 1) * ld + b] = ok ? hr[j].y : 0.0f;
+                            h1T[(4 * c4 + 2) * ld + b] = ok ? hr[j].z : 0.0f;
+                            h1T[(4 * c4 + 3) * ld + b] = ok ? hr[j].w : 0.0f;
+                        }
+                    }
+#ifdef GS_STAMPS
+                    if (bid == 0 && lt == 0) {
+                        asm volatile("s_waitcnt vmcnt(0) lgkmcnt(0)" ::: "memory");
+                        atomicAdd(&g_stamp_acc[2][13], t_ld0 - _st_t0);
+                        atomicAdd(&g_stamp_acc[2][14], __builtin_amdgcn_s_memtime() - _st_t0);
+                    }
+#endif
+                } else {
+                    GS_STAMP_ENTRY
+                    loss_rows_lds<S>(P, L, zpart, ff, la, B, kstep, 0, B, dzs, nullptr);
+                }
+            } else {
             int mr[NMk];
             float4 hr[NH1];
             float wh = 0.0f;
@@ -1460,6 +1515,7 @@
                     h1T[(4 * c4 + 2) * ld + b] = ok ? hr[j].z : 0.0f;
                     h1T[(4 * c4 + 3) * ld + b] = ok ? hr[j].w : 0.0f;
                 }
+            }
             }
         } else {
             if constexpr (FUSED)
@@ -1487,7 +1543,7 @@
         __syncthreads();
         GS_STAMP(0)
         const int nch = Bp / kTile;
-        const int ch0 = (wave * nch) / 4, ch1 = ((wave + 1) * nch) / 4;
+        const int ch0 = (cw * nch) / 4, ch1 = ((cw + 1) * nch) / 4;
         const int nt = sh.ka + (!fast && kb == 0 ? 1 : 0);
         if (fast) {
             float w[5];
@@ -1506,6 +1562,49 @@
                     av[c] = (mkA[b + c] >> li) & 1 ? sacc : 0.0f;
                 }
             };
+            if constexpr (W8) {
+                if (hi < nt) {
+                    const float *hb = h1T + (hi * kTile + li) * ld;
+                    const bool dsm = kb == 0 && hi == 0;
+                    f32x4 a0 = {0.f, 0.f, 0.f, 0.f}, a1 = {0.f, 0.f, 0.f, 0.f};
+                    if constexpr (S::BF) {
+                        const float4 z4 = make_float4(0.f, 0.f, 0.f, 0.f);
+#pragma unroll 2
+                        for (int ch = ch0; ch < ch1; ch += 2) {
+                            const int b = ch * kTile + 4 * lq;
+                            const bool two = ch + 1 < ch1;
+                            float av0[4], av1[4] = {0.f, 0.f, 0.f, 0.f};
+                            dh2_rows(b, av0);
+                            if (two) dh2_rows(b + kTile, av1);
+                            if (dsm) {
+                                dsum = (((dsum + av0[0]) + av0[1]) + av0[2]) + av0[3];
+                                dsum = (((dsum + av1[0]) + av1[1]) + av1[2]) + av1[3];
+                            }
+                            const float4 bb0 = *reinterpret_cast<const float4 *>(hb + b);
+                            const float4 bb1 = two ? *reinterpret_cast<const float4 *>(hb + b + kTile) : z4;
+                            a0 = mfma_bf16_pair(f4(av0), f4(av1), bb0, bb1, a0);
+                        }
+                    } else {
+#pragma unroll 2
+                        for (int ch = ch0; ch < ch1; ++ch) {
+                            const int b = ch * kTile + 4 * lq;
+                            float av[4];
+                            dh2_rows(b, av);
+                            if (dsm) dsum = (((dsum + av[0]) + av[1]) + av[2]) + av[3];
+                            const float4 bb = *reinterpret_cast<const float4 *>(hb + b);
+                            a0 = mfma4(av[0], bb.x, a0);
+                            a1 = mfma4(av[1], bb.y, a1);
+                            a0 = mfma4(av[2], bb.z, a0);
+                            a1 = mfma4(av[3], bb.w, a1);
+                        }
+                    }
+                    GS_STAMP(1)
+                    const f32x4 at = a0 + a1;
+#pragma unroll
+                    for (int r = 0; r < 4; ++r) red[(cw * 3 + hi) * 256 + (lq * 4 + r) * kTile + li] = at[r];
+                    if (dsm) red[(cw * 3 + 2) * 256 + lq * kTile + li] = dsum;
+                }
+            } else {
             if constexpr (S::BF) {
                 const float4 z4 = make_float4(0.f, 0.f, 0.f, 0.f);
 #pragma unroll 2
@@ -1556,6 +1655,7 @@
                 for (int r = 0; r < 4; ++r) red[(wave * 3 + t) * 256 + (lq * 4 + r) * kTile + li] = at[r];
             }
             if (kb == 0) red[(wave * 3 + 2) * 256 + lq * kTile + li] = dsum;
+            }
         } else {
             {
                 const int i = tid & 15;
@@ -1604,6 +1704,7 @@
                 const int j = t < sh.ka ? t : 2;
                 gv[j] = g;
                 ok[j] = t < sh.ka ? (n0 + row < H2 && k0 + t * kTile + col < H1) : (col == 0 && n0 + row < H2);
+                if constexpr (W8) ok[j] = ok[j] && tid < 256;
             }
             int db2n = n0 + row;
             if (fast && kb == 0) {
@@ -1651,7 +1752,7 @@
         GS_STAMP_BEGIN_IF(4, bid == 0)
         const int H2p = (H2 + 63) / 64 * 64;
         const int ld = H2p + 4;
-        const bool dh2_regs = A1 <= 5 && H2 % 64 == 0;
+        const bool dh2_regs = W8 || (A1 <= 5 && H2 % 64 == 0);
         float *dh2s = lds;
         float *W2T = dh2s + (dh2_regs ? round4(kRowsB / 16 * 16 * (D + 1)) : kRowsB * ld);
         float *whs = W2T + kTile * ld;
@@ -1660,8 +1761,8 @@
         float *xs = h1m + kRowsB * 16;
         float *tile = xs + round4(kRowsB * D);
         float *kred = tile + kRowsB * 17;
-        constexpr int kLd = FUSED ? 192 : 256;
-        int *mkB = reinterpret_cast<int *>(kred + 1024);
+        constexpr int kLd = FUSED ? NT - 64 : 256;
+        int *mkB = reinterpret_cast<int *>(kred + (W8 ? 2048 : 1024));
         if constexpr (S::H1c > 0 && S::Bc > 0) {
             constexpr Layout Lc = S::lay(Layout{});
             constexpr int cH1 = Lc.H1, cH2 = Lc.H2, cD = Lc.D, cA1 = Lc.A + 1, cB = S::Bc;
@@ -1669,7 +1770,7 @@
             constexpr int NM = (kRowsB * cncb + kLd - 1) / kLd, NW = (cH2p * 4 + kLd - 1) / kLd;
             constexpr int NH = (cA1 * cH2 + kLd - 1) / kLd, N1 = (kRowsB * 16 + kLd - 1) / kLd;
             constexpr int NX = (kRowsB * cD + kLd - 1) / kLd;
-            if (tid < kLd) {
+            if (W8 ? wave < NT / 64 - 1 : tid < kLd) {
                 int mr[NM];
                 float4 wr[NW];
                 float hr[NH], h1r[N1], xr[NX];
@@ -1764,13 +1865,13 @@
         }
 #endif
         if constexpr (FUSED) {
-            loss_rows_lds<S>(P, L, zpart, ff, la, B, kstep, b0, kRowsB, dzs, nullptr, kLd, 256 - kLd);
+            loss_rows_lds<S>(P, L, zpart, ff, la, B, kstep, b0, kRowsB, dzs, nullptr, kLd, NT - kLd);
         } else {
             for (int u = tid; u < kRowsB * A1; u += 256)
                 dzs[u] = b0 * A1 + u < B * A1 ? dz[(int64_t)b0 * A1 + u] : 0.0f;
         }
 #ifdef GS_STAMPS
-        if (bid == 0 && tid == 192) {
+        if (bid == 0 && tid == kLd) {
             asm volatile("s_waitcnt vmcnt(0) lgkmcnt(0)" ::: "memory");
             atomicAdd(&g_stamp_acc[7][0], __builtin_amdgcn_s_memtime() - t_rb0);
             atomicAdd(&g_stamp_cnt[7], 1ull);
@@ -1780,7 +1881,7 @@
         GS_STAMP(0)
         static_assert(kRowsB == 32 || kRowsB == 64, "role-B slabs of 32 or 64 rows");
         const int nchB = H2p / kTile;
-        const int rt = kRowsB == 64 ? wave : wave >> 1, half = kRowsB == 64 ? 0 : wave & 1;
+        const int rt = kRowsB == 64 ? cw : cw >> 1, half = kRowsB == 64 ? 0 : cw & 1;
         const int chb = half ? nchB / 2 : 0, che = (half || kRowsB == 64) ? nchB : nchB / 2;
         f32x4 acc0 = {0.f, 0.f, 0.f, 0.f}, acc1 = {0.f, 0.f, 0.f, 0.f};
         if (dh2_regs) {
@@ -1807,8 +1908,26 @@
                     av[j] = ((m >> j) & 1u) ? sacc : 0.0f;
                 }
             };
-            if constexpr (S::BF) {
+            if constexpr (W8 && !S::BF) {
+                auto chain = [&](auto sel) {
+                    constexpr int e = decltype(sel)::value;
+                    f32x4 a = {0.f, 0.f, 0.f, 0.f};
+#pragma unroll 2
+                    for (int ch = chb; ch < che; ++ch) {
+                        const int n = ch * kTile + 4 * lq;
+                        float av[4];
+                        dh2_cols(ch, av);
+                        const float4 w = *reinterpret_cast<const float4 *>(brow + n);
+                        a = mfma4(av[e], e ? w.y : w.x, a);
+                        a = mfma4(av[e + 2], e ? w.w : w.z, a);
+                    }
+                    return a;
+                };
+                if (hi) acc0 = chain(std::integral_constant<int, 1>{});
+                else acc0 = chain(std::integral_constant<int, 0>{});
+            } else if constexpr (S::BF) {
                 const float4 z4 = make_float4(0.f, 0.f, 0.f, 0.f);
+                if (!W8 || hi == 0)
 #pragma unroll 2
                 for (int ch = chb; ch < che; ch += 2) {
                     const int n = ch * kTile + 4 * lq;
@@ -1914,6 +2033,24 @@
             }
         }
         }
+        if constexpr (W8) {
+            constexpr bool kPairs = !S::BF;
+            if (kPairs || hi == 0) {
+                f32x4 acc = acc0;
+                if constexpr (!kPairs) acc = acc0 + acc1;
+#pragma unroll
+                for (int r = 0; r < 4; ++r) kred[wave * 256 + (lq * 4 + r) * kTile + li] = acc[r];
+            }
+            __syncthreads();
+            auto ktile = [&](int w, int e) { return kPairs ? kred[w * 256 + e] + kred[(w + 4) * 256 + e] : kred[w * 256 + e]; };
+            for (int u = tid; u < kRowsB * kTile; u += NT) {
+                const int row = u >> 4, col = u & 15;
+                const int t = row >> 4, rr = row & 15;
+                const float g = kRowsB == 64 ? ktile(t, rr * kTile + col)
+                                             : ktile(2 * t, rr * kTile + col) + ktile(2 * t + 1, rr * kTile + col);
+                tile[row * 17 + col] = h1m[row * 16 + col] > 0.0f ? g : 0.0f;
+            }
+        } else {
         {
             const f32x4 acc = acc0 + acc1;
 #pragma unroll
@@ -1927,13 +2064,14 @@
                                          : kred[(2 * t) * 256 + rr * kTile + col] + kred[(2 * t + 1) * 256 + rr * kTile + col];
             tile[row * 17 + col] = h1m[row * 16 + col] > 0.0f ? g : 0.0f;
         }
+        }
         __syncthreads();
         GS_STAMP(2)
         {
             constexpr int ng = kRowsB / 16;
             float *pr = dh2s;
             const int nout = kTile * (D + 1);
-            for (int u = tid; u < ng * nout; u += 256) {
+            for (int u = tid; u < ng * nout; u += NT) {
                 const int g = u / nout, o = u - g * nout;
                 const int col = o / (D + 1), d = o - col * (D + 1);
                 float s = 0.0f;
@@ -1965,7 +2103,7 @@
                     if (ok[j]) part1[((int64_t)rb * H1 + k0 + col) * (D + 1) + d] = pv[j];
                 }
             } else
-            for (int o = tid; o < nout; o += 256) {
+            for (int o = tid; o < nout; o += NT) {
                 const int col = o / (D + 1), d = o - col * (D + 1);
                 float t = 0.0f;
 #pragma unroll
@@ -1996,8 +2134,9 @@
                 }
             if (ge == 0) gs = 0;
         }
+        constexpr int kPartMin = W8 ? 2048 : 1024;
         double *dscrC = reinterpret_cast<double *>(
-            (reinterpret_cast<uintptr_t>(dzs + Bp * A1 + (A1 * 256 > 1024 ? A1 * 256 : 1024)) + 7) & ~(uintptr_t)7);
+            (reinterpret_cast<uintptr_t>(dzs + Bp * A1 + (A1 * 256 > kPartMin ? A1 * 256 : kPartMin)) + 7) & ~(uintptr_t)7);
         auto loss_in = [&]() {
             if constexpr (FUSED)
                 loss_rows_lds<S>(P, L, zpart, ff, la, B, kstep, 0, Bp, dzs, ge > gs ? dscrC : nullptr, 0, 256,
@@ -2008,6 +2147,42 @@
         if constexpr (S::H1c > 0 && S::Bc > 0) {
             constexpr Layout Lc = S::lay(Layout{});
             constexpr int cB = S::Bc, cBp = (cB + 15) / 16 * 16, NH = (cBp * 4 + 255) / 256;
+            if constexpr (W8) {
+                if (wave >= 4) {
+                    const int lt = tid - 256;
+                    float4 hr[NH];
+#pragma unroll
+                    for (int j = 0; j < NH; ++j) {
+                        const int u = lt + 256 * j, b = u >> 2, c4 = u & 3;
+                        hr[j] = *reinterpret_cast<const float4 *>(h2 + (int64_t)min(b, cB - 1) * Lc.H2 +
+                                                                  min(n0 + 4 * c4, Lc.H2 - 4));
+                    }
+#ifdef GS_STAMPS
+                    const unsigned long long t_ld0 = __builtin_amdgcn_s_memtime();
+#endif
+#pragma unroll
+                    for (int j = 0; j < NH; ++j) {
+                        const int u = lt + 256 * j, b = u >> 2, c4 = u & 3;
+                        if (u < cBp * 4) {
+                            const bool ok = b < cB && n0 + 4 * c4 < Lc.H2;
+                            hs[b * 17 + 4 * c4 + 0] = ok ? hr[j].x : 0.0f;
+                            hs[b * 17 + 4 * c4 + 1] = ok ? hr[j].y : 0.0f;
+                            hs[b * 17 + 4 * c4 + 2] = ok ? hr[j].z : 0.0f;
+                            hs[b * 17 + 4 * c4 + 3] = ok ? hr[j].w : 0.0f;
+                        }
+                    }
+#ifdef GS_STAMPS
+                    if (bid == 0 && lt == 0) {
+                        asm volatile("s_waitcnt vmcnt(0) lgkmcnt(0)" ::: "memory");
+                        atomicAdd(&g_stamp_acc[5][13], t_ld0 - _st_t0);
+                        atomicAdd(&g_stamp_acc[5][14], __builtin_amdgcn_s_memtime() - _st_t0);
+                    }
+#endif
+                } else {
+                    GS_STAMP_ENTRY
+                    loss_in();
+                }
+            } else {
             float4 hr[NH];
 #pragma unroll
             for (int j = 0; j < NH; ++j) {
@@ -2027,6 +2202,7 @@
                     hs[b * 17 + 4 * c4 + 2] = ok ? hr[j].z : 0.0f;
                     hs[b * 17 + 4 * c4 + 3] = ok ? hr[j].w : 0.0f;
                 }
+            }
             }
         } else {
 #pragma unroll 4
@@ -2055,7 +2231,7 @@
             if (A1 <= kTile) {
                 const int li = lane & 15, lq = lane >> 4;
                 const int nch = Bp / kTile;
-                const int ch0 = (wave * nch) / 4, ch1 = ((wave + 1) * nch) / 4;
+                const int ch0 = (cw * nch) / 4, ch1 = ((cw + 1) * nch) / 4;
                 f32x4 acc0 = {0.f, 0.f, 0.f, 0.f}, acc1 = {0.f, 0.f, 0.f, 0.f};
                 auto chunk = [&](int b, float (&av)[4], float (&bv)[4]) {
 #pragma unroll
@@ -2064,7 +2240,18 @@
                         bv[c] = hs[(b + c) * 17 + li];
                     }
                 };
-                if constexpr (S::BF) {
+                constexpr bool kPairs = W8 && !S::BF;
+                if constexpr (kPairs) {
+                    const int e = hi;
+#pragma unroll 2
+                    for (int ch = ch0; ch < ch1; ++ch) {
+                        const int b = ch * kTile + 4 * lq + e;
+                        const float a0 = li < A1 ? dzs[b * A1 + li] : 0.0f, a2 = li < A1 ? dzs[(b + 2) * A1 + li] : 0.0f;
+                        acc0 = mfma4(a0, hs[b * 17 + li], acc0);
+                        acc0 = mfma4(a2, hs[(b + 2) * 17 + li], acc0);
+                    }
+                } else if constexpr (S::BF) {
+                    if (!W8 || hi == 0)
 #pragma unroll 2
                     for (int ch = ch0; ch < ch1; ch += 2) {
                         const int b = ch * kTile + 4 * lq;
@@ -2085,12 +2272,24 @@
                     acc1 = mfma4(av[3], bv[3], acc1);
                 }
                 }
+                if constexpr (W8) {
+                    if (kPairs || hi == 0) {
+                        f32x4 acc = acc0;
+                        if constexpr (!kPairs) acc = acc0 + acc1;
+#pragma unroll
+                        for (int r = 0; r < 4; ++r) partC[wave * 256 + (lq * 4 + r) * kTile + li] = acc[r];
+                    }
+                } else {
                 const f32x4 acc = acc0 + acc1;
 #pragma unroll
                 for (int r = 0; r < 4; ++r) partC[wave * 256 + (lq * 4 + r) * kTile + li] = acc[r];
+                }
                 __syncthreads();
                 const int a = tid >> 4, i = tid & 15;
-                float hv[1] = {tid < nout ? ((partC[tid] + partC[256 + tid]) + partC[512 + tid]) + partC[768 + tid]
+                float hv[1] = {tid < nout ? (kPairs ? (((partC[tid] + partC[1024 + tid]) + (partC[256 + tid] + partC[1280 + tid])) +
+                                                       (partC[512 + tid] + partC[1536 + tid])) +
+                                                          (partC[768 + tid] + partC[1792 + tid])
+                                                    : ((partC[tid] + partC[256 + tid]) + partC[512 + tid]) + partC[768 + tid])
                                           : 0.0f};
                 bool ok[1] = {tid < nout && n0 + i < H2};
                 if (xchg) bwd_exchange<1>(bx, xseq, hv, ok);
@@ -2185,20 +2384,23 @@
     const int64_t *step_base;
     LossArgs la;
 };
-template <class S, bool BASE>
-__global__ __launch_bounds__(256) void k_bwd_chain(const float *__restrict__ P, const float *__restrict__ h1,
-                                                   const uint16_t *__restrict__ h2mask,
-                                                   const float *__restrict__ zpart, const float *__restrict__ fields,
-                                                   const float *__restrict__ x, int fstride, int k_local, BwdTail t)
+template <class S, bool BASE, int NT = 512>
+__global__ __launch_bounds__(NT) __attribute__((amdgpu_waves_per_eu(NT == 512 ? 2 : 1, NT == 512 ? 4 : 8)))
+void k_bwd_chain(const float *__restrict__ P, const float *__restrict__ h1,
+                                                  const uint16_t *__restrict__ h2mask,
+                                                  const float *__restrict__ zpart, const float *__restrict__ fields,
+                                                  const float *__restrict__ x, int fstride, int k_local, BwdTail t)
 {
     static_assert(S::Bc > 0 && S::H1c > 0, "chain entry: compile-time shapes only");
+    static_assert(NT == 256 || (S::lay(Layout{}).A + 1 <= 5 && S::lay(Layout{}).H2 % 64 == 0),
+                  "chain entry with 512 threads: A + 1 <= 5 and H2 a multiple of 64");
     FusedFwd ff{};
     ff.fa = reinterpret_cast<const int32_t *>(fields);
     ff.folp = fields + fstride, ff.fov = fields + 2 * (int64_t)fstride;
     ff.fadv = fields + 3 * (int64_t)fstride, ff.fret = fields + 4 * (int64_t)fstride;
     ff.mpart = t.mpart, ff.headsq = t.headsq, ff.step_base = t.step_base, ff.k_local = k_local;
-    bwd_body<S, true, false, BASE>(P, Layout{}, S::Bc, x, h1, t.h2, nullptr, t.G, t.part1, t.sumsq, nullptr, zpart, ff,
-                                   t.la, h2mask, BwdXchg{});
+    bwd_body<S, true, false, BASE, NT>(P, Layout{}, S::Bc, x, h1, t.h2, nullptr, t.G, t.part1, t.sumsq, nullptr, zpart,
+                                       ff, t.la, h2mask, BwdXchg{});
 }
 
 
@@ -2484,6 +2686,23 @@
     return ok && has_fused(L, B);
 }
 
+int bwd_chain_threads()
+{
+    const char *e = getenv("GS_BWD_NT");
+    return e && strcmp(e, "256") == 0 ? 256 : 512;
+}
+
+template <class S>
+static int set_chain_lds_limits(const Layout &L, int64_t B)
+{
+    const size_t l8 = bwd_lds_bytes(L, B, 512), l4 = bwd_lds_bytes(L, B, 256);
+    int r = set_lds_limit((const void *)k_bwd_chain<S, false, 512>, l8);
+    if (!r) r = set_lds_limit((const void *)k_bwd_chain<S, true, 512>, l8);
+    if (!r) r = set_lds_limit((const void *)k_bwd_chain<S, false, 256>, l4);
+    if (!r) r = set_lds_limit((const void *)k_bwd_chain<S, true, 256>, l4);
+    return r;
+}
+
 int prepare_kernels(const Layout &L, int64_t B)
 {
     if (has_bf16_chain(L, B)) {
@@ -2505,12 +2724,9 @@
             const size_t lds = bwd_lds_bytes(L, B);
             int r = set_lds_limit((const void *)k_bwd<Sh, true>, lds);
             if constexpr (chain_shape<Sh>()) {
-                if (!r) r = set_lds_limit((const void *)k_bwd_chain<Sh, false>, lds);
-                if (!r) r = set_lds_limit((const void *)k_bwd_chain<Sh, true>, lds);
-                if constexpr (bf16_shape<Sh>()) {
-                    if (!r) r = set_lds_limit((const void *)k_bwd_chain<Bf16Shape<Sh>, false>, lds);
-                    if (!r) r = set_lds_limit((const void *)k_bwd_chain<Bf16Shape<Sh>, true>, lds);
-                }
+                if (!r) r = set_chain_lds_limits<Sh>(L, B);
+                if constexpr (bf16_shape<Sh>())
+                    if (!r) r = set_chain_lds_limits<Bf16Shape<Sh>>(L, B);
             }
             return r;
         });
@@ -2572,11 +2788,13 @@
 }
 
 int launch_bwd(const float *P, const Layout &L, int64_t B, const Workspace &ws, float *G, const int32_t *stop,
-               hipStream_t s, const FusedFwd *ff, const LossArgs *la, const BwdXchg *bxp)
+               hipStream_t s, const FusedFwd *ff, const LossArgs *la, const BwdXchg *bxp, int chain_nt)
 {
     const BwdShape sh0 = BwdShape::make(L, (int)B, rows_b(L, B));
     const unsigned nblk = (unsigned)(sh0.nA + sh0.nB + sh0.nC);
     const size_t lds = bwd_lds_bytes(L, B);
+    if (chain_nt == 0) chain_nt = bwd_chain_threads();
+    GS_REQUIRE(chain_nt == 256 || chain_nt == 512, "k_bwd_chain: %d threads (256 or 512)", chain_nt);
     BwdXchg bx{};
     if (bxp && bxp->world > 1) {
         GS_REQUIRE(bwd_xchg_fits(L, B), "k_bwd exchange: %u workgroups or their output slots exceed the limits",
@@ -2601,17 +2819,21 @@
         auto chain = [&](auto shape) -> int {
             using S = decltype(shape);
             const float *fields = reinterpret_cast<const float *>(ff->fa);
-            const void *fn = ff->step_base ? (const void *)k_bwd_chain<S, true> : (const void *)k_bwd_chain<S, false>;
-            int rc = set_lds_limit(fn, lds);
-            if (rc) return rc;
-            if (ff->step_base)
-                hipLaunchKernelGGL((k_bwd_chain<S, true>), dim3(nblk), dim3(256), lds, s, P, ws.h1, ws.h2mask, ws.zpart,
-                                   fields, ws.x, (int)fstride, ff->k_local, t);
-            else
-                hipLaunchKernelGGL((k_bwd_chain<S, false>), dim3(nblk), dim3(256), lds, s, P, ws.h1, ws.h2mask,
+            auto go = [&](auto base, auto nt) -> int {
+                constexpr bool kBase = decltype(base)::value;
+                constexpr int kNT = decltype(nt)::value;
+                const size_t ldsc = bwd_lds_bytes(L, B, kNT);
+                int rc = set_lds_limit((const void *)k_bwd_chain<S, kBase, kNT>, ldsc);
+                if (rc) return rc;
+                hipLaunchKernelGGL((k_bwd_chain<S, kBase, kNT>), dim3(nblk), dim3(kNT), ldsc, s, P, ws.h1, ws.h2mask,
                                    ws.zpart, fields, ws.x, (int)fstride, ff->k_local, t);
-            GS_LAUNCH_CHECK("k_bwd_chain");
-            return GS_OK;
+                GS_LAUNCH_CHECK("k_bwd_chain");
+                return GS_OK;
+            };
+            using T8 = std::integral_constant<int, 512>;
+            using T4 = std::integral_constant<int, 256>;
+            if (ff->step_base) return chain_nt == 512 ? go(std::true_type{}, T8{}) : go(std::true_type{}, T4{});
+            return chain_nt == 512 ? go(std::false_type{}, T8{}) : go(std::false_type{}, T4{});
         };
         if (ff && la->bf16) {
             if constexpr (bf16_shape<Sh>()) {
diff --git a/gymnasium-solver_amd/csrc/gs_ppo.hip b/gymnasium-solver_amd/csrc/gs_ppo.hip
--- a/gymnasium-solver_amd/csrc/gs_ppo.hip
+++ b/gymnasium-solver_amd/csrc/gs_ppo.hip
@@ -369,6 +369,7 @@
     AdamArgs aa;
     bool sum_exchange;
     bool act_stats;
+    int bwd_nt;
 };
 
 StepArgs make_step_args(const gs_ppo_hparams &hp, const Layout &L, int64_t B, int64_t t,
@@ -464,7 +465,7 @@
     const bool inbwd = bwd_exchange_of(comm, L, B, &bx, sa.sum_exchange);
     int rc = launch_fwd_fused(P, L, B, ff, sa.la, ws, stop, s);
     if (rc) return rc;
-    rc = launch_bwd(P, L, B, ws, G, stop, s, &ff, &sa.la, inbwd ? &bx : nullptr);
+    rc = launch_bwd(P, L, B, ws, G, stop, s, &ff, &sa.la, inbwd ? &bx : nullptr, sa.bwd_nt);
     if (rc) return rc;
     if (!comm || inbwd) return launch_clip_adam(P, L, G, M, V, ws.part1, ws.sumsq, sa.aa, metrics, stop, s, false);
     return exchange_and_adam(P, G, M, V, L, sa, metrics, stop, ws, comm, s, &ff);
@@ -504,7 +505,7 @@
     af.aa = after ? exchanged_adam_args(sa_prev.aa, comm, sa_prev.sum_exchange) : sa_prev.aa;
     int rc = launch_fwd_fused(prev.P, L, B, ff, sa_prev.la, ws, stop, s, &af);
     if (rc) return rc;
-    rc = launch_bwd(cur.P, L, B, ws, G, stop, s, &ff, &sa_prev.la, inbwd ? &bx : nullptr);
+    rc = launch_bwd(cur.P, L, B, ws, G, stop, s, &ff, &sa_prev.la, inbwd ? &bx : nullptr, sa_prev.bwd_nt);
     if (rc || !after) return rc;
     int world = 1, n_slots = 0;
     rc = comm_grad_exchange(comm, G, L.P, Part1Fold{ws.part1, sa_prev.aa.nrb, L}, ws.sumsq, &n_slots, stop, s, &world);
@@ -739,6 +740,7 @@
         if (rc) return rc;
     }
     const bool lagged = fused && lagged_enabled() && has_lagged(L, batch);
+    const int bwd_nt = bwd_chain_threads();
     const ParamSet ps[2] = {{params, adam_m, adam_v}, {fw.p1, fw.m1, fw.v1}};
     if (lagged) GS_HIP(hipMemcpyAsync(fw.p1, params, sizeof(float) * (size_t)L.P, hipMemcpyDeviceToDevice, s));
     auto step_ff = [&](int64_t k_local, int64_t slot, const int64_t *base) {
@@ -752,10 +754,12 @@
         StepArgs sp = make_step_args(hp, L, batch, adam_step0 + k > 0 ? adam_step0 + k : 1);
         sp.aa.sched = sched;
         sp.aa.normsq = fw.normsq;
+        sp.bwd_nt = bwd_nt;
         return enqueue_step_lagged(ps, grads, L, sp, batch, step_ff(k, k, base), k, metrics, stop_flag, ws, comm, st);
     };
     auto with_norm = [&](StepArgs a, int64_t k) {
         a.aa.normsq = fw.normsq ? fw.normsq + k : nullptr;
+        a.bwd_nt = bwd_nt;
         return a;
     };
     auto finish = [&]() -> int {
@@ -814,7 +818,7 @@
     BwdXchg bx_key;
     const bool in_bwd = comm && bwd_exchange_of(comm, L, batch, &bx_key);
     key.n[4] = (int64_t)(intptr_t)stop_flag ^ ((int64_t)(intptr_t)comm << 1) ^ (fused ? 1 : 0) ^
-               ((int64_t)lagged << 62) ^ ((int64_t)in_bwd << 61);
+               ((int64_t)lagged << 62) ^ ((int64_t)in_bwd << 61) ^ ((int64_t)(fused && bwd_nt == 256) << 60);
     key.n[5] = ro.T * 1000003 + ro.N + (glob ? glob->batch_global << 40 : 0);
     uint32_t hbits[12];
     baked_hparam_bits(hp, hbits);
```
